# locuoco/coulomb_oscillators

Measured on AMD Instinct MI355X. Metric: particle-steps/sec (+ Gpair-interactions/sec), N=1048576 FMM-3D kd-tree p=6, 1 GPU(s), higher is better.
Workload: dtype f32; 1 GPU; FMM-3D kd-tree p=6, N=1048576 per GPU (one system of 1048576), leapfrog, Gaussian ball, tree rebuilt every 1 step(s); n_per_gpu=1048576, order=6, parallelism=single GPU, L=15, p2p_pairs=2017200, m2l_pairs=570291, build_mode=0, warm_builds=281, warm_misses=10, near_field=one-directional

## Files before the change

coulomb_oscillators_amd/csrc/k_farfield.hip:

```cpp
#include "nbco_internal.hpp"

namespace {

#include "fmm_ops.hpp"

constexpr int kBlock = 256;
constexpr int kTopNodes = 256;

__device__ inline float ld_agent(const float *p) { return __hip_atomic_load(p, __ATOMIC_RELAXED, __HIP_MEMORY_SCOPE_AGENT); }
__device__ inline int ld_agent(const int *p) { return __hip_atomic_load(p, __ATOMIC_RELAXED, __HIP_MEMORY_SCOPE_AGENT); }

template <int P, typename T>
__global__ __launch_bounds__(kBlock) void p2m_gen_kernel(const float4 *__restrict__ pos, const float *__restrict__ center,
                                                         const int *__restrict__ mult, const int *__restrict__ index, T *__restrict__ mpole,
                                                         int beg, int nleaf)
{
	constexpr int offM = P * (P + 1) * (P + 2) / 6;
	const int i = blockIdx.x * kBlock + threadIdx.x;
	if (i >= nleaf) return;
	const int leaf = beg + i, mlt = mult[leaf], ind = index[leaf];
	const T cx = (T)center[3 * leaf], cy = (T)center[3 * leaf + 1], cz = (T)center[3 * leaf + 2];
	T A[offM > 0 ? offM : 1];
#pragma unroll
	for (int k = 0; k < (offM > 0 ? offM : 1); ++k) A[k] = T(0);
// ... 32 lines not shown
	{
		float s = f0 * c0[a];
		s = s + f1 * c1[a];
		c[a] = s / ft;
	}
}
__device__ inline float4 node_csz(const float *__restrict__ lbound, const float *__restrict__ rbound, int i, float cx, float cy, float cz)
{
	const float dx = rbound[3 * i] - lbound[3 * i], dy = rbound[3 * i + 1] - lbound[3 * i + 1], dz = rbound[3 * i + 2] - lbound[3 * i + 2];
	const float sz = dx * dx + dy * dy + dz * dz;
	return make_float4(cx, cy, cz, sz);
}
#pragma clang fp contract(on)

__global__ __launch_bounds__(kBlock) void kd_centres_kernel(float *center, int *mult, int L, int lr, const float *__restrict__ lbound,
                                                            const float *__restrict__ rbound, float4 *__restrict__ csz, int leaves_too)
{
	__shared__ float Cl[kBlock][3];
	__shared__ int Nl[kBlock];
	const int t = threadIdx.x, b = blockIdx.x;
	const int nl = 1 << (L - lr);
	if (t < nl)
	{
		const int leaf = (1 << L) - 1 + b * nl + t;
		Cl[t][0] = center[3 * leaf]; Cl[t][1] = center[3 * leaf + 1]; Cl[t][2] = center[3 * leaf + 2];
		Nl[t] = mult[leaf];
		if (leaves_too) csz[leaf] = node_csz(lbound, rbound, leaf, Cl[t][0], Cl[t][1], Cl[t][2]);
	}
	__syncthreads();
	for (int l = L - 1; l >= lr; --l)
	{
		const int cnt = 1 << (l - lr);
		float c[3] = {0.f, 0.f, 0.f};
		int m0 = 0, m1 = 0;
		if (t < cnt)
		{
			m0 = Nl[2 * t]; m1 = Nl[2 * t + 1];
			centre_of(m0, m1, Cl[2 * t], Cl[2 * t + 1], c);
		}
		__syncthreads();
		if (t < cnt)
		{
			const int node = (1 << l) - 1 + b * cnt + t;
			Cl[t][0] = c[0]; Cl[t][1] = c[1]; Cl[t][2] = c[2];
			Nl[t] = m0 + m1;
			center[3 * node] = c[0]; center[3 * node + 1] = c[1]; center[3 * node + 2] = c[2];
			mult[node] = m0 + m1;
			csz[node] = node_csz(lbound, rbound, node, c[0], c[1], c[2]);
		}
		__syncthreads();
	}
}
__global__ __launch_bounds__(kBlock) void kd_centres_top_kernel(float *center, int *mult, int ltop, const float *__restrict__ lbound,
                                                                const float *__restrict__ rbound, float4 *__restrict__ csz)
{
	__shared__ float Cl[kBlock][3];
	__shared__ int Nl[kBlock];
	const int t = threadIdx.x;
	for (int l = ltop; l >= 0; --l)
	{
		const int cnt = 1 << l;
		float c[3] = {0.f, 0.f, 0.f};
		int mlt = 0;
		if (t < cnt)
		{
			if (l == ltop) parent_centre<false>(center, mult, (1 << l) - 1 + t, c, mlt);
			else
			{
				const int m0 = Nl[2 * t], m1 = Nl[2 * t + 1];
				centre_of(m0, m1, Cl[2 * t], Cl[2 * t + 1], c);
				mlt = m0 + m1;
			}
		}
		__syncthreads();
		if (t < cnt)
		{
			const int node = (1 << l) - 1 + t;
			Cl[t][0] = c[0]; Cl[t][1] = c[1]; Cl[t][2] = c[2];
			Nl[t] = mlt;
			center[3 * node] = c[0]; center[3 * node + 1] = c[1]; center[3 * node + 2] = c[2];
			mult[node] = mlt;
			csz[node] = node_csz(lbound, rbound, node, c[0], c[1], c[2]);
		}
		__syncthreads();
	}
}

template <int P, typename T>
__global__ __launch_bounds__(kTopNodes) void m2m_top_kernel(float *center, T *mpole, int *mult, int ltop, int lroot, int write_geom)
{
	constexpr int offM = P * (P + 1) * (P + 2) / 6, offS = offM > 0 ? offM : 1;
	extern __shared__ __attribute__((aligned(16))) unsigned char lds_raw[];
	const int width = 1 << (ltop - lroot);
	T *Ml = reinterpret_cast<T *>(lds_raw);
	float *Cl = reinterpret_cast<float *>(Ml + (size_t)width * offS);
	int *Nl = (int *)(Cl + (size_t)width * 3);
	const int t = threadIdx.x;
	for (int l = ltop; l >= lroot; --l)
	{
		const bool on = t < (1 << (l - lroot));
		const int k = (1 << l) - 1 + ((int)blockIdx.x << (l - lroot)) + t;
		T A[offS];
		float c[3] = {0.f, 0.f, 0.f};
		int mlt = 0;
		if (on)
		{
#pragma unroll
			for (int q = 0; q < offS; ++q) A[q] = T(0);
			if (l == ltop)
			{
				parent_centre<false>(center, mult, k, c, mlt);
				if (P >= 3)
					for (int ch = 0; ch < 2; ++ch)
					{
						const int child = 2 * k + 1 + ch;
						m2m_accum<P>(mpole + (size_t)child * offM, (T)c[0] - (T)center[3 * child], (T)c[1] - (T)center[3 * child + 1],
						             (T)c[2] - (T)center[3 * child + 2], A);
					}
			}
			else
			{
				const int s0 = 2 * t, s1 = 2 * t + 1;
				const int m0 = Nl[s0], m1 = Nl[s1];
				mlt = m0 + m1;
				centre_of(m0, m1, Cl + 3 * s0, Cl + 3 * s1, c);
				if (P >= 3)
					for (int ch = 0; ch < 2; ++ch)
					{
						const int sl = 2 * t + ch;
						m2m_accum<P>(Ml + (size_t)sl * offS, (T)c[0] - (T)Cl[3 * sl], (T)c[1] - (T)Cl[3 * sl + 1], (T)c[2] - (T)Cl[3 * sl + 2], A);
					}
			}
		}
		__syncthreads();
		if (on)
		{
			T *M = mpole + (size_t)k * offM;
			T *Ms = Ml + (size_t)t * offS;
			if (offM > 0) M[0] = (T)mlt;
			if (offM > 1) { M[1] = T(0); M[2] = T(0); M[3] = T(0); }
			m2m_store<P>(A, M);
			if (offM > 0) Ms[0] = (T)mlt;
			if (offM > 1) { Ms[1] = T(0); Ms[2] = T(0); Ms[3] = T(0); }
			m2m_store<P>(A, Ms);
			if (write_geom)
			{
				center[3 * k] = c[0]; center[3 * k + 1] = c[1]; center[3 * k + 2] = c[2];
				mult[k] = mlt;
			}
			Cl[3 * t] = c[0]; Cl[3 * t + 1] = c[1]; Cl[3 * t + 2] = c[2];
			Nl[t] = mlt;
		}
		__syncthreads();
	}
}

template <int P, typename T, bool AGENT>
__device__ inline void l2l_node(const float *center, T *local, int c)
{
	constexpr int offL = (P + 1) * (P + 1);
	const int p = (c - 1) >> 1;
	T Lp[offL], O[offL];
#pragma unroll
	for (int q = 0; q < offL; ++q) Lp[q] = local[(size_t)p * offL + q];
	l2l_body<P>(Lp, (T)center[3 * c] - (T)center[3 * p], (T)center[3 * c + 1] - (T)center[3 * p + 1], (T)center[3 * c + 2] - (T)center[3 * p + 2], O);
	T *Lc = local + (size_t)c * offL;
#pragma unroll
	for (int q = 1; q < offL; ++q) Lc[q] += O[q];
}

template <int P, typename T>
__global__ __launch_bounds__(kBlock) void l2l_gen_kernel(const float *__restrict__ center, T *local, int lchild, int first, int count)
{
	const int i = blockIdx.x * kBlock + threadIdx.x;
	if (i >= count) return;
	l2l_node<P, T, false>(center, local, (1 << lchild) - 1 + first + i);
}

template <int P, typename T>
__global__ __launch_bounds__(256) void l2l_sub_kernel(const float *__restrict__ center, T *local, int lroot, int L, int first)
{
	constexpr int offL = (P + 1) * (P + 1);
	extern __shared__ __attribute__((aligned(16))) unsigned char lds_raw[];
	T *lds = reinterpret_cast<T *>(lds_raw);
	const int t = threadIdx.x, r = first + blockIdx.x;
	for (int q = t; q < offL; q += blockDim.x) lds[q] = local[(size_t)((1 << lroot) - 1 + r) * offL + q];
	__syncthreads();
	for (int lc = lroot + 1; lc <= L; ++lc)
	{
		const bool on = t < (1 << (lc - lroot));
		const int c = (1 << lc) - 1 + (r << (lc - lroot)) + t, p = (c - 1) >> 1;
		T O[offL];
		if (on)
		{
			T Lp[offL];
			const T *src = lds + (size_t)(t >> 1) * offL;
#pragma unroll
			for (int q = 0; q < offL; ++q) Lp[q] = src[q];
			l2l_body<P>(Lp, (T)center[3 * c] - (T)center[3 * p], (T)center[3 * c + 1] - (T)center[3 * p + 1], (T)center[3 * c + 2] - (T)center[3 * p + 2], O);
			T *Lc = local + (size_t)c * offL;
#pragma unroll
			for (int q = 1; q < offL; ++q) { O[q] += Lc[q]; Lc[q] = O[q]; }
			O[0] = T(0);
		}
		if (lc == L) break;
		__syncthreads();
		if (on)
		{
			T *dst = lds + (size_t)t * offL;
#pragma unroll
			for (int q = 0; q < offL; ++q) dst[q] = O[q];
		}
		__syncthreads();
	}
}

template <int P, typename T>
__global__ __launch_bounds__(kBlock) void l2p_gen_kernel(const float4 *__restrict__ pos, const float *__restrict__ center,
                                                         const T *__restrict__ local, const float4 *__restrict__ near,
                                                         const int *__restrict__ chunk_off, const int *__restrict__ index, int mlt_max,
                                                         const int *__restrict__ unsort, int scatter, const float *__restrict__ param,
                                                         float *__restrict__ a_out, int have_near, long long n, int L, long long own0,
                                                         long long own_n, const int2 *__restrict__ sec_range, const float4 *__restrict__ react,
                                                         int react_cap, int react_stride)
{
	constexpr int offL = (P + 1) * (P + 1);
	const long long io = (long long)blockIdx.x * kBlock + threadIdx.x;
	if (io >= own_n) return;
	const long long i = own0 + io;
	const int lf = (int)(((1LL << L) * i) / n), leaf = (1 << L) - 1 + lf;
	const float4 p = pos[i];
	T Lp[offL];
#pragma unroll
	for (int q = 0; q < offL; ++q) Lp[q] = local[(size_t)leaf * offL + q];
	T fx, fy, fz;
	l2p_body<P>(Lp, (T)p.x - (T)center[3 * leaf], (T)p.y - (T)center[3 * leaf + 1], (T)p.z - (T)center[3 * leaf + 2], fx, fy, fz);
	if (have_near)
	{
		const int j = (int)(i - index[leaf]);
		float nx = 0.f, ny = 0.f, nz = 0.f;
		int ck0 = chunk_off[lf], ck1 = chunk_off[lf + 1];
		if (!NBCO_CHECKED_OK(ck0 >= 0 && ck0 <= ck1 && j >= 0 && j < mlt_max, NBCO_CHK_L2P)) ck1 = ck0;
#pragma unroll 8
		for (int ck = ck0; ck < ck1; ++ck)
		{
			const float4 nr = near[(size_t)ck * mlt_max + j];
			nx += nr.x; ny += nr.y; nz += nr.z;
		}
		if (sec_range)
		{
			int2 sr = sec_range[lf];
			if (!NBCO_CHECKED_OK(sr.x >= 0 && sr.x <= sr.y, NBCO_CHK_L2P)) sr.y = sr.x;
			if (sr.y > react_cap) sr.y = max(sr.x, react_cap);
#pragma unroll 8
			for (int e = sr.x; e < sr.y; ++e)
			{
				const float4 rr = react[(size_t)e * react_stride + j];
				nx += rr.x; ny += rr.y; nz += rr.z;
			}
		}
		fx += (T)nx; fy += (T)ny; fz += (T)nz;
	}
	const T scale = param ? (T)param[0] : T(1);
	const long long o = scatter ? (long long)unsort[io] : io;
	a_out[3 * o] = (float)(fx * scale); a_out[3 * o + 1] = (float)(fy * scale); a_out[3 * o + 2] = (float)(fz * scale);
}

#include "farfield_wide.hpp"

static int grid_for(long long n) { return (int)((n + kBlock - 1) / kBlock); }

template <int P, typename T>
static int run_upward_gen(nbco_ctx *c, const float4 *pos, float *center, T *mpole, int *mult, const int *index, int L, int write_geom)
{
	const int nleaf = 1 << L, beg = nleaf - 1;
	hipLaunchKernelGGL((p2m_gen_kernel<P, T>), dim3(grid_for(nleaf)), dim3(kBlock), 0, c->stream, pos, (const float *)center, (const int *)mult, index,
	                   mpole, beg, nleaf);
	constexpr int offM = P * (P + 1) * (P + 2) / 6, offS = offM > 0 ? offM : 1;
	int depth = 8;
	while (depth > 0 && (size_t)(1 << depth) * (offS * sizeof(T) + 16) > 60 * 1024) --depth;
	for (int l = L - 1; l >= 0;)
	{
		const int lroot = std::max(l - depth, 0), width = 1 << (l - lroot);
		hipLaunchKernelGGL((m2m_top_kernel<P, T>), dim3(1 << lroot), dim3(std::max(64, width)), (size_t)width * (offS * sizeof(T) + 16), c->stream, center, mpole,
		                   mult, l, lroot, write_geom);
		l = lroot - 1;
	}
	NBCO_HIP(hipGetLastError());
	return NBCO_OK;
}

template <int P, typename T>
static int run_m2m_top_gen(nbco_ctx *c, float *center, T *mpole, int *mult, int ltop, int write_geom)
{
	constexpr int offM = P * (P + 1) * (P + 2) / 6, offS = offM > 0 ? offM : 1;
	if ((1 << ltop) > kTopNodes || (size_t)(1 << ltop) * (offS * sizeof(T) + 16) > 60 * 1024)
		return c->fail(NBCO_ERR_UNSUPPORTED, "launch_m2m_top_gen: too many top levels");
	hipLaunchKernelGGL((m2m_top_kernel<P, T>), dim3(1), dim3(kTopNodes), (size_t)(1 << ltop) * (offS * sizeof(T) + 16), c->stream, center, mpole, mult, ltop, 0,
	                   write_geom);
	NBCO_HIP(hipGetLastError());
	return NBCO_OK;
}

template <int P, typename T>
static int run_downward_gen(nbco_ctx *c, const float *center, T *local, int L, int dom_d, int dom_g)
{
	constexpr int offL = (P + 1) * (P + 1);
	int top = kTopNodes;
	while (top > 4 && (size_t)top * offL * sizeof(T) > 60 * 1024) top >>= 1;
	int ltop = 1;
	while (ltop + 1 <= L && (1 << (ltop + 1)) <= top) ++ltop;
	{
	}
	constexpr int offD = P * (P + 1) * (P + 2) / 6;
	const int threads = 64 * ((std::max(offD, offL) + 63) / 64);
	const int wtop = ltop >= 2 ? std::max(ltop, L - 7) : 1;
	int lroot = L;
	if (ltop >= 2)
	{
		lroot = wtop;
		while (lroot < L && (size_t)(1 << (L - lroot - 1)) * offL * sizeof(T) > 60 * 1024) ++lroot;
		if (lroot < dom_d) lroot = L;
	}
	for (int lc = 2; lc <= lroot; ++lc)
	{
		const int first = lc >= dom_d ? dom_g << (lc - dom_d) : 0, count = lc >= dom_d ? 1 << (lc - dom_d) : 1 << lc;
		if (lc <= wtop) hipLaunchKernelGGL((l2l_wide_kernel<P, T>), dim3(count), dim3(threads), 0, c->stream, center, local, lc, first);
		else hipLaunchKernelGGL((l2l_gen_kernel<P, T>), dim3(grid_for(count)), dim3(kBlock), 0, c->stream, center, local, lc, first, count);
	}
	if (lroot < L)
	{
		const int first = dom_g << (lroot - dom_d), count = 1 << (lroot - dom_d);
		hipLaunchKernelGGL((l2l_sub_kernel<P, T>), dim3(count), dim3(std::max(64, 1 << (L - lroot))), (size_t)(1 << (L - lroot - 1)) * offL * sizeof(T),
		                   c->stream, center, local, lroot, L, first);
	}
	NBCO_HIP(hipGetLastError());
	return NBCO_OK;
}

template <int P, typename T>
static void launch_m2m_wide(nbco_ctx *c, float *center, T *mpole, int *mult, int l, int height, int write_geom)
{
	if (height <= 4) hipLaunchKernelGGL((m2m_wide_kernel<P, T, false>), dim3(1 << l), dim3(kWide), 0, c->stream, center, mpole, mult, l, write_geom);
	else hipLaunchKernelGGL((m2m_wide_kernel<P, T, true>), dim3(1 << l), dim3(kWide), 0, c->stream, center, mpole, mult, l, write_geom);
}
template <int P, typename T>
static int run_upward(nbco_ctx *c, const float4 *pos, float *center, T *mpole, int *mult, const int *index, int L, int write_geom)
{
	if constexpr (use_wide<P, T>())
	{
		const int nleaf = 1 << L;
		hipLaunchKernelGGL((p2m_wide_kernel<P, T>), dim3(nleaf), dim3(kWide), 0, c->stream, pos, (const float *)center, (const int *)mult, index, mpole,
		                   nleaf - 1);
		for (int l = L - 1; l >= 0; --l) launch_m2m_wide<P, T>(c, center, mpole, mult, l, L - l, write_geom);
		NBCO_HIP(hipGetLastError());
		return NBCO_OK;
	}
	else return run_upward_gen<P, T>(c, pos, center, mpole, mult, index, L, write_geom);
}
template <int P, typename T>
static int run_m2m_top(nbco_ctx *c, float *center, T *mpole, int *mult, int ltop, int L, int write_geom)
{
	if constexpr (use_wide<P, T>())
	{
		for (int l = ltop; l >= 0; --l) launch_m2m_wide<P, T>(c, center, mpole, mult, l, L - l, write_geom);
		NBCO_HIP(hipGetLastError());
		return NBCO_OK;
	}
	else return run_m2m_top_gen<P, T>(c, center, mpole, mult, ltop, write_geom);
}
template <int P, typename T>
static int run_downward(nbco_ctx *c, const float *center, T *local, int L, int dom_d, int dom_g)
{
	if constexpr (use_wide<P, T>())
	{
		for (int lc = 2; lc <= L; ++lc)
		{
			const int first = lc >= dom_d ? dom_g << (lc - dom_d) : 0, count = lc >= dom_d ? 1 << (lc - dom_d) : 1 << lc;
			hipLaunchKernelGGL((l2l_wide_kernel<P, T>), dim3(count), dim3(kWide), 0, c->stream, center, local, lc, first);
		}
		NBCO_HIP(hipGetLastError());
		return NBCO_OK;
	}
	else return run_downward_gen<P, T>(c, center, local, L, dom_d, dom_g);
}

template <int P, typename T>
static int run_l2p(nbco_ctx *c, const float4 *pos, const float *center, const T *local, const float4 *near, const int *chunk_off,
                   const int *index, int mlt_max, const int *unsort, int scatter, const float *param, float *a, int have_near, long long n, int L,
                   long long own0, long long own_n, const int2 *sec_range, const float4 *react, long long react_cap, int react_stride)
{
	hipLaunchKernelGGL((l2p_gen_kernel<P, T>), dim3(grid_for(own_n)), dim3(kBlock), 0, c->stream, pos, center, local, near, chunk_off, index, mlt_max,
	                   unsort, scatter, param, a, have_near, n, L, own0, own_n, sec_range, react, (int)std::min<long long>(react_cap, 0x7fffffff), react_stride);
	NBCO_HIP(hipGetLastError());
	return NBCO_OK;
}

}

#define NBCO_DISPATCH_P(P, CALL)                                                       \
	switch (P)                                                                         \
	{                                                                                  \
	case 1: return CALL(1); case 2: return CALL(2); case 3: return CALL(3); case 4: return CALL(4); \
	case 5: return CALL(5); case 6: return CALL(6); case 7: return CALL(7); case 8: return CALL(8); \
	case 9: return CALL(9); case 10: return CALL(10);                                                \
	default: return c->fail(NBCO_ERR_UNSUPPORTED, "generated far-field operators exist for orders 1..10"); \
	}

int launch_kd_centres(nbco_ctx *c, float *center, int *mult, int L, const float *lbound, const float *rbound, float4 *csz)
{
	if (L == 0)
	{
		hipLaunchKernelGGL(kd_centres_kernel, dim3(1), dim3(kBlock), 0, c->stream, center, mult, 0, 0, lbound, rbound, csz, 1);
		NBCO_HIP(hipGetLastError());
		return NBCO_OK;
	}
	int bottom = L;
	for (; bottom > 16; bottom -= 8)
		hipLaunchKernelGGL(kd_centres_kernel, dim3(1 << (bottom - 8)), dim3(kBlock), 0, c->stream, center, mult, bottom, bottom - 8, lbound, rbound, csz,
		                   bottom == L ? 1 : 0);
	const int lr = bottom > 8 ? bottom - 8 : 0;
	hipLaunchKernelGGL(kd_centres_kernel, dim3(1 << lr), dim3(kBlock), 0, c->stream, center, mult, bottom, lr, lbound, rbound, csz, bottom == L ? 1 : 0);
	if (lr > 0) hipLaunchKernelGGL(kd_centres_top_kernel, dim3(1), dim3(kBlock), 0, c->stream, center, mult, lr - 1, lbound, rbound, csz);
	NBCO_HIP(hipGetLastError());
	return NBCO_OK;
}

int launch_upward_gen(nbco_ctx *c, int P, const float4 *pos, float *center, void *mpole, int *mult, const int *index, int L, int write_geom, int f64)
{
	if (f64)
	{
#define CALL(PP) run_upward<PP, double>(c, pos, center, (double *)mpole, mult, index, L, write_geom)
		NBCO_DISPATCH_P(P, CALL)
#undef CALL
	}
#define CALL(PP) run_upward<PP, float>(c, pos, center, (float *)mpole, mult, index, L, write_geom)
	NBCO_DISPATCH_P(P, CALL)
#undef CALL
}

int launch_kd_centres_top(nbco_ctx *c, float *center, int *mult, int ltop, const float *lbound, const float *rbound, float4 *csz)
{
	if ((1 << ltop) > kBlock) return c->fail(NBCO_ERR_UNSUPPORTED, "launch_kd_centres_top: too many top levels");
	hipLaunchKernelGGL(kd_centres_top_kernel, dim3(1), dim3(kBlock), 0, c->stream, center, mult, ltop, lbound, rbound, csz);
	NBCO_HIP(hipGetLastError());
	return NBCO_OK;
}

int launch_m2m_top_gen(nbco_ctx *c, int P, float *center, void *mpole, int *mult, int ltop, int L, int write_geom, int f64)
{
	if (f64)
	{
#define CALL(PP) run_m2m_top<PP, double>(c, center, (double *)mpole, mult, ltop, L, write_geom)
		NBCO_DISPATCH_P(P, CALL)
#undef CALL
	}
#define CALL(PP) run_m2m_top<PP, float>(c, center, (float *)mpole, mult, ltop, L, write_geom)
	NBCO_DISPATCH_P(P, CALL)
#undef CALL
}

int launch_downward_gen(nbco_ctx *c, int P, const float *center, void *local, int L, int dom_d, int dom_g, int f64)
{
	if (f64)
	{
#define CALL(PP) run_downward<PP, double>(c, center, (double *)local, L, dom_d, dom_g)
		NBCO_DISPATCH_P(P, CALL)
#undef CALL
	}
#define CALL(PP) run_downward<PP, float>(c, center, (float *)local, L, dom_d, dom_g)
	NBCO_DISPATCH_P(P, CALL)
#undef CALL
}

int launch_l2p_gen(nbco_ctx *c, int P, const float4 *pos, const float *center, const void *local, const float4 *near, const int *chunk_off,
                   const int *index, int mlt_max, const int *unsort, int scatter, const float *param, float *a, int have_near, long long n, int L,
                   long long own0, long long own_n, const int2 *sec_range, const float4 *react, long long react_cap, int react_stride, int f64)
{
	if (f64)
	{
#define CALL(PP) run_l2p<PP, double>(c, pos, center, (const double *)local, near, chunk_off, index, mlt_max, unsort, scatter, param, a, have_near, n, L, own0, own_n, sec_range, react, react_cap, react_stride)
		NBCO_DISPATCH_P(P, CALL)
#undef CALL
	}
#define CALL(PP) run_l2p<PP, float>(c, pos, center, (const float *)local, near, chunk_off, index, mlt_max, unsort, scatter, param, a, have_near, n, L, own0, own_n, sec_range, react, react_cap, react_stride)
	NBCO_DISPATCH_P(P, CALL)
#undef CALL
}

NBCO_CHECKED_COLLECT(nbco_checked_collect_far)
```

coulomb_oscillators_amd/csrc/k_fmm_kd.hip:

```cpp
#include "nbco_internal.hpp"
#include "k_p2p.hpp"
#include "kd_common.hpp"
#include "host_util.hpp"
#include <chrono>
#include <cmath>
#include <algorithm>
#include <vector>

namespace {

using kdc::wave_scan_add;
using kdc::wave_min_u32;

constexpr int sym_off(int n) { return n * (n + 1) * (n + 2) / 6; }
constexpr int tl_off(int n) { return n * n; }

struct TreeView
{
	float *center, *lbound, *rbound;
	float4 *csz;
	float *mpole, *local;
	int *mult, *index, *splitdim;
	int L, ntot;
};

constexpr int kBlock = 256;

__host__ __device__ inline int kd_beg(int l) { return (1 << l) - 1; }
__host__ __device__ inline int kd_cnt(int l) { return 1 << l; }

struct Dom
{
	int d, g;
};
__host__ __device__ inline bool dom_touch(const Dom dm, int node)
{
#ifdef __HIP_DEVICE_COMPILE__
	const int l = 31 - __clz(node + 1);
#else
	int l = 0;
	while ((2 << l) <= node + 1) ++l;
#endif
	const int pos = node - ((1 << l) - 1);
	return l >= dm.d ? (pos >> (l - dm.d)) == dm.g : (dm.g >> (dm.d - l)) == pos;
}

#include "kd_build_kernels.hpp"
#include "kd_traverse_kernels.hpp"
#include "kd_list_kernels.hpp"

static int kd_levels(long long n, int p, float dens_inhom, int tree_L)
{
	int L;
	if (tree_L == 0)
	{
		float s = (float)(p * p);
		L = (int)std::round(std::log2(dens_inhom * (float)n / s));
	}
	else L = tree_L;
	L = std::max(2, std::min(30, L));
	while ((1LL << L) > n) --L;
	return L;
}

static TreeView view_of(const KdTreeDev &k)
{
	TreeView t;
	t.center = k.center; t.lbound = k.lbound; t.rbound = k.rbound; t.csz = k.csz; t.mpole = k.mpole; t.local = k.local;
	t.mult = k.mult; t.index = k.index; t.splitdim = k.splitdim; t.L = k.L; t.ntot = k.ntot;
	return t;
}

struct PackCounts
{
	__host__ __device__ uint64_t operator()(unsigned cnt) const { return (uint64_t)cnt | ((uint64_t)((cnt + kP2PChunk - 1) / kP2PChunk) << 32); }
};
struct SplitRef
{
	int *s, *o;
	__host__ __device__ SplitRef &operator=(uint64_t v) { *s = (int)(uint32_t)v; *o = (int)(v >> 32); return *this; }
};
struct SplitIter
{
	using iterator_category = std::random_access_iterator_tag;
	using value_type = uint64_t;
	using difference_type = std::ptrdiff_t;
	using pointer = uint64_t *;
	using reference = SplitRef;
	int *s, *o;
	__host__ __device__ SplitRef operator*() const { return SplitRef{s, o}; }
	__host__ __device__ SplitRef operator[](difference_type i) const { return SplitRef{s + i, o + i}; }
	__host__ __device__ SplitIter operator+(difference_type i) const { return SplitIter{s + i, o + i}; }
	__host__ __device__ SplitIter operator-(difference_type i) const { return SplitIter{s - i, o - i}; }
	__host__ __device__ SplitIter &operator+=(difference_type i) { s += i; o += i; return *this; }
	__host__ __device__ SplitIter &operator++() { ++s; ++o; return *this; }
	__host__ __device__ difference_type operator-(const SplitIter &b) const { return s - b.s; }
};
static int build_directed_list(nbco_ctx *c, const int2 *pairs, const int2 *ranks, const int *pref_dev, long long capR, long long npairs_hint, int sub,
                               int self0, int nself, int ntargets, int shift, unsigned *cnt, int *start, uint64_t *keys_tmp, uint64_t *keys_out,
                               DevBuf &scan_tmp, const int *leaf_index = nullptr, const int *leaf_mult = nullptr, int2 *desc = nullptr,
                               int *chunk_off = nullptr, int4 *chunks = nullptr, const MutualLists *mutual = nullptr)
{
	hipStream_t st = c->stream;
	if (desc)
	{
		NBCO_TRY(exclusive_scan(c, scan_tmp, rocprim::make_transform_iterator((const unsigned *)cnt, PackCounts{}), SplitIter{start, chunk_off}, (uint64_t)0,
		                        (size_t)(ntargets + 1)));
	}
	else
		NBCO_TRY(exclusive_scan(c, scan_tmp, (int *)cnt, start, 0, (size_t)(ntargets + 1)));
	hipLaunchKernelGGL(list_fill_kernel, dim3(grid1d(npairs_hint + nself)), dim3(kBlock), 0, st, pairs, ranks, pref_dev, capR, sub, self0, nself, shift,
	                   (const int *)start, keys_tmp, (const int *)chunk_off, ntargets, leaf_index, leaf_mult,
	                   (desc && !mutual) ? chunks : (int4 *)nullptr, mutual ? 1 : 0);
	if (desc)
	{
		MutualLists mu;
		if (mutual) { mu = *mutual; mu.chunk = chunks; mu.chunk_off = chunk_off; mu.self0 = self0; mu.nself = nself; }
		const bool long_kernel = shift >= 11 && shift <= 16 && c->hint_np2p > 0 && 2 * c->hint_np2p > 48LL * (nself > 0 ? nself : ntargets);
		const int long_from = long_kernel ? 512 : 0;
		c->info.long_lists = long_kernel ? 1 : 0;
		hipLaunchKernelGGL(list_segsort_kernel<true>, dim3((ntargets + kBlock / 64 - 1) / (kBlock / 64)), dim3(kBlock), 0, st, (const int *)start, ntargets,
		                   keys_tmp, keys_out, shift, leaf_index, leaf_mult, desc, mu, long_from);
		if (long_kernel)
			hipLaunchKernelGGL(list_longsort_kernel, dim3(256), dim3(kLongBlock), 0, st, (const int *)start,
			                   ntargets, (const uint64_t *)keys_tmp, keys_out, shift, leaf_index, leaf_mult, desc, mu, long_from);
	}
	else
		hipLaunchKernelGGL(list_segsort_kernel<false>, dim3((ntargets + kBlock / 64 - 1) / (kBlock / 64)), dim3(kBlock), 0, st, (const int *)start,
		                   ntargets, keys_tmp, keys_out, shift, (const int *)nullptr, (const int *)nullptr, (int2 *)nullptr, MutualLists{}, 0);
	NBCO_HIP(hipGetLastError());
	return NBCO_OK;
}

static int kd_carve(nbco_ctx *c, DevBuf &buf, KdTreeDev &k, int ntot, int offM, int offL)
{
	const size_t rb = c->o.far_fp64 ? 8 : 4;
	k.real_bytes = (int)rb;
	size_t bytes = (size_t)ntot * (3 * 3 * sizeof(float) + sizeof(float4) + (size_t)(offM + offL) * rb + 3 * sizeof(int)) + 256 + 64;
	NBCO_TRY(c->reserve(buf, bytes));
	char *q = (char *)buf.ptr;
	k.csz = (float4 *)q; q += sizeof(float4) * (size_t)ntot;
	k.center = (float *)q; q += 12 * (size_t)ntot;
	k.lbound = (float *)q; q += 12 * (size_t)ntot;
	k.rbound = (float *)q; q += 12 * (size_t)ntot;
	q = (char *)(((uintptr_t)q + 15) & ~(uintptr_t)15);
	k.mpole = (float *)q; q += rb * (size_t)ntot * offM;
	q = (char *)(((uintptr_t)q + 15) & ~(uintptr_t)15);
	k.local = (float *)q; q += rb * (size_t)ntot * offL;
	q = (char *)(((uintptr_t)q + 15) & ~(uintptr_t)15);
	k.mult = (int *)q; q += 4 * (size_t)ntot;
	k.index = (int *)q; q += 4 * (size_t)ntot;
	k.splitdim = (int *)q;
	return NBCO_OK;
}

static int kd_build_top(nbco_ctx *c, const TreeView &tv, float4 *&pos, float4 *&pos_alt, int *&unsort, int *&unsort_alt, long long n, int l0,
                        bool use_select, bool select_ready = false, bool warm = false, const KdRoot &root = KdRoot{})
{
	hipStream_t st = c->stream;
	if (use_select && l0 > 0 && !select_ready) NBCO_TRY(kd_select_begin(c, l0));
	for (int l = 0; l < l0; ++l)
	{
		if (use_select)
			NBCO_TRY(kd_select_level(c, l, n, pos, unsort, pos_alt, unsort_alt, tv.lbound, tv.rbound, tv.splitdim, tv.index,
			                         c->counters.as<int>() + 110, warm, root));
		else
		{
			if (l > 0) hipLaunchKernelGGL(kd_box_kernel, dim3(grid1d(kd_cnt(l))), dim3(kBlock), 0, st, tv, pos, n, l);
			hipLaunchKernelGGL(kd_keys_kernel, dim3(grid1d(n)), dim3(kBlock), 0, st, pos, tv.splitdim + kd_beg(l), n, l,
			                   c->keys.as<uint64_t>(), c->idx.as<uint32_t>());
			NBCO_TRY(sort_pairs(c, c->sort_tmp, c->keys.as<uint64_t>(), c->keys_alt.as<uint64_t>(), c->idx.as<uint32_t>(), c->idx_alt.as<uint32_t>(), n, 0u,
			                    (unsigned)(32 + l)));
			hipLaunchKernelGGL(kd_permute_kernel, dim3(grid1d(n)), dim3(kBlock), 0, st, pos, unsort, c->idx_alt.as<uint32_t>(), pos_alt, unsort_alt, n);
		}
		std::swap(pos, pos_alt);
		std::swap(unsort, unsort_alt);
	}
	if (l0 > 0 && !use_select) hipLaunchKernelGGL(kd_box_kernel, dim3(grid1d(kd_cnt(l0))), dim3(kBlock), 0, st, tv, pos, n, l0);
	NBCO_HIP(hipGetLastError());
	return NBCO_OK;
}

static int kd_reserve_particles(nbco_ctx *c, long long n)
{
	NBCO_TRY(c->reserve(c->pos4, sizeof(float4) * (size_t)n));
	NBCO_TRY(c->reserve(c->pos4_alt, sizeof(float4) * (size_t)n));
	NBCO_TRY(c->reserve(c->unsort, sizeof(int) * (size_t)n));
	NBCO_TRY(c->reserve(c->unsort_alt, sizeof(int) * (size_t)n));
	NBCO_TRY(c->reserve(c->keys, sizeof(uint64_t) * (size_t)n));
	NBCO_TRY(c->reserve(c->keys_alt, sizeof(uint64_t) * (size_t)n));
	NBCO_TRY(c->reserve(c->idx, sizeof(uint32_t) * (size_t)n));
	NBCO_TRY(c->reserve(c->idx_alt, sizeof(uint32_t) * (size_t)n));
	NBCO_TRY(c->reserve(c->counters, sizeof(int) * 128));
	return NBCO_OK;
}

static int kd_top_levels(long long n, int L)
{
	int l0 = 0;
	while (l0 < L && (n + (1LL << l0) - 1) / (1LL << l0) > kSubS) ++l0;
	return l0;
}

static int kd_build(nbco_ctx *c, const float *p, long long n, int L, const KdRoot &root, bool &rebuild, KdStepLink *link)
{
	const int P = c->o.fmm_order;
	const int ntot = (1 << (L + 1)) - 1, nleaf = 1 << L;
	const int mlt_max = (int)((n - 1) / nleaf + 1);
	hipStream_t st = c->stream;
	NBCO_TRY(c->join_aux());
	KdTreeDev &k = c->kd;
	const int old_real = k.real_bytes;
	NBCO_TRY(kd_carve(c, c->treebuf, k, ntot, sym_off(P), tl_off(P + 1)));
	const bool topo_change = k.L != L || k.ntot != ntot || k.order != P || k.n != n || k.real_bytes != old_real;
	if (topo_change) c->tree_valid = false;
	k.L = L; k.ntot = ntot; k.order = P; k.mlt_max = mlt_max; k.n = n;
	NBCO_TRY(kd_reserve_particles(c, n));
	rebuild = c->o.unsort || !c->tree_valid || (c->eval_counter % c->o.tree_steps) == 0;
	TreeView tv = view_of(c->kd);
	float4 *pos = c->pos4.as<float4>(), *pos_alt = c->pos4_alt.as<float4>();
	int *unsort = c->unsort.as<int>(), *unsort_alt = c->unsort_alt.as<int>();
	PhaseScope ph(c, NBCO_PH_BUILD);
	const int prep_done = link ? link->prep_done : 0;
	if (rebuild)
	{
		const int l0 = kd_top_levels(n, L);
		const bool use_select = !c->force_sort_build;
		long long words_a = 0, words_b = 0;
		if (use_select && l0 > 0) NBCO_TRY(kd_select_begin(c, l0, false, &words_a, &words_b));
		if (!c->prep_state.ptr)
		{
			NBCO_TRY(c->reserve(c->prep_state, 64));
			const unsigned arm[8] = {0xFFFFFFFFu, 0xFFFFFFFFu, 0xFFFFFFFFu, 0u, 0u, 0u, 0u, 0u};
			NBCO_HIP(hipMemcpyAsync(c->prep_state.ptr, arm, sizeof arm, hipMemcpyHostToDevice, st));
			NBCO_HIP(hipStreamSynchronize(st));
		}
		if (c->perm_primed_n != n)
		{
			hipLaunchKernelGGL(iota_kernel, dim3(grid1d(n)), dim3(kBlock), 0, st, unsort_alt, n);
			hipLaunchKernelGGL(iota_kernel, dim3(grid1d(n)), dim3(kBlock), 0, st, unsort, n);
			c->perm_primed_n = n;
		}
		if (prep_done != 1)
			hipLaunchKernelGGL(kd_prep_kernel, dim3(kPrepGrid), dim3(kPrepBlock), 0, st, p, n, pos, unsort, c->sel_hist.as<uint32_t>(), words_a,
			                   c->sel_nodes.as<uint32_t>(), words_b, c->counters.as<int>() + 110, c->prep_state.as<unsigned>(), tv, root.root6);
		bool warm = use_select && l0 > 0 && c->sel_warm_enabled && c->tree_valid && !c->sel_three_pass;
		if (warm && c->sel_warm_cooldown > 0) { --c->sel_warm_cooldown; warm = false; }
		c->sel_warm_used = warm;
		if (warm) ++c->sel_warm_builds;
		NBCO_TRY(kd_build_top(c, tv, pos, pos_alt, unsort, unsort_alt, n, l0, use_select, true, warm, root));
		int launches = 1;
#ifdef NBCO_SUBTREE_PROF
		if (std::getenv("NBCO_SUBTREE_TWICE")) launches = 2;
#endif
		for (int i = 0; i < launches; ++i)
			hipLaunchKernelGGL(kd_subtree_kernel, dim3(kd_cnt(l0)), dim3(kSubT), 0, st, tv, (const float4 *)pos, (const int *)unsort, pos_alt, unsort_alt, n, l0,
			                   use_select ? 1 : 0, c->sel_three_pass ? 0 : 1, c->counters.as<int>() + 110, root.top_sd, root.top_root1);
		std::swap(pos, pos_alt);
		std::swap(unsort, unsort_alt);
		NBCO_HIP(hipGetLastError());
		if (pos != c->pos4.as<float4>()) { std::swap(c->pos4, c->pos4_alt); std::swap(c->unsort, c->unsort_alt); }
	}
	else
	{
		c->sel_warm_used = false;
		if (prep_done == 0)
		{
			NBCO_TRY(launch_pack4(c, pos, p, n));
			NBCO_HIP(hipMemsetAsync(c->counters.as<int>() + 110, 0, sizeof(int), st));
		}
		hipLaunchKernelGGL(kd_leaf_kernel, dim3(grid1d(nleaf)), dim3(kBlock), 0, st, tv, pos, n);
	}
	if (link) link->prep_done = 0;
	NBCO_TRY(launch_kd_centres(c, tv.center, tv.mult, L, tv.lbound, tv.rbound, tv.csz));
	NBCO_HIP(hipGetLastError());
	return NBCO_OK;
}

static int kd_upward(nbco_ctx *c)
{
	const KdTreeDev &k = c->kd;
	NBCO_TRY(c->fork_aux());
	StreamScope on_aux(c, c->aux);
	PhaseScope ph(c, NBCO_PH_P2M_M2M);
	NBCO_TRY(launch_upward_gen(c, k.order, c->pos4.as<float4>(), k.center, k.mpole, k.mult, k.index, k.L, 0, k.real_bytes == 8));
	NBCO_HIP(hipGetLastError());
	return NBCO_OK;
}

struct LetHave { const unsigned char *node, *leaf; };
constexpr int kLetWord = 16;
__global__ __launch_bounds__(kBlock) void let_guard_kernel(const uint64_t *__restrict__ keys, const int *__restrict__ total, int shift,
                                                           const unsigned char *__restrict__ have, int *__restrict__ host_word)
{
	const uint64_t mask = (1ull << shift) - 1;
	const int n = *total;
	int missing = 0;
	for (int i = blockIdx.x * kBlock + threadIdx.x; i < n; i += gridDim.x * kBlock)
	{
		const int id = (int)(keys[i] & mask);
		if (!have[id]) missing = id + 1;
	}
	if (missing) { *host_word = missing; __threadfence_system(); }
}
static int launch_let_guard(nbco_ctx *c, const uint64_t *keys, const int *total, int shift, const unsigned char *have, int word, long long hint)
{
	hipLaunchKernelGGL(let_guard_kernel, dim3(grid1d(hint, 2048)), dim3(kBlock), 0, c->stream, keys, total, shift, have,
	                   c->h_flags + kLetWord + 2 * (int)(c->dist.let_epoch & 1) + word);
	NBCO_HIP(hipGetLastError());
	return NBCO_OK;
}

struct KdCounts
{
	long long np2p = 0, nm2l = 0;
	int sel_overflow = 0, react_overflow = 0;
};

static int kd_list_room(nbco_ctx *c, int ntot, long long &capR, long long &cap)
{
	capR = 2 * (((long long)c->o.list_factor * c->list_growth * ntot + 4096 + kTravK - 1) / kTravK);
	cap = capR * kTravK;
	NBCO_TRY(c->reserve(c->frontier_a, sizeof(int2) * (size_t)cap));
	NBCO_TRY(c->reserve(c->frontier_b, sizeof(int2) * (size_t)cap));
	NBCO_TRY(c->reserve(c->p2p_list, sizeof(int2) * 2 * (size_t)cap));
	NBCO_TRY(c->reserve(c->m2l_list, sizeof(int2) * 2 * (size_t)cap));
	NBCO_TRY(c->reserve(c->counters, sizeof(int) * 128));
	c->list_cap = cap;
	return NBCO_OK;
}

static int kd_traverse(nbco_ctx *c, const TreeView &tv, long long n, const Dom dm)
{
	const int L = tv.L, ntot = tv.ntot, nleaf = 1 << L;
	const int self0 = dm.g << (L - dm.d), nself = 1 << (L - dm.d);
	hipStream_t st = c->stream;
	long long capR, cap;
	NBCO_TRY(kd_list_room(c, ntot, capR, cap));
	PhaseScope ph(c, NBCO_PH_TRAVERSE);
	AdmTab tab;
	for (int l = 0; l < 32; ++l)
	{
		long long lo = l <= L ? (n >> l) : 0;
		long long hi = l <= L ? ((n + (1LL << l) - 1) >> l) : 0;
		tab.lo[l] = (int)lo;
		const float e = 1.f / (float)(3 * c->o.fmm_order + 6);
		tab.Mlo[l] = lo > 0 ? std::pow((float)lo / (float)n, e) : 0.f;
		tab.Mhi[l] = hi > 0 ? std::pow((float)hi / (float)n, e) : 0.f;
	}
	int *ctr = c->counters.as<int>();
	int2 *fa = c->frontier_a.as<int2>(), *fb = c->frontier_b.as<int2>();
	const size_t np_ = (size_t)nleaf + 2, nm_ = (size_t)ntot + 2;
	NBCO_TRY(c->reserve(c->list_cnt, sizeof(unsigned) * 2 * (np_ + nm_)));
	unsigned *cnt_p2p = c->list_cnt.as<unsigned>(), *cnt_m2l = cnt_p2p + 2 * np_;
	NBCO_TRY(c->reserve(c->trav_ctr, sizeof(int) * 1024));
	static_assert(kTcInts <= 1024, "traversal counter block");
	int *tctr = c->trav_ctr.as<int>();
	NBCO_TRY(c->flags_begin());
	hipLaunchKernelGGL(traverse_init_kernel, dim3(grid1d((long long)(2 * (np_ + nm_)) / 8 + 1, 256)), dim3(kBlock), 0, st, fa, ctr, 104, tctr,
	                   c->list_cnt.as<unsigned>(), (long long)(2 * (np_ + nm_)), (long long)self0, (long long)(c->o.coll ? nself : 0));
	const int iters = L + NBCO_TRAV_EXTRA;
	for (int it = 0; it < iters; ++it)
	{
		hipLaunchKernelGGL(traverse_kernel, dim3(1024), dim3(kBlock), 0, st, tv, tab, (const int2 *)fa, fb, c->p2p_list.as<int2>(),
		                   c->m2l_list.as<int2>(), c->p2p_list.as<int2>() + cap, c->m2l_list.as<int2>() + cap, ctr, tctr, it, capR,
		                   c->o.tree_radius, c->o.m2l_first, cnt_p2p, cnt_m2l, dm);
		std::swap(fa, fb);
	}
	hipLaunchKernelGGL(traverse_finish_kernel, dim3(1), dim3(1024), 0, st, ctr, tctr, capR, c->list_cnt.as<unsigned>(), (long long)(2 * (np_ + nm_)),
	                   cnt_p2p + self0, c->o.coll ? nself : 0, c->h_flags, iters, ++c->flags_seq);
	NBCO_HIP(hipGetLastError());
	NBCO_HIP(hipEventRecord(c->ev_flags, st));
	return NBCO_OK;
}

static int kd_no_pre_far() { return NBCO_OK; }

template <class PreFar>
static int kd_fields(nbco_ctx *c, const TreeView &tv, const float4 *pos, long long n, int mlt_max, const Dom dm, long long own0, long long own_n,
                     const int *unsort, float *a, const float *param, KdCounts &out, PreFar pre_far, const LetHave *let = nullptr)
{
	const int P = c->o.fmm_order;
	const int L = tv.L, ntot = tv.ntot, nleaf = 1 << L, beg = kd_beg(L);
	const int offL = tl_off(P + 1);
	out = KdCounts{};
	const int self0 = dm.g << (L - dm.d), nself = 1 << (L - dm.d);
	long long capR, cap;
	NBCO_TRY(kd_list_room(c, ntot, capR, cap));
	const int *p2p_pref = c->trav_ctr.as<int>() + kTcP2PPref, *m2l_pref = c->trav_ctr.as<int>() + kTcM2LPref;
	const int shift = L + 1;
	const long long dp2p_cap = c->o.coll ? 2 * cap + nself : 0, dm2l_cap = 2 * cap;
	const long long np2p_hint = c->hint_np2p > 0 ? std::min(cap, c->hint_np2p + c->hint_np2p / 4 + 1024) : cap;
	const long long nm2l_hint = c->hint_nm2l > 0 ? std::min(cap, c->hint_nm2l + c->hint_nm2l / 4 + 1024) : cap;
	const long long dp2p_hint = 2 * np2p_hint + nself;
	const long long max_chunks = c->o.coll ? dp2p_cap / kP2PChunk + nself : 0, chunks_hint = dp2p_hint / kP2PChunk + nself;
	const int mutual_th = (c->o.coll && c->o.p2p_mutual) ? p2p_mutual_halves(mlt_max) : 0;
	const bool mutual = mutual_th > 0;
	c->info.p2p_halves = mutual_th;
	long long react_cap = 0;
	if (mutual)
	{
		if (c->hint_np2p <= 0)
		{
			NBCO_TRY(c->wait_flags());
			c->hint_np2p = c->h_flags[0];
			c->hint_nm2l = c->h_flags[1];
		}
		const long long pairs_room = std::min(cap, c->hint_np2p + c->hint_np2p / 4 + 1024);
		react_cap = 2 * pairs_room + nself;
		NBCO_TRY(c->reserve(c->p2p_react, sizeof(float4) * 32 * (size_t)mutual_th * (size_t)react_cap));
	}
	float4 *near = nullptr;
	auto enqueue_p2p = [&]() -> int {
		NBCO_TRY(c->reserve(c->part, sizeof(float4) * (size_t)max_chunks * (size_t)mlt_max));
		near = c->part.as<float4>();
		PhaseScope ph(c, NBCO_PH_P2P);
		const int4 *pc = c->p2p_chunks.as<int4>();
		const int *pt = c->p2p_chunk_off.as<int>() + nleaf;
		const int2 *pd = c->p2p_desc.as<int2>();
		if (mutual)
		{
			launch_p2p_mutual(c, mutual_th, pos, c->p2p_desc.as<int4>(), pc, pt, chunks_hint, mlt_max, near, c->p2p_react.as<float4>(), react_cap, n);
		}
		else if (mlt_max <= 8) launch_p2p<8>(c, pos, pd, pc, pt, chunks_hint, mlt_max, mlt_max, near, n);
		else if (mlt_max <= 16) launch_p2p<16>(c, pos, pd, pc, pt, chunks_hint, mlt_max, mlt_max, near, n);
		else if (mlt_max <= 32) launch_p2p<32>(c, pos, pd, pc, pt, chunks_hint, mlt_max, mlt_max, near, n);
		else launch_p2p<64>(c, pos, pd, pc, pt, chunks_hint, mlt_max, mlt_max, near, n);
		NBCO_HIP(hipGetLastError());
		static const char *dump_path = std::getenv("NBCO_P2P_DUMP");
		if (dump_path && !mutual) NBCO_TRY(p2p_dump(c, dump_path, pos, pd, pc, pt, c->p2p_start.as<int>() + nleaf, mlt_max, near, n));
		return NBCO_OK;
	};
	{
		NBCO_TRY(c->reserve(c->p2p_keys, sizeof(uint64_t) * (size_t)(dp2p_cap + 1)));
		NBCO_TRY(c->reserve(c->p2p_keys_alt, sizeof(uint64_t) * (size_t)(dp2p_cap + 1)));
		NBCO_TRY(c->reserve(c->m2l_keys, sizeof(uint64_t) * (size_t)(dm2l_cap + 1)));
		NBCO_TRY(c->reserve(c->m2l_keys_alt, sizeof(uint64_t) * (size_t)(dm2l_cap + 1)));
		NBCO_TRY(c->reserve(c->p2p_start, sizeof(int) * (size_t)(nleaf + 2)));
		NBCO_TRY(c->reserve(c->m2l_start, sizeof(int) * (size_t)(ntot + 2)));
		NBCO_TRY(c->fork_mark());
		if (c->o.coll)
		{
			PhaseScope ph(c, NBCO_PH_LISTS);
			unsigned *cp = c->list_cnt.as<unsigned>();
			NBCO_TRY(c->reserve(c->p2p_desc, (mutual ? sizeof(int4) : sizeof(int2)) * (size_t)(dp2p_cap + 1)));
			MutualLists mu;
			if (mutual)
			{
				NBCO_TRY(c->reserve(c->p2p_sec, sizeof(int2) * (size_t)(nleaf + 2)));
				mu.desc4 = c->p2p_desc.as<int4>();
				mu.sec_range = c->p2p_sec.as<int2>();
			}
			NBCO_TRY(c->reserve(c->p2p_chunk_off, sizeof(int) * (size_t)(nleaf + 2)));
			NBCO_TRY(c->reserve(c->p2p_chunks, sizeof(int4) * (size_t)max_chunks));
			NBCO_TRY(build_directed_list(c, c->p2p_list.as<int2>(), c->p2p_list.as<int2>() + cap, p2p_pref, capR, np2p_hint, beg, self0, nself, nleaf, shift, cp,
			                             c->p2p_start.as<int>(), c->p2p_keys.as<uint64_t>(), c->p2p_keys_alt.as<uint64_t>(), c->sort_tmp,
			                             tv.index + beg, tv.mult + beg, c->p2p_desc.as<int2>(), c->p2p_chunk_off.as<int>(), c->p2p_chunks.as<int4>(),
			                             mutual ? &mu : nullptr));
			if (mutual) launch_p2p_link(c, c->p2p_desc.as<int4>(), c->p2p_keys_alt.as<uint64_t>(), c->p2p_start.as<int>(), c->p2p_start.as<int>() + nleaf, shift, dp2p_hint);
			if (let) NBCO_TRY(launch_let_guard(c, c->p2p_keys_alt.as<uint64_t>(), c->p2p_start.as<int>() + nleaf, shift, let->leaf, 1, dp2p_hint));
			c->pc_mult = tv.mult + beg; c->pc_shift = shift; c->pc_total = c->p2p_start.as<int>() + nleaf;
		}
		if (c->o.coll) NBCO_TRY(enqueue_p2p());
		const int f64 = c->o.far_fp64 ? 1 : 0;
		NBCO_HIP(hipMemsetAsync(tv.local, 0, (f64 ? sizeof(double) : sizeof(float)) * (size_t)ntot * offL, c->aux));
		NBCO_TRY(c->fork_wait());
		{
			StreamScope on_aux(c, c->aux);
			NBCO_TRY(pre_far());
			unsigned *cm = c->list_cnt.as<unsigned>() + 2 * ((size_t)nleaf + 2);
			NBCO_TRY(build_directed_list(c, c->m2l_list.as<int2>(), c->m2l_list.as<int2>() + cap, m2l_pref, capR, nm2l_hint, 0, 0, 0, ntot, shift, cm,
			                             c->m2l_start.as<int>(), c->m2l_keys.as<uint64_t>(), c->m2l_keys_alt.as<uint64_t>(), c->scan_tmp_aux));
			if (let) NBCO_TRY(launch_let_guard(c, c->m2l_keys_alt.as<uint64_t>(), c->m2l_start.as<int>() + ntot, shift, let->node, 0, 2 * nm2l_hint));
			{
				PhaseScope ph(c, NBCO_PH_M2L);
				if (f64) NBCO_TRY(launch_m2l_lanes_f64(c, P, tv.csz, (const double *)tv.mpole, (double *)tv.local, c->m2l_keys_alt.as<uint64_t>(), c->m2l_start.as<int>(), shift, ntot));
				else NBCO_TRY(launch_m2l_lanes(c, P, tv.csz, tv.mpole, tv.local, c->m2l_keys_alt.as<uint64_t>(), c->m2l_start.as<int>(), shift, ntot));
			}
			{
				PhaseScope ph(c, NBCO_PH_L2L);
				NBCO_TRY(launch_downward_gen(c, P, tv.center, tv.local, L, dm.d, dm.g, f64));
			}
		}
		NBCO_HIP(hipGetLastError());
	}
	NBCO_TRY(c->join_aux());
	{
		PhaseScope ph(c, NBCO_PH_L2P);
		NBCO_TRY(launch_l2p_gen(c, P, pos, tv.center, tv.local, near, c->p2p_chunk_off.as<int>(), tv.index, mlt_max, unsort, c->o.unsort ? 1 : 0,
		                        param, a, c->o.coll ? 1 : 0, n, L, own0, own_n, mutual ? c->p2p_sec.as<int2>() : nullptr,
		                        mutual ? c->p2p_react.as<float4>() : nullptr, react_cap, 32 * mutual_th, c->o.far_fp64 ? 1 : 0));
	}
	{
		const auto t0 = std::chrono::steady_clock::now();
		NBCO_TRY(c->wait_flags());
		c->host_wait_s += std::chrono::duration<double>(std::chrono::steady_clock::now() - t0).count();
	}
	const int *h = c->h_flags;
	if (h[3] != 0)
	{
		out.sel_overflow = 1;
		return NBCO_OK;
	}
	if (h[2] == 2) return c->fail(NBCO_ERR_HIP, "internal error: the dual tree traversal did not finish in its launches");
	if (h[2] != 0) return c->fail(NBCO_ERR_CAPACITY, "dual tree traversal exceeded the list capacity (raise opts.list_factor or set opts.list_grow)");
	out.np2p = h[0]; out.nm2l = h[1];
	c->hint_np2p = h[0]; c->hint_nm2l = h[1];
	{
		nbco_ctx::LastEval &le = c->last_eval;
		le.valid = true;
		le.center = tv.center; le.csz = tv.csz; le.mpole = tv.mpole; le.mult = tv.mult; le.index = tv.index;
		le.L = L; le.ntot = ntot; le.order = P; le.shift = shift; le.real_bytes = c->o.far_fp64 ? 8 : 4;
		le.pos = pos; le.n = n; le.own0 = own0; le.own_n = own_n;
		le.have_p2p = c->o.coll != 0;
	}
	if (mutual && 2LL * h[0] + nself > react_cap) out.react_overflow = 1;
	return NBCO_OK;
}

static int kd_finish_order(nbco_ctx *c, float *p, long long n, KdStepLink *link)
{
	PhaseScope ph(c, NBCO_PH_FINISH);
	hipStream_t st = c->stream;
	NBCO_TRY(c->reserve(c->tmp3, sizeof(float) * 3 * (size_t)n));
	const int *order_in = nullptr;
	int *order_out = nullptr;
	if (c->o.track_order)
	{
		NBCO_TRY(c->reserve(c->order, sizeof(int) * (size_t)n));
		NBCO_TRY(c->reserve(c->order_alt, sizeof(int) * (size_t)n));
		if (c->order_n == n) order_in = c->order.as<int>();
		order_out = c->order_alt.as<int>();
	}
	else c->order_n = -1;
	hipLaunchKernelGGL(reorder_state_kernel, dim3(grid1d(n)), dim3(kBlock), 0, st, (const float4 *)c->pos4.as<float4>(), (const int *)c->unsort.as<int>(),
	                   (const float *)(p + 3 * n), p, c->tmp3.as<float>(), n, order_in, order_out);
	if (order_out) { std::swap(c->order, c->order_alt); c->order_n = n; }
	if (link && link->defer_v_copy) link->v_now = c->tmp3.as<float>();
	else NBCO_HIP(hipMemcpyAsync(p + 3 * n, c->tmp3.ptr, sizeof(float) * 3 * (size_t)n, hipMemcpyDeviceToDevice, st));
	NBCO_HIP(hipGetLastError());
	return NBCO_OK;
}

#include "kd_energy_kernels.hpp"
}

int kd_energy_fmm(nbco_ctx *c, long long n_own, double *half_phi_sum)
{
	const nbco_ctx::LastEval &le = c->last_eval;
	if (!le.valid || !c->tree_valid) return c->fail(NBCO_ERR_ARG, "nbco_energy_fmm: no kd-tree evaluation to take the lists from");
	if (le.own_n != n_own) return c->fail(NBCO_ERR_ARG, "nbco_energy_fmm: particle count differs from the last evaluation's");
	const int grid = (int)((le.own_n + kBlock - 1) / kBlock);
	NBCO_TRY(c->reserve(c->part, sizeof(double) * (size_t)grid));
	double *part = c->part.as<double>();
	switch (le.order)
	{
	case 1: launch_potential<1>(c, grid, part); break;
	case 2: launch_potential<2>(c, grid, part); break;
	case 3: launch_potential<3>(c, grid, part); break;
	case 4: launch_potential<4>(c, grid, part); break;
	case 5: launch_potential<5>(c, grid, part); break;
	case 6: launch_potential<6>(c, grid, part); break;
	case 7: launch_potential<7>(c, grid, part); break;
	case 8: launch_potential<8>(c, grid, part); break;
	case 9: launch_potential<9>(c, grid, part); break;
	case 10: launch_potential<10>(c, grid, part); break;
	default: return c->fail(NBCO_ERR_UNSUPPORTED, "nbco_energy_fmm: order");
	}
	NBCO_HIP(hipGetLastError());
	std::vector<double> h((size_t)grid);
	NBCO_HIP(hipMemcpyAsync(h.data(), part, sizeof(double) * (size_t)grid, hipMemcpyDeviceToHost, c->stream));
	NBCO_HIP(hipStreamSynchronize(c->stream));
	double s = 0.0;
	for (double v : h) s += v;
	*half_phi_sum = 0.5 * s;
	return NBCO_OK;
}

static bool kd_wants_room(nbco_ctx *c, int rc, const KdCounts &cnt, int ntot)
{
	if (rc == NBCO_ERR_CAPACITY) return c->grow_lists(ntot);
	return rc == NBCO_OK && cnt.react_overflow && !cnt.sel_overflow;
}

static int kd_retry(nbco_ctx *c, int rc, const KdCounts &cnt, bool rebuild, int ntot, bool &again)
{
	again = true;
	if (kd_wants_room(c, rc, cnt, ntot)) return NBCO_OK;
	if (rc != NBCO_OK) return rc;
	if (cnt.sel_overflow)
		return c->demote_build() ? NBCO_OK : c->fail(NBCO_ERR_UNSUPPORTED, "kd-tree build: tie flag raised by the sorting build");
	if (rebuild && c->sel_warm_used) c->note_warm_ok();
	again = false;
	return NBCO_OK;
}

static void kd_commit(nbco_ctx *c, const KdTreeDev &k, long long n, const KdCounts &cnt, bool rebuilt)
{
	c->tree_valid = true;
	c->tree_n = n;
	c->tree_order = k.order;
	c->eval_counter += 1;
	nbco_kd_info &info = c->info;
	info.L = k.L; info.ntot = k.ntot; info.order = k.order; info.mlt_max = k.mlt_max; info.n = k.n;
	info.p2p_pairs = cnt.np2p; info.m2l_pairs = cnt.nm2l; info.rebuilt = rebuilt ? 1 : 0;
	info.directed_p2p = -1;
}

int kd_finish_pending_order(nbco_ctx *c, float *p, long long n, KdStepLink *link)
{
	if (!link->order_pending) return NBCO_OK;
	link->order_pending = false;
	return kd_finish_order(c, p, n, link);
}

int kd_turnaround(nbco_ctx *c, float *p, const float *param, float ks, float ds, bool elastic, long long n, KdStepLink *link, const float *root6)
{
	const bool gather = link->order_pending;
	link->order_pending = false;
	float *x = p, *v = p + 3 * n, *a = p + 6 * n;
	const float *v_in = link->v_now ? link->v_now : v;
	const int L = c->kd.L;
	const bool next_rebuild = (c->eval_counter % c->o.tree_steps) == 0;
	long long words_a = 0, words_b = 0;
	if (next_rebuild)
	{
		const int l0 = kd_top_levels(n, L);
		if (!c->force_sort_build && l0 > 0) NBCO_TRY(kd_select_begin(c, l0, false, &words_a, &words_b));
	}
	float *v_out = v;
	if (gather)
	{
		NBCO_TRY(c->reserve(c->tmp3, sizeof(float) * 3 * (size_t)n));
		NBCO_TRY(c->reserve(c->tmp3b, sizeof(float) * 3 * (size_t)n));
		v_out = v_in == c->tmp3.as<float>() ? c->tmp3b.as<float>() : c->tmp3.as<float>();
	}
	else if (v_in != v) v_out = const_cast<float *>(v_in);
	PhaseScope ph(c, NBCO_PH_AXPY);
	TreeView tv = view_of(c->kd);
	hipStream_t st = c->stream;
#define NBCO_TURN_ARGS c->pos4.as<float4>(), c->unsort.as<int>(), x, v_in, v_out, (const float *)a, param, ks, ds, elastic ? 1 : 0, n, next_rebuild ? 1 : 0, \
	c->sel_hist.as<uint32_t>(), words_a, c->sel_nodes.as<uint32_t>(), words_b, c->counters.as<int>() + 110, c->prep_state.as<unsigned>(), tv, root6
	if (gather) hipLaunchKernelGGL(kd_turnaround_kernel<true>, dim3(kPrepGrid), dim3(kPrepBlock), 0, st, NBCO_TURN_ARGS);
	else hipLaunchKernelGGL(kd_turnaround_kernel<false>, dim3(kPrepGrid), dim3(kPrepBlock), 0, st, NBCO_TURN_ARGS);
#undef NBCO_TURN_ARGS
	NBCO_HIP(hipGetLastError());
	link->prep_done = next_rebuild ? 1 : 2;
	c->order_n = -1;
	c->last_eval.valid = false;
	link->v_now = v_out == v ? nullptr : v_out;
	return NBCO_OK;
}

int fmm_kdtree_eval(nbco_ctx *c, float *p, float *a, long long n, const float *param, KdStepLink *link)
{
	if (n <= 0) return c->fail(NBCO_ERR_ARG, "nbco_fmm_kdtree: n must be positive");
	if (n > 0x7fffffffLL / 4) return c->fail(NBCO_ERR_UNSUPPORTED, "nbco_fmm_kdtree: n too large for 32-bit tree indices");
	const int L = kd_levels(n, c->o.fmm_order, c->o.dens_inhom, c->o.tree_L);
	const Dom whole{0, 0};
	bool rebuild = false;
	KdCounts cnt;
	for (bool again = true; again;)
	{
		NBCO_TRY(kd_build(c, p, n, L, KdRoot{}, rebuild, link));
		NBCO_TRY(kd_upward(c));
		const TreeView tv = view_of(c->kd);
		int rc = kd_traverse(c, tv, n, whole);
		if (rc == NBCO_OK) rc = kd_fields(c, tv, c->pos4.as<float4>(), n, c->kd.mlt_max, whole, 0, n, c->unsort.as<int>(), a, param, cnt, kd_no_pre_far);
		NBCO_TRY(kd_retry(c, rc, cnt, rebuild, c->kd.ntot, again));
	}
	if (!c->o.unsort && rebuild)
	{
		if (link && link->defer_order) link->order_pending = true;
		else NBCO_TRY(kd_finish_order(c, p, n, link));
	}
	kd_commit(c, c->kd, n, cnt, rebuild);
	return NBCO_OK;
}

#include "kd_dist.hpp"
#include "kd_let.hpp"
int kd_count_pairs(nbco_ctx *c, long long *out)
{
	if (!c->pc_mult || !c->p2p_keys_alt.ptr) { *out = 0; return NBCO_OK; }
	unsigned long long *ctr = (unsigned long long *)(c->counters.as<int>() + 100);
	NBCO_HIP(hipMemsetAsync(ctr, 0, sizeof(unsigned long long), c->stream));
	hipLaunchKernelGGL(pair_count_kernel, dim3(1024), dim3(kBlock), 0, c->stream, c->pc_mult, (const uint64_t *)c->p2p_keys_alt.as<uint64_t>(), c->pc_total,
	                   c->pc_shift, ctr);
	NBCO_HIP(hipGetLastError());
	unsigned long long v = 0;
	NBCO_HIP(hipMemcpyAsync(&v, ctr, sizeof v, hipMemcpyDeviceToHost, c->stream));
	NBCO_HIP(hipStreamSynchronize(c->stream));
	*out = (long long)v;
	return NBCO_OK;
}

int kd_copy_out(nbco_ctx *c, int which, void *dst, long long bytes)
{
	const KdTreeDev &k = c->kd;
	if (!c->tree_valid) return c->fail(NBCO_ERR_ARG, "nbco_kd_copy: no kd-tree evaluation has run");
	const void *src = nullptr;
	size_t need = 0;
	const int offM = sym_off(k.order), offL = tl_off(k.order + 1);
	switch (which)
	{
	case NBCO_KD_MULT: src = k.mult; need = 4 * (size_t)k.ntot; break;
	case NBCO_KD_INDEX: src = k.index; need = 4 * (size_t)k.ntot; break;
	case NBCO_KD_SPLITDIM: src = k.splitdim; need = 4 * (size_t)k.ntot; break;
	case NBCO_KD_CENTER: src = k.center; need = 12 * (size_t)k.ntot; break;
	case NBCO_KD_LBOUND: src = k.lbound; need = 12 * (size_t)k.ntot; break;
	case NBCO_KD_RBOUND: src = k.rbound; need = 12 * (size_t)k.ntot; break;
	case NBCO_KD_MPOLE: src = k.mpole; need = (size_t)k.real_bytes * (size_t)k.ntot * offM; break;
	case NBCO_KD_LOCAL: src = k.local; need = (size_t)k.real_bytes * (size_t)k.ntot * offL; break;
	case NBCO_KD_P2P_LIST:
	case NBCO_KD_M2L_LIST:
	{
		const bool p2p = which == NBCO_KD_P2P_LIST;
		need = 8 * (size_t)(p2p ? c->info.p2p_pairs : c->info.m2l_pairs);
		const long long capR = c->list_cap / kTravK;
		hipLaunchKernelGGL(list_compact_kernel, dim3(1024), dim3(kBlock), 0, c->stream, (const int2 *)(p2p ? c->p2p_list.ptr : c->m2l_list.ptr),
		                   (const int *)(c->trav_ctr.as<int>() + (p2p ? kTcP2PPref : kTcM2LPref)), capR, c->frontier_a.as<int2>());
		NBCO_HIP(hipGetLastError());
		src = c->frontier_a.ptr;
		break;
	}
	case NBCO_KD_UNSORT: src = c->unsort.ptr; need = 4 * (size_t)k.n; break;
	case NBCO_KD_ORDER:
		if (!c->o.track_order || c->order_n != k.n) return c->fail(NBCO_ERR_ARG, "nbco_kd_copy: NBCO_KD_ORDER needs opts.track_order and unsort = 0 evaluations");
		src = c->order.ptr; need = 4 * (size_t)k.n; break;
	default: return c->fail(NBCO_ERR_ARG, "nbco_kd_copy: unknown array");
	}
	if ((long long)need > bytes) return c->fail(NBCO_ERR_ARG, "nbco_kd_copy: destination too small");
	NBCO_HIP(hipStreamSynchronize(c->stream));
	if (need) NBCO_HIP(hipMemcpy(dst, src, need, hipMemcpyDeviceToHost));
	return NBCO_OK;
}

NBCO_CHECKED_COLLECT(nbco_checked_collect_kd)
```

coulomb_oscillators_amd/csrc/k_m2l.hip:

```cpp
#include "nbco_internal.hpp"

namespace {

__device__ __forceinline__ float nb_fma(float a, float b, float c) { return __builtin_fmaf(a, b, c); }
__device__ __forceinline__ double nb_fma(double a, double b, double c) { return __builtin_fma(a, b, c); }
__device__ __forceinline__ float nb_sqrt(float x) { return sqrtf(x); }
__device__ __forceinline__ double nb_sqrt(double x) { return sqrt(x); }

template <int P, typename T> struct M2LBody;

#include "m2l_gen.inc"

constexpr int kTargets = 6;

template <int P, typename T>
__global__ __launch_bounds__(64) void m2l_lane_kernel(const float4 *__restrict__ csz, const T *__restrict__ mpole,
                                                      T *__restrict__ local, const uint64_t *__restrict__ keys,
                                                      const int *__restrict__ start, int shift, int ntot, float eps2, int mstride)
{
	constexpr int offM = P * (P + 1) * (P + 2) / 6, offL = (P + 1) * (P + 1), NOUT = offL - 1;
	constexpr int CPL = (NOUT + 63) / 64;
	__shared__ T buf[64][NOUT + 1 + (NOUT % 2)];
	__shared__ int tg[64];
	const int lane = threadIdx.x;
	const int t0 = blockIdx.x * kTargets, t1 = min(t0 + kTargets, ntot);
	const int i0 = start[t0], i1 = start[t1];
	const uint64_t mask = (1ull << shift) - 1;
	T acc[CPL];
#pragma unroll
	for (int q = 0; q < CPL; ++q) acc[q] = T(0);
	int cur = -1;
	for (int base = i0; base < i1; base += 64)
	{
		const int i = base + lane;
		int tgt = -1;
		T L[NOUT];
		if (i < i1)
		{
			const uint64_t key = keys[i];
			tgt = (int)(key >> shift);
			const int src = (int)(key & mask);
			const float4 ct = csz[tgt], cs = csz[src];
			const T dx = (T)ct.x - (T)cs.x, dy = (T)ct.y - (T)cs.y, dz = (T)ct.z - (T)cs.z;
			const T r = nb_sqrt(dx * dx + dy * dy + dz * dz + (T)eps2);
			const T rinv = T(1) / r;
			M2LBody<P, T>::run(mpole + (size_t)src * mstride, dx * rinv, dy * rinv, dz * rinv, rinv, L);
		}
		else
		{
#pragma unroll
			for (int c = 0; c < NOUT; ++c) L[c] = T(0);
		}
#pragma unroll
		for (int c = 0; c < NOUT; ++c) buf[lane][c] = L[c];
		tg[lane] = tgt;
		__syncthreads();
		const int rows = min(64, i1 - base);
		constexpr int RB = 8;
		for (int r0 = 0; r0 < rows; r0 += RB)
		{
			T v[RB][CPL];
			int tt[RB];
#pragma unroll
			for (int k = 0; k < RB; ++k)
			{
				const int r = min(r0 + k, 63);
				tt[k] = tg[r];
#pragma unroll
				for (int q = 0; q < CPL; ++q)
				{
					const int c = lane + 64 * q;
					v[k][q] = c < NOUT ? buf[r][c] : T(0);
				}
			}
#pragma unroll
			for (int k = 0; k < RB; ++k)
			{
				if (r0 + k >= rows) break;
				const int t = tt[k];
				if (t != cur)
				{
					if (cur >= 0)
					{
#pragma unroll
						for (int q = 0; q < CPL; ++q)
						{
							const int c = lane + 64 * q;
							if (c < NOUT) local[(size_t)cur * offL + 1 + c] = acc[q];
						}
					}
#pragma unroll
					for (int q = 0; q < CPL; ++q) acc[q] = T(0);
					cur = t;
				}
#pragma unroll
				for (int q = 0; q < CPL; ++q) acc[q] += v[k][q];
			}
		}
		__syncthreads();
	}
	if (cur >= 0)
	{
#pragma unroll
		for (int q = 0; q < CPL; ++q)
		{
			const int c = lane + 64 * q;
			if (c < NOUT) local[(size_t)cur * offL + 1 + c] = acc[q];
		}
	}
}

template <int P, typename T>
static void launch(nbco_ctx *c, const float4 *csz, const T *mpole, T *local, const uint64_t *keys, const int *start, int shift, int ntot, int mstride)
{
	const int grid = (ntot + kTargets - 1) / kTargets;
	hipLaunchKernelGGL((m2l_lane_kernel<P, T>), dim3(grid), dim3(64), 0, c->stream, csz, mpole, local, keys, start, shift, ntot, c->o.eps2,
	                   mstride > 0 ? mstride : P * (P + 1) * (P + 2) / 6);
}

template <typename T>
static int dispatch(nbco_ctx *c, int P, const float4 *csz, const T *mpole, T *local, const uint64_t *keys, const int *start, int shift, int ntot, int mstride)
{
	switch (P)
	{
	case 1: launch<1, T>(c, csz, mpole, local, keys, start, shift, ntot, mstride); break;
	case 2: launch<2, T>(c, csz, mpole, local, keys, start, shift, ntot, mstride); break;
	case 3: launch<3, T>(c, csz, mpole, local, keys, start, shift, ntot, mstride); break;
	case 4: launch<4, T>(c, csz, mpole, local, keys, start, shift, ntot, mstride); break;
	case 5: launch<5, T>(c, csz, mpole, local, keys, start, shift, ntot, mstride); break;
	case 6: launch<6, T>(c, csz, mpole, local, keys, start, shift, ntot, mstride); break;
	case 7: launch<7, T>(c, csz, mpole, local, keys, start, shift, ntot, mstride); break;
	case 8: launch<8, T>(c, csz, mpole, local, keys, start, shift, ntot, mstride); break;
	case 9: launch<9, T>(c, csz, mpole, local, keys, start, shift, ntot, mstride); break;
	case 10: launch<10, T>(c, csz, mpole, local, keys, start, shift, ntot, mstride); break;
	default: return c->fail(NBCO_ERR_UNSUPPORTED, "launch_m2l_lanes: order not generated");
	}
	NBCO_HIP(hipGetLastError());
	return NBCO_OK;
}

}

int launch_m2l_lanes(nbco_ctx *c, int P, const float4 *csz, const float *mpole, float *local, const uint64_t *keys, const int *start,
                     int shift, int ntot, int mstride)
{
	return dispatch<float>(c, P, csz, mpole, local, keys, start, shift, ntot, mstride);
}
int launch_m2l_lanes_f64(nbco_ctx *c, int P, const float4 *csz, const double *mpole, double *local, const uint64_t *keys, const int *start,
                         int shift, int ntot, int mstride)
{
	return dispatch<double>(c, P, csz, mpole, local, keys, start, shift, ntot, mstride);
}
```

coulomb_oscillators_amd/csrc/kd_traverse_kernels.hpp:

```cpp

__device__ inline uint64_t block_exclusive_scan3(uint64_t v, uint64_t *sh_wave, uint64_t &total)
{
	const int lane = threadIdx.x & 63, w = threadIdx.x >> 6;
	const uint64_t incl = (uint64_t)wave_scan_add((uint32_t)(v & 0xFFFFFu)) | ((uint64_t)wave_scan_add((uint32_t)((v >> 20) & 0xFFFFFu)) << 20) |
	                      ((uint64_t)wave_scan_add((uint32_t)(v >> 40)) << 40);
	if (lane == 63) sh_wave[w] = incl;
	__syncthreads();
	uint64_t base = 0, tot = 0;
	for (int k = 0; k < 4; ++k)
	{
		uint64_t s = sh_wave[k];
		if (k < w) base += s;
		tot += s;
	}
	total = tot;
	return base + incl - v;
}

__device__ inline int classify_pair(const TreeView &t, const AdmTab *tab, int2 np, float par, int m2l_first, const Dom dm)
{
	const int ntot = t.ntot;
	if (dm.d > 0 && !dom_touch(dm, np.x) && !dom_touch(dm, np.y)) return 0;
	const bool leaf1 = 2 * np.x + 1 >= ntot, leaf2 = 2 * np.y + 1 >= ntot;
	if (!m2l_first && leaf1 && leaf2) return (np.x != np.y) ? 1 : 0;
	if (np.x == np.y) return leaf1 ? 0 : 3;
	const float4 c1 = t.csz[np.x], c2 = t.csz[np.y];
	if (kd_admissible(c1, c2, np.x, np.y, t.mult, tab, par)) return 2;
	if (leaf1 && leaf2) return 1;
	return (leaf1 || (!leaf2 && c1.w <= c2.w)) ? 4 : 5;
}

struct NodeRec { float4 c; int m; };
#pragma clang fp contract(off)
__device__ inline bool kd_admissible_rec(const NodeRec a, const NodeRec b, int n1, int n2, const AdmTab *tabp, float par)
{
	float dx = b.c.x - a.c.x, dy = b.c.y - a.c.y, dz = b.c.z - a.c.z;
	float dist2 = dx * dx + dy * dy + dz * dz;
	int nb = a.m >= b.m ? n1 : n2, mb = a.m >= b.m ? a.m : b.m;
	int lev = 31 - __clz(nb + 1);
	float M = (mb == tabp->lo[lev]) ? tabp->Mlo[lev] : tabp->Mhi[lev];
	float parM = par * M;
	float sz = fmaxf(a.c.w, b.c.w);
	return parM * parM * sz < dist2;
}
#pragma clang fp contract(fast)
__device__ inline int classify_rec(int ntot, const AdmTab *tab, int2 np, const NodeRec a, const NodeRec b, float par, int m2l_first, const Dom dm)
{
	if (dm.d > 0 && !dom_touch(dm, np.x) && !dom_touch(dm, np.y)) return 0;
	const bool leaf1 = 2 * np.x + 1 >= ntot, leaf2 = 2 * np.y + 1 >= ntot;
	if (!m2l_first && leaf1 && leaf2) return (np.x != np.y) ? 1 : 0;
	if (np.x == np.y) return leaf1 ? 0 : 3;
	if (kd_admissible_rec(a, b, np.x, np.y, tab, par)) return 2;
	if (leaf1 && leaf2) return 1;
	return (leaf1 || (!leaf2 && a.c.w <= b.c.w)) ? 4 : 5;
}

struct PairKids
{
	int2 a, b, c;
	int n;
};
__device__ inline PairKids pair_children(int kd, int2 np)
{
	const int x1 = 2 * np.x + 1, x2 = 2 * np.x + 2, y1 = 2 * np.y + 1, y2 = 2 * np.y + 2;
	PairKids k;
	k.a.x = kd == 4 ? np.x : x1;
	k.a.y = kd == 5 ? np.y : (kd == 4 ? y1 : x1);
	k.b.x = kd == 4 ? np.x : (kd == 5 ? x2 : x1);
	k.b.y = kd == 5 ? np.y : (kd == 4 ? y2 : x2);
	k.c.x = x2;
	k.c.y = x2;
	k.n = kd == 3 ? 3 : (kd >= 4 ? 2 : 0);
	return k;
}

constexpr int kTravK = 16;
constexpr int kTcFrontier = 0;
constexpr int kTcP2P = 36 * kTravK;
constexpr int kTcM2L = kTcP2P + kTravK;
constexpr int kTcP2PPref = kTcM2L + kTravK;
constexpr int kTcM2LPref = kTcP2PPref + kTravK + 1;
constexpr int kTcInts = kTcM2LPref + kTravK + 1;
#ifndef NBCO_TRAV_EXTRA
#define NBCO_TRAV_EXTRA 1
#endif

__device__ inline long long region_slot(const int *__restrict__ pref, long long capR, long long i)
{
	int r = 0;
#pragma unroll
	for (int q = 1; q < kTravK; ++q) r += (i >= pref[q]) ? 1 : 0;
	return (long long)r * capR + (i - pref[r]);
}

__global__ __launch_bounds__(kBlock) void traverse_kernel(TreeView t, AdmTab tab_arg, const int2 *__restrict__ fin, int2 *__restrict__ fout,
                                                          int2 *__restrict__ p2p, int2 *__restrict__ m2l, int2 *__restrict__ p2p_rank,
                                                          int2 *__restrict__ m2l_rank, int *__restrict__ counters,
                                                          int *__restrict__ tctr, int it, long long capR, float par, int m2l_first,
                                                          unsigned *__restrict__ cnt_p2p, unsigned *__restrict__ cnt_m2l, const Dom dm)
{
	__shared__ uint64_t sh_wave[4];
	__shared__ int sh_base[3];
	__shared__ int in_pref[kTravK + 1];
	__shared__ AdmTab tab;
#ifdef NBCO_SUBTREE_PROF
	bool first_pass;
#endif
	TRAV_FIRST_PASS(true);
	TRAV_MARK(0);
	for (int q = threadIdx.x; q < (int)(sizeof(AdmTab) / sizeof(int)); q += kBlock) reinterpret_cast<int *>(&tab)[q] = reinterpret_cast<const int *>(&tab_arg)[q];
	if (threadIdx.x < 64)
	{
		const int lane = threadIdx.x;
		const int v = lane < kTravK ? (int)min((long long)tctr[kTcFrontier + it * kTravK + lane], capR) : 0, incl = (int)wave_scan_add((uint32_t)v);
		if (lane < kTravK) in_pref[lane] = incl - v;
		if (lane == kTravK - 1) in_pref[kTravK] = incl;
	}
	__syncthreads();
	TRAV_MARK(1);
	const int nin = in_pref[kTravK];
	const int lbeg = kd_beg(t.L);
	const int rout = (blockIdx.x + 5 * it) & (kTravK - 1);
	const long long obase = (long long)rout * capR;
	for (long long base = (long long)blockIdx.x * kBlock; base < nin; base += (long long)gridDim.x * kBlock)
	{
		const long long i = base + threadIdx.x;
		int2 p0 = make_int2(0, 0);
		int k0 = 0, k1 = 0, k2 = 0, k3 = 0;
		PairKids ch;
		ch.a = ch.b = ch.c = make_int2(0, 0);
		ch.n = 0;
		if (i < nin)
		{
			p0 = fin[region_slot(in_pref, capR, i)];
			if (!NBCO_CHECKED_OK((unsigned)p0.x < (unsigned)t.ntot && (unsigned)p0.y < (unsigned)t.ntot, NBCO_CHK_FRONTIER)) p0 = make_int2(0, 0);
			TRAV_DEP(p0.x);
			TRAV_MARK(2);
			const int last = t.ntot - 1;
			const int ix1 = min(2 * p0.x + 1, last), ix2 = min(2 * p0.x + 2, last), iy1 = min(2 * p0.y + 1, last), iy2 = min(2 * p0.y + 2, last);
			const NodeRec X{t.csz[p0.x], t.mult[p0.x]}, Y{t.csz[p0.y], t.mult[p0.y]};
			const NodeRec X1{t.csz[ix1], t.mult[ix1]}, X2{t.csz[ix2], t.mult[ix2]}, Y1{t.csz[iy1], t.mult[iy1]}, Y2{t.csz[iy2], t.mult[iy2]};
			TRAV_DEP(Y2.m); TRAV_DEP(X.c.x); TRAV_DEP(Y.c.x); TRAV_DEP(X1.c.x); TRAV_DEP(X2.c.x); TRAV_DEP(Y1.c.x); TRAV_DEP(Y2.c.x);
			TRAV_MARK(3);
			k0 = classify_rec(t.ntot, &tab, p0, X, Y, par, m2l_first, dm);
			ch = pair_children(k0, p0);
			const NodeRec A1 = k0 == 4 ? X : X1, A2 = k0 == 5 ? Y : (k0 == 4 ? Y1 : X1);
			const NodeRec B1 = k0 == 4 ? X : (k0 == 5 ? X2 : X1), B2 = k0 == 5 ? Y : (k0 == 4 ? Y2 : X2);
			if (ch.n > 0) k1 = classify_rec(t.ntot, &tab, ch.a, A1, A2, par, m2l_first, dm);
			if (ch.n > 1) k2 = classify_rec(t.ntot, &tab, ch.b, B1, B2, par, m2l_first, dm);
			if (ch.n > 2) k3 = classify_rec(t.ntot, &tab, ch.c, X2, X2, par, m2l_first, dm);
		}
		const int nch = ch.n;
		TRAV_DEP(k0 + k1 + k2 + k3);
		TRAV_MARK(4);
		auto weight = [](int q) { return (uint64_t)(q == 3 ? 3 : (q >= 4 ? 2 : 0)) | ((uint64_t)(q == 1) << 20) | ((uint64_t)(q == 2) << 40); };
		const uint64_t cnt = nch > 0 ? weight(k1) + weight(k2) + weight(k3) : weight(k0);
		uint64_t tot;
		const uint64_t off = block_exclusive_scan3(cnt, sh_wave, tot);
		const int tf = (int)(tot & 0xFFFFF), tp = (int)((tot >> 20) & 0xFFFFF), tm = (int)(tot >> 40);
		TRAV_MARK(5);
		if (threadIdx.x == 0) sh_base[0] = tf ? atomicAdd(&tctr[kTcFrontier + (it + 1) * kTravK + rout], tf) : 0;
		if (threadIdx.x == 64) sh_base[1] = tp ? atomicAdd(&tctr[kTcP2P + rout], tp) : 0;
		if (threadIdx.x == 128) sh_base[2] = tm ? atomicAdd(&tctr[kTcM2L + rout], tm) : 0;
		const int lane = threadIdx.x & 63;
		const int m2l_at = (int)(cnt_m2l - cnt_p2p);
		struct Req { int from, place; unsigned pend; };
		auto request = [&](int key, bool on) {
			Req r{lane, 0, 0u};
			const uint64_t todo = __ballot(on);
			int size = 1;
			if (todo)
			{
				const int first = __builtin_amdgcn_readfirstlane(__ffsll((unsigned long long)todo) - 1);
				const int v = __builtin_amdgcn_readlane(key, first);
				const uint64_t same = __ballot(on && key == v);
				if (on && key == v) { r.from = first; r.place = __popcll(same & ((1ull << lane) - 1ull)); size = __popcll(same); }
			}
			if (on && r.from == lane) r.pend = atomicAdd(&cnt_p2p[key], (unsigned)size);
			return r;
		};
		auto slots = [&](int q, int2 np, bool ok, Req &rx, Req &ry) {
			const bool lst = ok && (q == 1 || q == 2);
			const int kx = q == 1 ? np.x - lbeg : m2l_at + np.x, ky = q == 1 ? np.y - lbeg : m2l_at + np.y;
			rx = request(kx, lst && (dm.d == 0 || dom_touch(dm, np.x)));
			ry = request(ky, lst && (dm.d == 0 || dom_touch(dm, np.y)));
			return make_int2(lst && (dm.d == 0 || dom_touch(dm, np.x)) ? 0 : -1, lst && (dm.d == 0 || dom_touch(dm, np.y)) ? 0 : -1);
		};
		Req q0x, q0y, q1x, q1y, q2x, q2y, q3x, q3y;
		int2 r0 = slots(k0, p0, nch == 0 && i < nin, q0x, q0y), r1 = slots(k1, ch.a, nch > 0, q1x, q1y), r2 = slots(k2, ch.b, nch > 1, q2x, q2y),
		     r3 = slots(k3, ch.c, nch > 2, q3x, q3y);
		asm volatile("s_waitcnt lgkmcnt(0)\n\ts_barrier" ::: "memory");
		TRAV_MARK(7);
		long long bf = sh_base[0], bp = sh_base[1], bm = sh_base[2];
		const bool okf = bf + tf <= capR, okp = bp + tp <= capR, okm = bm + tm <= capR;
		if (threadIdx.x == 0 && !(okf && okp && okm)) counters[2] = 1;
		if (!okf && bf < capR)
			for (long long k = bf + threadIdx.x; k < capR; k += kBlock) fout[obase + k] = make_int2(0, 0);
		bf += (long long)(off & 0xFFFFF); bp += (long long)((off >> 20) & 0xFFFFF); bm += (long long)(off >> 40);
		auto emit = [&](int q, int2 np) {
			long long at = -1;
			if (q == 1 && okp) { p2p[obase + bp] = np; at = obase + bp; }
			if (q == 2 && okm) { m2l[obase + bm] = np; at = obase + bm; }
			const PairKids g = pair_children(q, np);
			if (q >= 3 && okf)
			{
				fout[obase + bf] = g.a;
				fout[obase + bf + 1] = g.b;
				if (g.n > 2) fout[obase + bf + 2] = g.c;
			}
			bp += q == 1 ? 1 : 0;
			bm += q == 2 ? 1 : 0;
			bf += g.n;
			return at;
		};
		long long at0 = -1, at1 = -1, at2 = -1, at3 = -1;
		if (nch == 0) at0 = emit(k0, p0);
		else
		{
			at1 = emit(k1, ch.a);
			at2 = emit(k2, ch.b);
			if (nch > 2) at3 = emit(k3, ch.c);
		}
		auto settle = [&](const Req &rq, int &slot) {
			const int base = __shfl((int)rq.pend, rq.from);
			if (slot >= 0) slot = base + rq.place;
		};
		settle(q0x, r0.x); settle(q0y, r0.y); settle(q1x, r1.x); settle(q1y, r1.y);
		settle(q2x, r2.x); settle(q2y, r2.y); settle(q3x, r3.x); settle(q3y, r3.y);
		TRAV_DEP(r0.x + r1.x + r2.x + r3.x + r0.y + r1.y + r2.y + r3.y);
		TRAV_MARK(6);
		auto put_slots = [&](int q, long long at, int2 r) {
			if (at < 0) return;
			if (q == 1) p2p_rank[at] = r; else m2l_rank[at] = r;
		};
		put_slots(k0, at0, r0); put_slots(k1, at1, r1); put_slots(k2, at2, r2); put_slots(k3, at3, r3);
		TRAV_MARK(8);
		TRAV_DRAIN();
		TRAV_MARK(9);
		__syncthreads();
		TRAV_MARK(10);
		TRAV_FIRST_PASS(false);
	}
	TRAV_MARK(11);
}

__global__ __launch_bounds__(kBlock) void traverse_init_kernel(int2 *frontier, int *counters, int nctr, int *tctr, unsigned *__restrict__ list_cnt,
                                                               long long words, long long self0, long long nself)
{
	for (long long i = (long long)blockIdx.x * kBlock + threadIdx.x; i < words; i += (long long)gridDim.x * kBlock)
		list_cnt[i] = (i >= self0 && i < self0 + nself) ? 1u : 0u;
	if (blockIdx.x != 0) return;
	for (int i = threadIdx.x; i < nctr; i += kBlock) counters[i] = 0;
	for (int i = threadIdx.x; i < kTcInts; i += kBlock) tctr[i] = 0;
	__syncthreads();
	if (threadIdx.x == 0) { frontier[0] = make_int2(0, 0); tctr[kTcFrontier] = 1; }
}

__global__ __launch_bounds__(1024) void traverse_finish_kernel(int *counters, int *tctr, long long capR, unsigned *cnt_all, long long ncnt,
                                                               unsigned *cnt_self, int nself, int *__restrict__ host_flags, int iters, int seq)
{
	const int lane = threadIdx.x;
	const bool overflow = counters[2] != 0;
	if (overflow)
	{
		for (long long i = threadIdx.x; i < ncnt; i += blockDim.x) cnt_all[i] = 0u;
		__syncthreads();
		for (int i = threadIdx.x; i < nself; i += blockDim.x) cnt_self[i] = 1u;
	}
	if (lane >= 64) return;
	for (int which = 0; which < 2; ++which)
	{
		const int src = which ? kTcM2L : kTcP2P, dst = which ? kTcM2LPref : kTcP2PPref;
		int v = (lane < kTravK && !overflow) ? tctr[src + lane] : 0, incl = v;
		for (int o = 1; o < kTravK; o <<= 1) { const int y = __shfl_up(incl, o); if (lane >= o) incl += y; }
		if (lane < kTravK) tctr[dst + lane] = incl - v;
		if (lane == kTravK - 1) { tctr[dst + kTravK] = incl; counters[which] = incl; host_flags[which] = incl; }
	}
	int left = lane < kTravK ? tctr[kTcFrontier + iters * kTravK + lane] : 0;
	for (int o = 32; o > 0; o >>= 1) left += __shfl_xor(left, o);
	if (lane == 0) { host_flags[2] = overflow ? 1 : (left != 0 ? 2 : 0); host_flags[3] = counters[110]; }
	__threadfence_system();
	if (lane == 0) __hip_atomic_store(&host_flags[4], seq, __ATOMIC_RELEASE, __HIP_MEMORY_SCOPE_SYSTEM);
}

__global__ __launch_bounds__(kBlock) void list_compact_kernel(const int2 *__restrict__ src, const int *__restrict__ pref, long long capR,
                                                              int2 *__restrict__ dst)
{
	const long long n = pref[kTravK];
	for (long long i = (long long)blockIdx.x * kBlock + threadIdx.x; i < n; i += (long long)gridDim.x * kBlock) dst[i] = src[region_slot(pref, capR, i)];
}
```

coulomb_oscillators_amd/csrc/nbco_api.hip:

```cpp
#include "nbco_internal.hpp"
#include <chrono>
#include <cstdio>
#include <cmath>
#include <new>
#include <random>

int nbco_ctx::reserve(DevBuf &b, size_t bytes)
{
	nbco_ctx *c = this;
	if (bytes <= b.bytes) return NBCO_OK;
	if (b.ptr)
	{
		NBCO_HIP(hipStreamSynchronize(stream));
		NBCO_HIP(hipFree(b.ptr));
		b.ptr = nullptr;
		b.bytes = 0;
	}
	size_t want = bytes + bytes / 8 + 256;
	NBCO_HIP(hipMalloc(&b.ptr, want));
	b.bytes = want;
	if (poison) NBCO_HIP(hipMemsetAsync(b.ptr, 0x7f, want, stream));
	return NBCO_OK;
}

void nbco_ctx::phase_begin(int ph)
{
	if (!(profiling & (1u << ph))) return;
	hipEvent_t a, b;
	if (hipEventCreate(&a) != hipSuccess || hipEventCreate(&b) != hipSuccess) return;
	hipEventRecord(a, stream);
	timers[ph].pending.push_back({a, b});
}

void nbco_ctx::phase_end(int ph)
{
	if (!(profiling & (1u << ph)) || timers[ph].pending.empty()) return;
	hipEventRecord(timers[ph].pending.back().second, stream);
}

int nbco_ctx::fork_mark()
{
	if (!aux && !aux_is_main)
	{
		int prio_lo = 0, prio_hi = 0;
		NBCO_HIP_M(this, hipDeviceGetStreamPriorityRange(&prio_lo, &prio_hi));
		if (getenv("NBCO_AUX_PRIO") && atoi(getenv("NBCO_AUX_PRIO")) == 0) prio_hi = prio_lo;
		if (getenv("NBCO_AUX_SERIAL") && atoi(getenv("NBCO_AUX_SERIAL")) != 0) { aux = stream; aux_is_main = true; }
		else NBCO_HIP_M(this, hipStreamCreateWithPriority(&aux, hipStreamNonBlocking, prio_hi));
		NBCO_HIP_M(this, hipEventCreateWithFlags(&ev_fork, hipEventDisableTiming));
		NBCO_HIP_M(this, hipEventCreateWithFlags(&ev_join, hipEventDisableTiming));
	}
	NBCO_HIP_M(this, hipEventRecord(ev_fork, stream));
	return NBCO_OK;
}

int nbco_ctx::fork_wait()
{
	NBCO_HIP_M(this, hipStreamWaitEvent(aux, ev_fork, 0));
	aux_pending = true;
	return NBCO_OK;
}

int nbco_ctx::fork_aux()
{
	NBCO_TRY(fork_mark());
	return fork_wait();
}

int nbco_ctx::flags_begin()
{
	if (!h_flags)
	{
		NBCO_HIP_M(this, hipHostMalloc((void **)&h_flags, 64 * sizeof(int), hipHostMallocDefault));
		memset(h_flags, 0, 64 * sizeof(int));
		NBCO_HIP_M(this, hipEventCreateWithFlags(&ev_flags, hipEventDisableTiming));
	}
	return NBCO_OK;
}

int nbco_ctx::wait_flags()
{
	nbco_ctx *c = this;
	volatile int *seq = h_flags + 4;
	for (unsigned spin = 1;; ++spin)
	{
		if (__atomic_load_n(seq, __ATOMIC_ACQUIRE) == flags_seq) return NBCO_OK;
		if ((spin & 0x3FFu) == 0)
		{
			const hipError_t e = hipEventQuery(ev_flags);
			if (e == hipSuccess) { if (__atomic_load_n(seq, __ATOMIC_ACQUIRE) == flags_seq) return NBCO_OK; NBCO_HIP(hipEventSynchronize(ev_flags)); return NBCO_OK; }
			if (e != hipErrorNotReady) return fail_hip(e, "hipEventQuery(ev_flags)", __FILE__, __LINE__);
		}
#if defined(__x86_64__)
		__builtin_ia32_pause();
#endif
	}
}

int nbco_ctx::join_aux()
{
	if (!aux_pending) return NBCO_OK;
	NBCO_HIP_M(this, hipEventRecord(ev_join, aux));
	NBCO_HIP_M(this, hipStreamWaitEvent(stream, ev_join, 0));
	aux_pending = false;
	return NBCO_OK;
}

static int check_opts(nbco_ctx *c, const nbco_opts *o)
{
	if (o->fmm_order < 1 || o->fmm_order > kMaxOrder) return c->fail(NBCO_ERR_ARG, "fmm_order must be in 1..10");
	if (!(o->tree_radius > 0)) return c->fail(NBCO_ERR_ARG, "tree_radius must be positive");
	if (!(o->eps2 > 0)) return c->fail(NBCO_ERR_ARG, "eps2 must be positive");
	if (!(o->dens_inhom > 0)) return c->fail(NBCO_ERR_ARG, "dens_inhom must be positive");
	if (o->tree_L < 0 || o->tree_L > 30) return c->fail(NBCO_ERR_ARG, "tree_L must be in 0..30");
	if (o->tree_steps < 1) return c->fail(NBCO_ERR_ARG, "tree_steps must be >= 1");
	if (o->list_factor < 1) return c->fail(NBCO_ERR_ARG, "list_factor must be >= 1");
	return NBCO_OK;
}

template <class Run>
static int closing_kick(nbco_ctx *c, KdStepLink &link, Run run, float *buf, long long n, const float *param, float ds, bool elastic)
{
	float *x = buf, *v = buf + 3 * n, *a = buf + 6 * n;
	link.defer_v_copy = true;
	link.v_now = nullptr;
	const int rc = run();
	const float *v_in = link.v_now ? link.v_now : v;
	if (rc != NBCO_OK)
	{
		if (v_in != v) hipMemcpyAsync(v, v_in, sizeof(float) * 3 * (size_t)n, hipMemcpyDeviceToDevice, c->stream);
		return rc;
	}
	PhaseScope ph(c, NBCO_PH_AXPY);
	return launch_finish_kick(c, x, v_in, v, a, param, ds, n, elastic);
}

extern "C" {

int nbco_opts_default(nbco_opts *o)
{
	if (!o) return NBCO_ERR_ARG;
	o->fmm_order = 3;
	o->tree_radius = 1.f;
	o->eps2 = 1.e-18f;
	o->coll = 1;
	o->unsort = 1;
	o->dens_inhom = 1.f;
	o->tree_L = 0;
	o->tree_steps = 1;
	o->m2l_first = 0;
	o->sync = 1;
	o->list_factor = 48;
	o->list_grow = 1;
	o->far_fp64 = 0;
	o->p2p_mutual = 0;
	o->track_order = 0;
	o->stream = nullptr;
	return NBCO_OK;
}

int nbco_create(nbco_ctx **out, const nbco_opts *o)
{
	if (!out) return NBCO_ERR_ARG;
	*out = nullptr;
	nbco_ctx *c = new (std::nothrow) nbco_ctx();
	if (!c) return NBCO_ERR_HIP;
	nbco_opts def;
	nbco_opts_default(&def);
	c->o = o ? *o : def;
	int rc = check_opts(c, &c->o);
	if (rc != NBCO_OK) { delete c; return rc; }
	int ndev = 0;
	hipError_t e = hipGetDeviceCount(&ndev);
	if (e != hipSuccess || ndev <= 0)
	{
		fprintf(stderr, "nbco_create: no usable HIP device (%s)\n", e != hipSuccess ? hipGetErrorString(e) : "device count is 0");
		delete c;
		return NBCO_ERR_HIP;
	}
	if (hipGetDevice(&c->device) != hipSuccess) { delete c; return NBCO_ERR_HIP; }
	hipDeviceProp_t prop;
	if (hipGetDeviceProperties(&prop, c->device) == hipSuccess) c->num_cu = prop.multiProcessorCount;
	c->stream = (hipStream_t)c->o.stream;
	c->poison = getenv("NBCO_POISON") && atoi(getenv("NBCO_POISON")) != 0;
	if (getenv("NBCO_SEL_WARM")) c->sel_warm_enabled = atoi(getenv("NBCO_SEL_WARM")) != 0;
	if (hipMalloc(&c->small.ptr, 4096) != hipSuccess) { delete c; return NBCO_ERR_HIP; }
	c->small.bytes = 4096;
	*out = c;
	return NBCO_OK;
}

int nbco_destroy(nbco_ctx *c)
{
	if (c && getenv("NBCO_HOST_TIMING") && c->host_calls)
		fprintf(stderr, "[nbco] nbco_integrate: %lld calls, %.1f us host time per call, of which %.1f us waiting for the traversal flags\n", c->host_calls,
		        1e6 * c->host_call_s / c->host_calls, 1e6 * c->host_wait_s / c->host_calls);
	if (!c) return NBCO_OK;
	hipStreamSynchronize(c->stream);
	if (c->aux && !c->aux_is_main) { hipStreamSynchronize(c->aux); hipStreamDestroy(c->aux); }
	if (c->ev_fork) hipEventDestroy(c->ev_fork);
	if (c->ev_join) hipEventDestroy(c->ev_join);
	if (c->ev_flags) hipEventDestroy(c->ev_flags);
	if (c->h_flags) hipHostFree(c->h_flags);
	for (auto &t : c->timers)
		for (auto &ev : t.pending) { hipEventDestroy(ev.first); hipEventDestroy(ev.second); }
	delete c;
	return NBCO_OK;
}

int nbco_set_opts(nbco_ctx *c, const nbco_opts *o)
{
	if (!c || !o) return NBCO_ERR_ARG;
	NBCO_TRY(check_opts(c, o));
	if ((hipStream_t)o->stream != c->stream) NBCO_HIP(hipStreamSynchronize(c->stream));
	if (o->list_factor != c->o.list_factor) c->list_growth = 1;
	bool topo = o->fmm_order != c->o.fmm_order || o->dens_inhom != c->o.dens_inhom || o->tree_L != c->o.tree_L
	            || o->unsort != c->o.unsort || o->p2p_mutual != c->o.p2p_mutual || o->track_order != c->o.track_order
	            || o->tree_steps != c->o.tree_steps;
	c->o = *o;
	c->stream = (hipStream_t)o->stream;
	if (topo) { c->tree_valid = false; c->eval_counter = 0; }
	if (!o->track_order) c->order_n = -1;
	return NBCO_OK;
}

int nbco_get_opts(const nbco_ctx *c, nbco_opts *o)
{
	if (!c || !o) return NBCO_ERR_ARG;
	*o = c->o;
	return NBCO_OK;
}

const char *nbco_last_error(const nbco_ctx *c) { return c ? c->err.c_str() : "null context"; }

int nbco_sync(nbco_ctx *c)
{
	if (!c) return NBCO_ERR_ARG;
	NBCO_HIP(hipStreamSynchronize(c->stream));
	return NBCO_OK;
}

static int maybe_sync(nbco_ctx *c)
{
	if (c->o.sync) NBCO_HIP(hipStreamSynchronize(c->stream));
	return NBCO_OK;
}

int nbco_step(nbco_ctx *c, float *b, const float *a, float ds, long long n)
{
	if (!c || !b || !a || n < 0) return c ? c->fail(NBCO_ERR_ARG, "nbco_step: bad arguments") : NBCO_ERR_ARG;
	PhaseScope ph(c, NBCO_PH_AXPY);
	return launch_step(c, b, a, ds, 3 * n);
}
int nbco_add_elastic(nbco_ctx *c, const float *p, float *a, long long n, const float *k)
{
	if (!c || !p || !a || n < 0) return c ? c->fail(NBCO_ERR_ARG, "nbco_add_elastic: bad arguments") : NBCO_ERR_ARG;
	PhaseScope ph(c, NBCO_PH_AXPY);
	return launch_add_elastic(c, p, a, n, k, false);
}
int nbco_elastic(nbco_ctx *c, const float *p, float *a, long long n, const float *k)
{
	if (!c || !p || !a || n < 0) return c ? c->fail(NBCO_ERR_ARG, "nbco_elastic: bad arguments") : NBCO_ERR_ARG;
	PhaseScope ph(c, NBCO_PH_AXPY);
	return launch_add_elastic(c, p, a, n, k, true);
}
int nbco_rescale(nbco_ctx *c, float *a, long long n, const float *param)
{
	if (!c || !a || !param || n < 0) return c ? c->fail(NBCO_ERR_ARG, "nbco_rescale: bad arguments") : NBCO_ERR_ARG;
	PhaseScope ph(c, NBCO_PH_AXPY);
	return launch_rescale(c, a, 3 * n, param);
}
int nbco_gather(nbco_ctx *c, float *dst, const float *src, const int *map, long long n)
{
	if (!c || !dst || !src || !map || n < 0) return c ? c->fail(NBCO_ERR_ARG, "nbco_gather: bad arguments") : NBCO_ERR_ARG;
	return launch_gather3(c, dst, src, map, n, false);
}
int nbco_gather_inverse(nbco_ctx *c, float *dst, const float *src, const int *map, long long n)
{
	if (!c || !dst || !src || !map || n < 0) return c ? c->fail(NBCO_ERR_ARG, "nbco_gather_inverse: bad arguments") : NBCO_ERR_ARG;
	return launch_gather3(c, dst, src, map, n, true);
}
int nbco_copy(nbco_ctx *c, float *dst, const float *src, long long n)
{
	if (!c || !dst || !src || n < 0) return c ? c->fail(NBCO_ERR_ARG, "nbco_copy: bad arguments") : NBCO_ERR_ARG;
	return launch_copy(c, dst, src, 3 * n);
}

int nbco_direct(nbco_ctx *c, const float *p, float *a, long long n, const float *param)
{
	if (!c || !p || !a) return c ? c->fail(NBCO_ERR_ARG, "nbco_direct: null pointer") : NBCO_ERR_ARG;
	NBCO_TRY(launch_direct(c, p, a, n, param, false));
	return maybe_sync(c);
}
int nbco_direct3(nbco_ctx *c, const float *p, float *a, long long n, const float *param)
{
	if (!c || !p || !a) return c ? c->fail(NBCO_ERR_ARG, "nbco_direct3: null pointer") : NBCO_ERR_ARG;
	NBCO_TRY(launch_direct(c, p, a, n, param, true));
	return maybe_sync(c);
}
int nbco_fmm_kdtree(nbco_ctx *c, float *p, float *a, long long n, const float *param)
{
	if (!c || !p || !a) return c ? c->fail(NBCO_ERR_ARG, "nbco_fmm_kdtree: null pointer") : NBCO_ERR_ARG;
	NBCO_TRY(fmm_kdtree_eval(c, p, a, n, param));
	return maybe_sync(c);
}
int nbco_fmm_traceless(nbco_ctx *c, float *p, float *a, long long n, const float *param)
{
	if (!c || !p || !a) return c ? c->fail(NBCO_ERR_ARG, "nbco_fmm_traceless: null pointer") : NBCO_ERR_ARG;
	NBCO_TRY(fmm_oct_traceless_eval(c, p, a, n, param));
	return maybe_sync(c);
}
int nbco_fmm_symmetric(nbco_ctx *c, float *p, float *a, long long n, const float *param)
{
	if (!c || !p || !a) return c ? c->fail(NBCO_ERR_ARG, "nbco_fmm_symmetric: null pointer") : NBCO_ERR_ARG;
	NBCO_TRY(fmm_oct_traceless_eval(c, p, a, n, param, true));
	return maybe_sync(c);
}
int nbco_oct_get_info(nbco_ctx *c, nbco_oct_info *out)
{
	if (!c || !out) return c ? c->fail(NBCO_ERR_ARG, "nbco_oct_get_info: null pointer") : NBCO_ERR_ARG;
	if (!c->oct.valid) return c->fail(NBCO_ERR_ARG, "nbco_oct_get_info: no octree evaluation has run");
	const OctTreeDev &o = c->oct;
	out->L = o.L; out->ntot = o.ntot; out->order = o.order; out->tpl = o.tpl; out->n = o.n;
	out->m2l_entries = o.m2l_entries; out->p2p_groups = o.p2p_groups; out->p2p_desc = o.p2p_desc; out->p2p_chunks = o.p2p_chunks;
	out->real_bytes = o.real_bytes;
	out->mpole_reals = o.mpole_reals;
	return NBCO_OK;
}
int nbco_oct_copy(nbco_ctx *c, int which, void *host_dst, long long host_bytes)
{
	if (!c || !host_dst) return c ? c->fail(NBCO_ERR_ARG, "nbco_oct_copy: null pointer") : NBCO_ERR_ARG;
	return oct_copy_out(c, which, host_dst, host_bytes);
}

int nbco_dist_layout_query(nbco_ctx *c, long long n_global, int world, int rank, nbco_dist_layout *out)
{
	if (!c || !out) return c ? c->fail(NBCO_ERR_ARG, "nbco_dist_layout_query: null pointer") : NBCO_ERR_ARG;
	return kd_dist_layout(c, n_global, world, rank, out);
}
int nbco_dist_partition(nbco_ctx *c, const float *state_all, long long n_global, int world, int rank, float *state_local)
{
	if (!c || !state_all || !state_local) return c ? c->fail(NBCO_ERR_ARG, "nbco_dist_partition: null pointer") : NBCO_ERR_ARG;
	NBCO_TRY(kd_dist_partition(c, state_all, n_global, world, rank, state_local));
	return maybe_sync(c);
}
int nbco_dist_local(nbco_ctx *c, float *buf_local, long long n_local, void *nodes_send, void *pos_send)
{
	if (!c || !buf_local || !nodes_send || !pos_send) return c ? c->fail(NBCO_ERR_ARG, "nbco_dist_local: null pointer") : NBCO_ERR_ARG;
	NBCO_TRY(kd_dist_local_build(c, buf_local, n_local, pos_send, nullptr, false));
	NBCO_TRY(kd_dist_local_upward(c, n_local, nodes_send, nullptr, false));
	return maybe_sync(c);
}
int nbco_dist_local_build(nbco_ctx *c, float *buf_local, long long n_local, void *pos_send)
{
	if (!c || !buf_local || !pos_send) return c ? c->fail(NBCO_ERR_ARG, "nbco_dist_local_build: null pointer") : NBCO_ERR_ARG;
	NBCO_TRY(kd_dist_local_build(c, buf_local, n_local, pos_send, nullptr, false));
	return maybe_sync(c);
}
int nbco_dist_local_upward(nbco_ctx *c, float *buf_local, long long n_local, void *nodes_send)
{
	if (!c || !buf_local || !nodes_send) return c ? c->fail(NBCO_ERR_ARG, "nbco_dist_local_upward: null pointer") : NBCO_ERR_ARG;
	NBCO_TRY(kd_dist_local_upward(c, n_local, nodes_send, nullptr, false));
	return maybe_sync(c);
}
int nbco_dist_local_geom(nbco_ctx *c, float *buf_local, long long n_local, void *pos_send, void *csz_send)
{
	if (!c || !buf_local || !pos_send || !csz_send) return c ? c->fail(NBCO_ERR_ARG, "nbco_dist_local_geom: null pointer") : NBCO_ERR_ARG;
	NBCO_TRY(kd_dist_local_build(c, buf_local, n_local, pos_send, csz_send, false));
	return maybe_sync(c);
}
int nbco_dist_local_mpole(nbco_ctx *c, float *buf_local, long long n_local, void *mpole_send)
{
	if (!c || !buf_local || !mpole_send) return c ? c->fail(NBCO_ERR_ARG, "nbco_dist_local_mpole: null pointer") : NBCO_ERR_ARG;
	NBCO_TRY(kd_dist_local_upward(c, n_local, nullptr, mpole_send, false));
	return maybe_sync(c);
}
int nbco_dist_let_local_geom(nbco_ctx *c, float *buf_local, long long n_local, void *csz_send)
{
	if (!c || !buf_local || !csz_send) return c ? c->fail(NBCO_ERR_ARG, "nbco_dist_let_local_geom: null pointer") : NBCO_ERR_ARG;
	NBCO_TRY(kd_dist_local_build(c, buf_local, n_local, nullptr, csz_send, true));
	return maybe_sync(c);
}
int nbco_dist_let_local_mpole(nbco_ctx *c, float *buf_local, long long n_local)
{
	if (!c || !buf_local) return c ? c->fail(NBCO_ERR_ARG, "nbco_dist_let_local_mpole: null pointer") : NBCO_ERR_ARG;
	return kd_dist_local_upward(c, n_local, nullptr, nullptr, true);
}
int nbco_dist_let_select(nbco_ctx *c, const void *csz_all, long long *counts_send)
{
	if (!c || !csz_all || !counts_send) return c ? c->fail(NBCO_ERR_ARG, "nbco_dist_let_select: null pointer") : NBCO_ERR_ARG;
	return kd_dist_let_select(c, csz_all, counts_send);
}
int nbco_dist_let_pack(nbco_ctx *c, const long long *counts_all, void *pos_send, void *mpole_send)
{
	if (!c || !counts_all) return c ? c->fail(NBCO_ERR_ARG, "nbco_dist_let_pack: null pointer") : NBCO_ERR_ARG;
	return kd_dist_let_pack(c, counts_all, pos_send, mpole_send);
}
int nbco_dist_let_finish(nbco_ctx *c, const long long *counts_all, const void *pos_recv, const void *mpole_recv, float *buf_local, float *a_local,
                         const float *param)
{
	if (!c || !counts_all || !buf_local || !a_local) return c ? c->fail(NBCO_ERR_ARG, "nbco_dist_let_finish: null pointer") : NBCO_ERR_ARG;
	NBCO_TRY(kd_dist_let_finish(c, counts_all, pos_recv, mpole_recv, buf_local, a_local, param));
	return maybe_sync(c);
}
int nbco_dist_turnaround(nbco_ctx *c, float *buf_local, long long n_local, const float *param, double dt_, double scale_, int elastic)
{
	if (!c || !buf_local || !param) return c ? c->fail(NBCO_ERR_ARG, "nbco_dist_turnaround: null pointer") : NBCO_ERR_ARG;
	const long double dt = dt_, scale = scale_;
	return kd_dist_turnaround(c, buf_local, n_local, param, (float)(dt * scale * 0.5L), (float)dt, elastic != 0);
}
int nbco_dist_let_check(nbco_ctx *c)
{
	if (!c) return NBCO_ERR_ARG;
	return kd_dist_let_check(c);
}
int nbco_dist_let_pack_capped(nbco_ctx *c, const long long *caps_out, void *pos_send, void *mpole_send)
{
	if (!c || !caps_out) return c ? c->fail(NBCO_ERR_ARG, "nbco_dist_let_pack_capped: null pointer") : NBCO_ERR_ARG;
	return kd_dist_let_pack_capped(c, caps_out, pos_send, mpole_send);
}
int nbco_dist_let_finish_capped(nbco_ctx *c, const long long *caps_in, const void *pos_recv, const void *mpole_recv, float *buf_local, float *a_local,
                                const float *param)
{
	if (!c || !caps_in || !buf_local || !a_local) return c ? c->fail(NBCO_ERR_ARG, "nbco_dist_let_finish_capped: null pointer") : NBCO_ERR_ARG;
	NBCO_TRY(kd_dist_let_finish_capped(c, caps_in, pos_recv, mpole_recv, buf_local, a_local, param));
	return maybe_sync(c);
}
int nbco_dist_let_settle(nbco_ctx *c, int ok)
{
	if (!c) return NBCO_ERR_ARG;
	return kd_dist_let_settle(c, ok);
}
int nbco_dist_repartition_workspace(nbco_ctx *c, long long n_global, int world, long long *bytes)
{
	if (!c || !bytes) return c ? c->fail(NBCO_ERR_ARG, "nbco_dist_repartition_workspace: null pointer") : NBCO_ERR_ARG;
	return dpart_workspace(c, n_global, world, bytes);
}
int nbco_dist_repartition_begin(nbco_ctx *c, float *state_local, long long n_global, int world, int rank, void *work, long long work_bytes, nbco_dist_step *next)
{
	if (!c || !state_local || !work || !next) return c ? c->fail(NBCO_ERR_ARG, "nbco_dist_repartition_begin: null pointer") : NBCO_ERR_ARG;
	return dpart_begin(c, state_local, n_global, world, rank, work, work_bytes, next);
}
int nbco_dist_repartition_next(nbco_ctx *c, nbco_dist_step *next)
{
	if (!c || !next) return c ? c->fail(NBCO_ERR_ARG, "nbco_dist_repartition_next: null pointer") : NBCO_ERR_ARG;
	return dpart_next(c, next);
}
int nbco_dist_finish_traverse(nbco_ctx *c, const void *csz_all, const void *pos_all)
{
	if (!c || !csz_all || !pos_all) return c ? c->fail(NBCO_ERR_ARG, "nbco_dist_finish_traverse: null pointer") : NBCO_ERR_ARG;
	return kd_dist_finish_traverse(c, csz_all, pos_all);
}
int nbco_dist_finish_rest(nbco_ctx *c, const void *mpole_all, float *buf_local, float *a_local, const float *param)
{
	if (!c || !mpole_all || !buf_local || !a_local) return c ? c->fail(NBCO_ERR_ARG, "nbco_dist_finish_rest: null pointer") : NBCO_ERR_ARG;
	NBCO_TRY(kd_dist_finish_rest(c, mpole_all, buf_local, a_local, param));
	return maybe_sync(c);
}
int nbco_aux_stream(nbco_ctx *c, void **stream_out)
{
	if (!c || !stream_out) return c ? c->fail(NBCO_ERR_ARG, "nbco_aux_stream: null pointer") : NBCO_ERR_ARG;
	NBCO_TRY(c->fork_mark());
	*stream_out = (void *)c->aux;
	return NBCO_OK;
}
int nbco_dist_finish(nbco_ctx *c, const void *nodes_all, const void *pos_all, float *buf_local, float *a_local, const float *param)
{
	if (!c || !nodes_all || !pos_all || !buf_local || !a_local) return c ? c->fail(NBCO_ERR_ARG, "nbco_dist_finish: null pointer") : NBCO_ERR_ARG;
	NBCO_TRY(kd_dist_finish(c, nodes_all, pos_all, buf_local, a_local, param));
	return maybe_sync(c);
}

static int eval_kind(nbco_ctx *c, int kind, float *p, float *a, long long n, const float *param, KdStepLink *link = nullptr)
{
	switch (kind)
	{
	case NBCO_EVAL_DIRECT: return launch_direct(c, p, a, n, param, false);
	case NBCO_EVAL_DIRECT_KAHAN: return launch_direct(c, p, a, n, param, true);
	case NBCO_EVAL_FMM_KDTREE: return fmm_kdtree_eval(c, p, a, n, param, link);
	case NBCO_EVAL_FMM_TRACELESS: return fmm_oct_traceless_eval(c, p, a, n, param, false);
	case NBCO_EVAL_FMM_SYMMETRIC: return fmm_oct_traceless_eval(c, p, a, n, param, true);
	default: return c->fail(NBCO_ERR_ARG, "unknown evaluator kind");
	}
}

int nbco_fmm_oct_shard(nbco_ctx *c, float *p, float *a, long long n, const float *param, int symmetric, int world, int rank, long long *bounds_host)
{
	if (!c || !p || !a || !bounds_host) return c ? c->fail(NBCO_ERR_ARG, "nbco_fmm_oct_shard: null pointer") : NBCO_ERR_ARG;
	NBCO_TRY(fmm_oct_traceless_eval(c, p, a, n, param, symmetric != 0, world, rank, bounds_host));
	return maybe_sync(c);
}

int nbco_force(nbco_ctx *c, int kind, float *buf, long long n, const float *param, int elastic)
{
	if (!c || !buf || !param || n <= 0) return c ? c->fail(NBCO_ERR_ARG, "nbco_force: bad arguments") : NBCO_ERR_ARG;
	float *x = buf, *a = buf + 6 * n;
	NBCO_TRY(eval_kind(c, kind, x, a, n, param));
	if (elastic)
	{
		PhaseScope ph(c, NBCO_PH_AXPY);
		NBCO_TRY(launch_add_elastic(c, x, a, n, param + 3, false));
	}
// ... 343 lines not shown
```

coulomb_oscillators_amd/csrc/nbco_internal.hpp:

```cpp
#pragma once
#include <hip/hip_runtime.h>
#include <cstdint>
#include <cstdio>
#include <cstring>
#include <string>
#include <utility>
#include <vector>
#include "../../include/nbco.h"

#define NBCO_HIP(call)                                                                           \
	do {                                                                                         \
		hipError_t e_ = (call);                                                                  \
		if (e_ != hipSuccess) return c->fail_hip(e_, #call, __FILE__, __LINE__);                 \
	} while (0)

#define NBCO_HIP_M(ctx_, call)                                                                   \
	do {                                                                                         \
		hipError_t e_ = (call);                                                                  \
		if (e_ != hipSuccess) return (ctx_)->fail_hip(e_, #call, __FILE__, __LINE__);            \
	} while (0)

#define NBCO_TRY(call)                   \
	do {                                 \
		int rc_ = (call);                \
		if (rc_ != NBCO_OK) return rc_;  \
	} while (0)

enum
{
	NBCO_CHK_FRONTIER = 0,
	NBCO_CHK_FILL = 1,
	NBCO_CHK_SORT = 2,
	NBCO_CHK_CHUNK = 3,
	NBCO_CHK_DESC = 4,
	NBCO_CHK_L2P = 5,
	NBCO_CHK_SITES = 8
};
#ifdef NBCO_CHECKED
namespace { __device__ unsigned nbco_violation_count[NBCO_CHK_SITES]; }
#define NBCO_CHECKED_OK(cond, site) ((cond) ? true : (atomicAdd(&nbco_violation_count[site], 1u), false))
#define NBCO_CHECKED_COLLECT(fn)                                                                                      \
	int fn(unsigned *out)                                                                                             \
	{                                                                                                                 \
		unsigned v[NBCO_CHK_SITES];                                                                                   \
		if (hipMemcpyFromSymbol(v, HIP_SYMBOL(nbco_violation_count), sizeof v) != hipSuccess) return NBCO_ERR_HIP;    \
		for (int i = 0; i < NBCO_CHK_SITES; ++i) out[i] += v[i];                                                      \
		return NBCO_OK;                                                                                               \
	}
#else
#define NBCO_CHECKED_OK(cond, site) (true)
#define NBCO_CHECKED_COLLECT(fn) int fn(unsigned *) { return NBCO_OK; }
#endif
int nbco_checked_collect_kd(unsigned *out);
int nbco_checked_collect_oct(unsigned *out);
int nbco_checked_collect_far(unsigned *out);

struct DevBuf
{
	void *ptr = nullptr;
	size_t bytes = 0;
	DevBuf() = default;
	DevBuf(DevBuf &&o) noexcept : ptr(o.ptr), bytes(o.bytes) { o.ptr = nullptr; o.bytes = 0; }
	DevBuf &operator=(DevBuf &&o) noexcept { std::swap(ptr, o.ptr); std::swap(bytes, o.bytes); return *this; }
	~DevBuf() { if (ptr) hipFree(ptr); }
	template <class T> T *as() const { return (T *)ptr; }
};

struct PhaseTimer
{
	std::vector<std::pair<hipEvent_t, hipEvent_t>> pending;
	double total_ms = 0;
	long long launches = 0;
};

constexpr int kMaxOrder = 10;

struct KdTreeDev
{
	int L = 0, ntot = 0, order = 0, mlt_max = 0;
	long long n = 0;
	float *center = nullptr, *lbound = nullptr, *rbound = nullptr;
	float4 *csz = nullptr;
	float *mpole = nullptr, *local = nullptr;
	int *mult = nullptr, *index = nullptr, *splitdim = nullptr;
	int real_bytes = 4;
};

struct OctTreeDev
{
	bool valid = false;
	int L = 0, ntot = 0, order = 0, tpl = 0;
	long long n = 0, m2l_entries = 0, p2p_groups = 0, p2p_desc = 0, p2p_chunks = 0;
	float4 *csz = nullptr;
	void *mpole = nullptr, *local = nullptr;
	int real_bytes = 4;
	int mpole_reals = 0;
	int *mult = nullptr, *index = nullptr;
	uint32_t *keys = nullptr, *perm = nullptr;
};

struct KdStepLink
{
	bool defer_order = false, defer_v_copy = false;
	int prep_done = 0;
	bool order_pending = false;
	const float *v_now = nullptr;
};

struct KdRoot { const float *root6 = nullptr; const int *top_sd = nullptr; int top_root1 = 1; };

struct nbco_ctx
{
	nbco_opts o;
	hipStream_t stream = nullptr;
	hipStream_t aux = nullptr;
	hipEvent_t ev_fork = nullptr, ev_join = nullptr;
	bool aux_pending = false;
	int list_growth = 1;
	bool grow_lists(int ntot)
	{
		if (!o.list_grow || list_growth >= 64) return false;
		if (8LL * list_growth * o.list_factor * (long long)ntot + 16384 + ntot >= (1LL << 31)) return false;
		list_growth *= 2;
		return true;
	}
	long long perm_primed_n = -1;
	double host_wait_s = 0, host_call_s = 0;
	long long host_calls = 0;
	bool aux_is_main = false;
	bool poison = false;
	int *h_flags = nullptr;
	hipEvent_t ev_flags = nullptr;
	long long hint_np2p = 0, hint_nm2l = 0;
	int flags_begin();
	int flags_seq = 0;
	int wait_flags();
	DevBuf scan_tmp_aux;
	int fork_aux();
	int fork_mark();
	int fork_wait();
	int join_aux();
	std::string err;
	int device = 0;
	int num_cu = 256;

	DevBuf pos4;
	DevBuf pos4_alt;
	DevBuf part;
	DevBuf small;
	DevBuf tmp3, tmp3b;
	DevBuf keys, keys_alt, idx, idx_alt, unsort, unsort_alt, sort_tmp;
	DevBuf treebuf;
	KdTreeDev kd;
	DevBuf frontier_a, frontier_b, p2p_list, m2l_list, counters;
	DevBuf p2p_keys, p2p_keys_alt, m2l_keys, m2l_keys_alt, p2p_start, m2l_start;
	DevBuf p2p_chunk_off, p2p_chunks, p2p_desc;
	DevBuf order, order_alt;
	long long order_n = -1;
	DevBuf p2p_sec, p2p_react;
	const int *pc_mult = nullptr, *pc_total = nullptr;
	int pc_shift = 0;
	DevBuf list_cnt, trav_ctr;
	DevBuf prep_state;
	DevBuf sel_hist, sel_nodes, sel_ties;
	DevBuf dist_top, dist_tree;
	DevBuf let_sel, let_have, dist_pos;
	DevBuf oct_tree, oct_groups;
	DevBuf f2d_tree, f2d_keys, f2d_tmp, f2d_part;
	OctTreeDev oct;
	struct DistState
	{
		int world = 0, rank = 0, d = 0, L = 0;
		long long n_global = 0, n_local = 0;
		bool partitioned = false, build_done = false, local_done = false, rebuilt = false, traversed = false, let_selected = false, let_packed = false;
		const void *pos_all = nullptr;
		bool let_capped = false, let_flagged = false;
		long long let_epoch = 0;
		bool let_ignore[2] = {false, false};
		int prep_done = 0;
	} dist;
	bool sel_warm_enabled = true, sel_warm_used = false;
	int sel_warm_coarsen = 0, sel_warm_good = 0, sel_warm_recent = 0, sel_warm_recent_miss = 0, sel_warm_cooldown = 0, sel_warm_cool_len = 128;
	long long sel_warm_builds = 0, sel_warm_misses = 0;
	void note_warm_miss()
	{
		++sel_warm_misses;
		sel_warm_good = 0;
		if (sel_warm_coarsen < 3) ++sel_warm_coarsen;
		if (++sel_warm_recent_miss >= 2)
		{
			sel_warm_cooldown = sel_warm_cool_len;
			sel_warm_cool_len = sel_warm_cool_len < 2048 ? 2 * sel_warm_cool_len : 4096;
			sel_warm_recent = sel_warm_recent_miss = 0;
		}
	}
	void note_warm_ok()
	{
		if (++sel_warm_recent >= 32) sel_warm_recent = sel_warm_recent_miss = 0;
		if (++sel_warm_good >= 64)
		{
			if (sel_warm_coarsen > 0) --sel_warm_coarsen;
			sel_warm_cool_len = sel_warm_cool_len > 256 ? sel_warm_cool_len / 2 : 128;
			sel_warm_good = 0;
		}
	}
	bool sel_three_pass = false;
	bool force_sort_build = false;
	bool escalate_build()
	{
		if (!sel_three_pass) { sel_three_pass = true; return true; }
		if (!force_sort_build) { force_sort_build = true; return true; }
		return false;
	}
	bool demote_build()
	{
		tree_valid = false;
		if (sel_warm_used) note_warm_miss();
		return sel_warm_used || escalate_build();
	}
	long long list_cap = 0;
	struct DPart
	{
		int stage = 0, level = 0, pass = 0, world = 0, rank = 0, d = 0;
		long long n_global = 0, n_local = 0;
		float *state = nullptr;
		void *work = nullptr;
		size_t tie_bytes = 0;
		bool seg_flip = false, pos_flip = false;
		long long rows_send[64] = {}, rows_recv[64] = {};
	} dpart;
	DevBuf dpart_buf;
	struct LastEval
	{
		bool valid = false, have_p2p = false;
		const float *center = nullptr, *mpole = nullptr;
		const float4 *csz = nullptr, *pos = nullptr;
		const int *mult = nullptr, *index = nullptr;
		int L = 0, ntot = 0, order = 0, shift = 0, real_bytes = 4;
		long long n = 0, own0 = 0, own_n = 0;
	} last_eval;
	nbco_kd_info info{};
	long long eval_counter = 0;
	bool tree_valid = false;
	long long tree_n = 0;
	int tree_order = 0;
	unsigned profiling = 0;
	PhaseTimer timers[NBCO_PH_COUNT];

	int fail(int code, const std::string &msg) { err = msg; return code; }
	int fail_hip(hipError_t e, const char *what, const char *file, int line)
	{
		char buf[512];
		snprintf(buf, sizeof buf, "HIP error: %s (%s) at %s:%d", hipGetErrorString(e), what, file, line);
		err = buf;
		return NBCO_ERR_HIP;
	}
	int reserve(DevBuf &b, size_t bytes);
	void phase_begin(int ph);
	void phase_end(int ph);
};

struct StreamScope
{
	nbco_ctx *c;
	hipStream_t saved;
	StreamScope(nbco_ctx *c_, hipStream_t s) : c(c_), saved(c_->stream) { c->stream = s; }
	~StreamScope() { c->stream = saved; }
};

struct PhaseScope
{
	nbco_ctx *c;
	int ph;
	PhaseScope(nbco_ctx *c_, int ph_) : c(c_), ph(ph_) { c->phase_begin(ph); }
	~PhaseScope() { c->phase_end(ph); }
};

static inline int ceil_div(long long a, long long b) { return (int)((a + b - 1) / b); }

int launch_step(nbco_ctx *c, float *b, const float *a, float ds, long long n3);
int launch_add_elastic(nbco_ctx *c, const float *p, float *a, long long n, const float *k, bool assign);
int launch_rescale(nbco_ctx *c, float *a, long long n3, const float *param);
int launch_gather3(nbco_ctx *c, float *dst, const float *src, const int *map, long long n, bool inverse);
int launch_copy(nbco_ctx *c, float *dst, const float *src, long long n3);
int launch_pack4(nbco_ctx *c, float4 *dst, const float *src3, long long n);
int launch_kick_drift(nbco_ctx *c, float *x, float *v, const float *a, float ks, float ds, long long n3);
int launch_finish_kick(nbco_ctx *c, const float *x, const float *v_in, float *v, float *a, const float *param, float ks, long long n, bool elastic);
int launch_direct(nbco_ctx *c, const float *p, float *a, long long n, const float *param, bool kahan);
int launch_minmax(nbco_ctx *c, const float *p3, long long n, float *out6_dev);
int launch_minmax4(nbco_ctx *c, const float4 *p4, long long n, float *out6_dev);
int launch_mean_relerr(nbco_ctx *c, const float *x, const float *ref, long long n, float *out_host);
int launch_pow_sum(nbco_ctx *c, const float *x, int expo, long long n, double *out3_host);
int launch_energy(nbco_ctx *c, const float *buf, long long n, const float *param, double *out3_host);
int fmm_kdtree_eval(nbco_ctx *c, float *p, float *a, long long n, const float *param, KdStepLink *link = nullptr);
int kd_copy_out(nbco_ctx *c, int which, void *host_dst, long long host_bytes);
int kd_count_pairs(nbco_ctx *c, long long *out);
int kd_energy_fmm(nbco_ctx *c, long long n_own, double *half_phi_sum);
int launch_energy_kin_ela(nbco_ctx *c, const float *buf, long long n, const float *param, double *out2_host);
int fmm_oct_traceless_eval(nbco_ctx *c, float *p, float *a, long long n, const float *param, bool symmetric = false, int world = 1, int rank = 0,
                           long long *pbounds_host = nullptr);
int oct_copy_out(nbco_ctx *c, int which, void *host_dst, long long host_bytes);
int kd_dist_layout(nbco_ctx *c, long long n_global, int world, int rank, nbco_dist_layout *out);
int kd_dist_partition(nbco_ctx *c, const float *state_all, long long n_global, int world, int rank, float *state_local);
int dpart_workspace(nbco_ctx *c, long long n_global, int world, long long *bytes);
int dpart_begin(nbco_ctx *c, float *state_local, long long n_global, int world, int rank, void *work, long long work_bytes, nbco_dist_step *out);
int dpart_next(nbco_ctx *c, nbco_dist_step *out);
int kd_finish_pending_order(nbco_ctx *c, float *p, long long n, KdStepLink *link);
int kd_turnaround(nbco_ctx *c, float *p, const float *param, float ks, float ds, bool elastic, long long n, KdStepLink *link, const float *root6 = nullptr);
int kd_dist_turnaround(nbco_ctx *c, float *buf_local, long long n_local, const float *param, float ks, float ds, bool elastic);
int kd_dist_let_select(nbco_ctx *c, const void *csz_all, long long *counts);
int kd_dist_let_pack(nbco_ctx *c, const long long *counts_all, void *pos_send, void *mpole_send);
int kd_dist_let_finish(nbco_ctx *c, const long long *counts_all, const void *pos_recv, const void *mpole_recv, float *buf_local, float *a_local, const float *param);
int kd_dist_let_check(nbco_ctx *c);
int kd_dist_let_pack_capped(nbco_ctx *c, const long long *caps_out, void *pos_send, void *mpole_send);
int kd_dist_let_finish_capped(nbco_ctx *c, const long long *caps_in, const void *pos_recv, const void *mpole_recv, float *buf_local, float *a_local, const float *param);
int kd_dist_let_settle(nbco_ctx *c, int ok);
int kd_dist_local_build(nbco_ctx *c, float *buf_local, long long n_local, void *pos_send, void *csz_send, bool let);
int kd_dist_local_upward(nbco_ctx *c, long long n_local, void *nodes_send, void *mpole_send, bool let);
int kd_dist_finish(nbco_ctx *c, const void *nodes_all, const void *pos_all, float *buf_local, float *a_local, const float *param);
int kd_dist_finish_traverse(nbco_ctx *c, const void *csz_all, const void *pos_all);
int kd_dist_finish_rest(nbco_ctx *c, const void *mpole_all, float *buf_local, float *a_local, const float *param);
int kd_select_begin(nbco_ctx *c, int l0, bool zero = true, long long *words_a = nullptr, long long *words_b = nullptr);
int kd_select_level(nbco_ctx *c, int l, long long n, const float4 *pos_in, const int *unsort_in, float4 *pos_out, int *unsort_out,
                    float *lbound, float *rbound, int *splitdim, int *index, int *flag, bool warm = false, const KdRoot &root = KdRoot{});
int launch_upward_gen(nbco_ctx *c, int P, const float4 *pos, float *center, void *mpole, int *mult, const int *index, int L, int write_geom, int f64 = 0);
int launch_kd_centres(nbco_ctx *c, float *center, int *mult, int L, const float *lbound, const float *rbound, float4 *csz);
int launch_downward_gen(nbco_ctx *c, int P, const float *center, void *local, int L, int dom_d, int dom_g, int f64 = 0);
int launch_m2m_top_gen(nbco_ctx *c, int P, float *center, void *mpole, int *mult, int ltop, int L, int write_geom, int f64 = 0);
int launch_kd_centres_top(nbco_ctx *c, float *center, int *mult, int ltop, const float *lbound, const float *rbound, float4 *csz);
int launch_l2p_gen(nbco_ctx *c, int P, const float4 *pos, const float *center, const void *local, const float4 *near, const int *chunk_off,
                   const int *index, int mlt_max, const int *unsort, int scatter, const float *param, float *a, int have_near, long long n, int L,
                   long long own0, long long own_n, const int2 *sec_range = nullptr, const float4 *react = nullptr, long long react_cap = 0,
                   int react_stride = 32, int f64 = 0);
int launch_m2l_lanes(nbco_ctx *c, int P, const float4 *csz, const float *mpole, float *local, const uint64_t *keys, const int *start,
                     int shift, int ntot, int mstride = 0);
int launch_m2l_lanes_f64(nbco_ctx *c, int P, const float4 *csz, const double *mpole, double *local, const uint64_t *keys, const int *start,
                         int shift, int ntot, int mstride = 0);
```

coulomb_oscillators_amd/engine.py:

```python
import ctypes as C
import os
import subprocess

_HERE = os.path.dirname(os.path.abspath(__file__))
_LIB = os.environ.get("NBCO_LIB") or os.path.join(_HERE, "libnbco_hip.so")

EVAL_DIRECT, EVAL_DIRECT_KAHAN, EVAL_FMM_KDTREE, EVAL_FMM_TRACELESS, EVAL_FMM_SYMMETRIC = 0, 1, 2, 3, 4
INTEG_EULER, INTEG_PRE_EULER, INTEG_LEAPFROG, INTEG_FORESTRUTH, INTEG_PEFRL = 0, 1, 2, 3, 4
EVAL2D_DIRECT, EVAL2D_DIRECT_KAHAN, EVAL2D_FMM = 0, 1, 2
REF_SEED, REF_DISCARD = 5351550349027530206, 1248
PHASES = ["build", "p2m_m2m", "traverse", "lists", "p2p", "m2l", "l2l", "l2p", "finish", "direct", "axpy"]

KD_FIELDS = {"mult": 0, "index": 1, "splitdim": 2, "center": 3, "lbound": 4, "rbound": 5,
             "mpole": 6, "local": 7, "p2p": 8, "m2l": 9, "unsort": 10, "order": 11}


class EngineError(RuntimeError):

    def __init__(self, msg, status=None):
        super().__init__(msg)
        self.status = status


ERR_UNSUPPORTED = 4


class Opts(C.Structure):
    _fields_ = [("fmm_order", C.c_int), ("tree_radius", C.c_float), ("eps2", C.c_float), ("coll", C.c_int),
                ("unsort", C.c_int), ("dens_inhom", C.c_float), ("tree_L", C.c_int), ("tree_steps", C.c_int),
                ("m2l_first", C.c_int), ("sync", C.c_int), ("list_factor", C.c_int), ("list_grow", C.c_int), ("far_fp64", C.c_int),
                ("p2p_mutual", C.c_int), ("track_order", C.c_int), ("stream", C.c_void_p)]


class KdInfo(C.Structure):
    _fields_ = [("L", C.c_int), ("ntot", C.c_int), ("order", C.c_int), ("mlt_max", C.c_int), ("n", C.c_longlong),
                ("p2p_pairs", C.c_longlong), ("m2l_pairs", C.c_longlong), ("directed_p2p", C.c_longlong),
                ("rebuilt", C.c_int), ("build_mode", C.c_int), ("p2p_halves", C.c_int), ("warm_builds", C.c_longlong), ("warm_misses", C.c_longlong),
                ("real_bytes", C.c_int), ("long_lists", C.c_int)]


class OctInfo(C.Structure):
    _fields_ = [("L", C.c_int), ("ntot", C.c_int), ("order", C.c_int), ("tpl", C.c_int), ("n", C.c_longlong),
                ("m2l_entries", C.c_longlong), ("p2p_groups", C.c_longlong), ("p2p_desc", C.c_longlong),
                ("p2p_chunks", C.c_longlong), ("real_bytes", C.c_int), ("mpole_reals", C.c_int)]


OCT_FIELDS = {"mult": 0, "index": 1, "center4": 2, "mpole": 3, "local": 4, "keys": 5, "perm": 6}


class DistLayout(C.Structure):
    _fields_ = [("world", C.c_int), ("rank", C.c_int), ("d", C.c_int), ("L", C.c_int), ("L_local", C.c_int),
                ("ntot_local", C.c_int), ("order", C.c_int), ("n_global", C.c_longlong), ("n_local", C.c_longlong),
                ("nodes_bytes", C.c_longlong), ("pos_bytes", C.c_longlong), ("csz_bytes", C.c_longlong),
                ("mpole_bytes", C.c_longlong), ("let_node_bytes", C.c_longlong), ("let_counts", C.c_int)]


class DistStep(C.Structure):
    _fields_ = [("op", C.c_int), ("row_bytes", C.c_int), ("send_off", C.c_longlong), ("recv_off", C.c_longlong), ("count", C.c_longlong),
                ("rows_send", C.c_longlong * 64), ("rows_recv", C.c_longlong * 64)]


COLL_DONE, COLL_ALLREDUCE_MIN_I32, COLL_ALLREDUCE_SUM_I32, COLL_ALLGATHER, COLL_ALLTOALL = range(5)


def lib_path():
    return _LIB


def build_library(force=False):
    csrc = os.path.join(_HERE, "csrc")
    cmd = ["make", "-C", csrc, "-s", "-j8"]
    if force:
        cmd.append("-B")
    subprocess.check_call(cmd)
    return _LIB


_lib = None


def _load():
    global _lib
    if _lib is not None:
        return _lib
    if not os.path.exists(_LIB):
        raise EngineError("libnbco_hip.so is not built (run `python -c 'import __graft_entry__ as g; g.build()'`); "
                          "there is no CPU fallback")
    L = C.CDLL(_LIB)
    P, LL, I, F, D = C.c_void_p, C.c_longlong, C.c_int, C.c_float, C.c_double
    sig = {
        "nbco_opts_default": [C.POINTER(Opts)],
        "nbco_create": [C.POINTER(P), C.POINTER(Opts)],
        "nbco_destroy": [P],
        "nbco_set_opts": [P, C.POINTER(Opts)],
        "nbco_get_opts": [P, C.POINTER(Opts)],
        "nbco_sync": [P],
        "nbco_step": [P, P, P, F, LL],
        "nbco_add_elastic": [P, P, P, LL, P],
        "nbco_elastic": [P, P, P, LL, P],
        "nbco_rescale": [P, P, LL, P],
        "nbco_gather": [P, P, P, P, LL],
        "nbco_gather_inverse": [P, P, P, P, LL],
        "nbco_copy": [P, P, P, LL],
        "nbco_direct": [P, P, P, LL, P],
        "nbco_direct3": [P, P, P, LL, P],
        "nbco_fmm_kdtree": [P, P, P, LL, P],
        "nbco_fmm_traceless": [P, P, P, LL, P],
        "nbco_fmm_symmetric": [P, P, P, LL, P],
        "nbco_fmm_oct_shard": [P, P, P, LL, P, I, I, I, C.POINTER(LL)],
        "nbco_force": [P, I, P, LL, P, I],
        "nbco_integrate": [P, I, I, P, LL, P, D, D, I],
        "nbco_integrate_steps": [P, I, I, P, LL, P, D, D, I, I],
        "nbco_minmax": [P, P, LL, P],
        "nbco_mean_relerr": [P, P, P, LL, C.POINTER(F)],
        "nbco_pow_sum": [P, P, I, LL, C.POINTER(D)],
        "nbco_energy": [P, P, LL, P, C.POINTER(D)],
        "nbco_energy_fmm": [P, P, LL, P, C.POINTER(D)],
        "nbco_kd_get_info": [P, C.POINTER(KdInfo)],
        "nbco_kd_copy": [P, I, P, LL],
        "nbco_oct_get_info": [P, C.POINTER(OctInfo)],
        "nbco_oct_copy": [P, I, P, LL],
        "nbco_dist_layout_query": [P, LL, I, I, C.POINTER(DistLayout)],
        "nbco_dist_partition": [P, P, LL, I, I, P],
        "nbco_dist_local": [P, P, LL, P, P],
        "nbco_dist_local_build": [P, P, LL, P],
        "nbco_dist_local_upward": [P, P, LL, P],
        "nbco_dist_finish": [P, P, P, P, P, P],
        "nbco_dist_local_geom": [P, P, LL, P, P],
        "nbco_dist_local_mpole": [P, P, LL, P],
        "nbco_dist_finish_traverse": [P, P, P],
        "nbco_dist_finish_rest": [P, P, P, P, P],
        "nbco_dist_repartition_workspace": [P, LL, I, C.POINTER(LL)],
        "nbco_dist_repartition_begin": [P, P, LL, I, I, P, LL, C.POINTER(DistStep)],
        "nbco_dist_repartition_next": [P, C.POINTER(DistStep)],
        "nbco_dist_let_local_geom": [P, P, LL, P],
        "nbco_dist_let_local_mpole": [P, P, LL],
        "nbco_dist_let_select": [P, P, P],
        "nbco_dist_let_pack": [P, P, P, P],
        "nbco_dist_let_finish": [P, P, P, P, P, P, P],
        "nbco_dist_let_check": [P],
        "nbco_dist_let_pack_capped": [P, P, P, P],
        "nbco_dist_let_finish_capped": [P, P, P, P, P, P, P],
        "nbco_dist_let_settle": [P, I],
        "nbco_dist_turnaround": [P, P, LL, P, D, D, I],
        "nbco_aux_stream": [P, C.POINTER(C.c_void_p)],
        "nbco_debug_violations": [P, C.POINTER(LL)],
        "nbco_profile_enable": [P, I],
        "nbco_profile_reset": [P],
        "nbco_profile_get": [P, I, C.POINTER(D), C.POINTER(LL)],
        "nbco_2d_direct": [P, P, P, LL, P],
        "nbco_2d_direct3": [P, P, P, LL, P],
        "nbco_2d_fmm": [P, P, P, LL, P],
        "nbco_2d_force": [P, I, P, LL, P, I],
        "nbco_2d_integrate": [P, I, I, P, LL, P, D, D, I],
        "nbco_2d_integrate_steps": [P, I, I, P, LL, P, D, D, I, I],
        "nbco_2d_mean_relerr": [P, P, P, LL, C.POINTER(D)],
        "nbco_2d_energy": [P, P, LL, P, C.POINTER(D), P],
        "nbco_2d_energy_fmm": [P, P, LL, P, C.POINTER(D), P],
        "nbco_2d_init_kv": [P, LL, P, P, C.c_ulonglong, C.c_ulonglong],
        "nbco_2d_init_gaussian": [P, LL, P, P, C.c_ulonglong, C.c_ulonglong],
    }
    for name, args in sig.items():
        fn = getattr(L, name)
        fn.argtypes = args
        fn.restype = I
    L.nbco_last_error.argtypes = [P]
    L.nbco_last_error.restype = C.c_char_p
    _lib = L
    return L


def init2d(n, kind="kv", a=None, b=None, seed=REF_SEED, discard=REF_DISCARD):
    import numpy as np
    out = np.zeros((2, n, 2), dtype=np.float64)
    a2 = (C.c_double * 2)(*a)
    b2 = (C.c_double * 2)(*b)
    fn = _load().nbco_2d_init_kv if kind == "kv" else _load().nbco_2d_init_gaussian
    rc = fn(out.ctypes.data_as(C.c_void_p), n, C.cast(a2, C.c_void_p), C.cast(b2, C.c_void_p), seed, discard)
    if rc != 0:
        raise EngineError("nbco_2d_init_%s failed with status %d" % (kind, rc), status=rc)
    return out


def default_opts(**kw):
    o = Opts()
    _load().nbco_opts_default(C.byref(o))
    for k, v in kw.items():
        setattr(o, k, v)
    return o


def _ptr(t):
    return C.c_void_p(t.data_ptr()) if t is not None else None


class Engine:

    def __init__(self, stream=None, **opts):
        import torch
        self.lib = _load()
        if not torch.cuda.is_available():
            raise EngineError("no HIP device visible to PyTorch; the engine has no CPU fallback")
        self.torch = torch
        if stream is None:
            stream = torch.cuda.current_stream().cuda_stream
        o = default_opts(**opts)
        o.stream = stream
        self.ctx = C.c_void_p()
        rc = self.lib.nbco_create(C.byref(self.ctx), C.byref(o))
        if rc != 0:
            raise EngineError("nbco_create failed with status %d" % rc)

    def close(self):
        if getattr(self, "ctx", None):
            self.lib.nbco_destroy(self.ctx)
            self.ctx = None

    def __del__(self):
        try:
            self.close()
        except Exception:
            pass

    def _chk(self, rc):
        if rc != 0:
            raise EngineError("nbco status %d: %s" % (rc, self.lib.nbco_last_error(self.ctx).decode()), status=rc)

    def opts(self):
        o = Opts()
        self._chk(self.lib.nbco_get_opts(self.ctx, C.byref(o)))
        return o

    def set(self, **kw):
        o = self.opts()
        for k, v in kw.items():
            setattr(o, k, v)
        self._chk(self.lib.nbco_set_opts(self.ctx, C.byref(o)))

    def sync(self):
        self._chk(self.lib.nbco_sync(self.ctx))

    def step(self, b, a, ds, n=None):
        n = b.numel() // 3 if n is None else n
        self._chk(self.lib.nbco_step(self.ctx, _ptr(b), _ptr(a), ds, n))

    def add_elastic(self, p, a, n, k=None):
        self._chk(self.lib.nbco_add_elastic(self.ctx, _ptr(p), _ptr(a), n, _ptr(k)))

    def elastic(self, p, a, n, k=None):
        self._chk(self.lib.nbco_elastic(self.ctx, _ptr(p), _ptr(a), n, _ptr(k)))

    def rescale(self, a, n, param):
        self._chk(self.lib.nbco_rescale(self.ctx, _ptr(a), n, _ptr(param)))

    def gather(self, dst, src, idx, n):
        self._chk(self.lib.nbco_gather(self.ctx, _ptr(dst), _ptr(src), _ptr(idx), n))

    def gather_inverse(self, dst, src, idx, n):
        self._chk(self.lib.nbco_gather_inverse(self.ctx, _ptr(dst), _ptr(src), _ptr(idx), n))

    def copy(self, dst, src, n):
        self._chk(self.lib.nbco_copy(self.ctx, _ptr(dst), _ptr(src), n))

    def direct(self, p, a, n, param=None):
        self._chk(self.lib.nbco_direct(self.ctx, _ptr(p), _ptr(a), n, _ptr(param)))

    def direct3(self, p, a, n, param=None):
        self._chk(self.lib.nbco_direct3(self.ctx, _ptr(p), _ptr(a), n, _ptr(param)))

    def fmm_cart3_kdtree(self, p, a, n, param=None):
        self._chk(self.lib.nbco_fmm_kdtree(self.ctx, _ptr(p), _ptr(a), n, _ptr(param)))

    def fmm_cart3_traceless(self, p, a, n, param=None):
        self._chk(self.lib.nbco_fmm_traceless(self.ctx, _ptr(p), _ptr(a), n, _ptr(param)))

    def fmm_cart3(self, p, a, n, param=None):
        self._chk(self.lib.nbco_fmm_symmetric(self.ctx, _ptr(p), _ptr(a), n, _ptr(param)))

    def fmm_oct_shard(self, p, a, n, param, world, rank, symmetric=False):
        b = (C.c_longlong * (world + 1))()
        self._chk(self.lib.nbco_fmm_oct_shard(self.ctx, _ptr(p), _ptr(a), n, _ptr(param), int(symmetric), world, rank, b))
        return list(b)

    def compute_force(self, kind, buf, n, param, elastic=True):
        self._chk(self.lib.nbco_force(self.ctx, kind, _ptr(buf), n, _ptr(param), int(elastic)))

    def integrate(self, scheme, kind, buf, n, param, dt, scale=1.0, elastic=True):
        self._chk(self.lib.nbco_integrate(self.ctx, scheme, kind, _ptr(buf), n, _ptr(param), dt, scale, int(elastic)))

    def integrate_steps(self, scheme, kind, buf, n, param, dt, steps, scale=1.0, elastic=True):
        self._chk(self.lib.nbco_integrate_steps(self.ctx, scheme, kind, _ptr(buf), n, _ptr(param), dt, scale, int(elastic), int(steps)))

    def direct_2d(self, p, a, n, param=None):
        self._chk(self.lib.nbco_2d_direct(self.ctx, _ptr(p), _ptr(a), n, _ptr(param)))

    def direct3_2d(self, p, a, n, param=None):
        self._chk(self.lib.nbco_2d_direct3(self.ctx, _ptr(p), _ptr(a), n, _ptr(param)))

    def fmm_2d(self, p, a, n, param):
        self._chk(self.lib.nbco_2d_fmm(self.ctx, _ptr(p), _ptr(a), n, _ptr(param)))

    def compute_force_2d(self, kind, buf, n, param, elastic=True):
        self._chk(self.lib.nbco_2d_force(self.ctx, kind, _ptr(buf), n, _ptr(param), int(elastic)))

    def integrate_2d(self, scheme, kind, buf, n, param, dt, scale=1.0, elastic=True):
        self._chk(self.lib.nbco_2d_integrate(self.ctx, scheme, kind, _ptr(buf), n, _ptr(param), dt, scale, int(elastic)))

    def integrate_steps_2d(self, scheme, kind, buf, n, param, dt, steps, scale=1.0, elastic=True):
        self._chk(self.lib.nbco_2d_integrate_steps(self.ctx, scheme, kind, _ptr(buf), n, _ptr(param), dt, scale, int(elastic), int(steps)))

    def mean_relerr_2d(self, x, ref, n):
        out = C.c_double()
        self._chk(self.lib.nbco_2d_mean_relerr(self.ctx, _ptr(x), _ptr(ref), n, C.byref(out)))
        return out.value

    def _energy_2d(self, fn, buf, n, param, phi):
        import numpy as np
        out = (C.c_double * 3)()
        self._chk(fn(self.ctx, _ptr(buf), n, _ptr(param), out, _ptr(phi)))
        return np.array(out[:], dtype=np.float64)

    def energy_2d(self, buf, n, param, phi=None):
        return self._energy_2d(self.lib.nbco_2d_energy, buf, n, param, phi)

    def energy_fmm_2d(self, buf, n, param, phi=None):
        return self._energy_2d(self.lib.nbco_2d_energy_fmm, buf, n, param, phi)

    def minmax(self, p, n):
        out = self.torch.empty(6, dtype=self.torch.float32, device=p.device)
        self._chk(self.lib.nbco_minmax(self.ctx, _ptr(p), n, _ptr(out)))
        return out.view(2, 3)

    def mean_relerr(self, x, ref, n):
        out = C.c_float()
        self._chk(self.lib.nbco_mean_relerr(self.ctx, _ptr(x), _ptr(ref), n, C.byref(out)))
        return out.value

    def pow_sum(self, x, expo, n):
        out = (C.c_double * 3)()
        self._chk(self.lib.nbco_pow_sum(self.ctx, _ptr(x), expo, n, out))
        return list(out)
# ... 163 lines not shown
```

include/nbco.h:

```cpp
#ifndef NBCO_H
#define NBCO_H

#ifdef __cplusplus
extern "C" {
#endif

typedef struct nbco_ctx nbco_ctx;

enum {
	NBCO_OK = 0,
	NBCO_ERR_HIP = 1,
	NBCO_ERR_ARG = 2,
	NBCO_ERR_CAPACITY = 3,
	NBCO_ERR_UNSUPPORTED = 4
};

enum {
	NBCO_EVAL_DIRECT = 0,
	NBCO_EVAL_DIRECT_KAHAN = 1,
	NBCO_EVAL_FMM_KDTREE = 2,
	NBCO_EVAL_FMM_TRACELESS = 3,
	NBCO_EVAL_FMM_SYMMETRIC = 4
};

enum {
	NBCO_INTEG_EULER = 0,
	NBCO_INTEG_PRE_EULER = 1,
	NBCO_INTEG_LEAPFROG = 2,
	NBCO_INTEG_FORESTRUTH = 3,
	NBCO_INTEG_PEFRL = 4
};

typedef struct nbco_opts {
	int   fmm_order;
	float tree_radius;
	float eps2;
	int   coll;
	int   unsort;
	float dens_inhom;
	int   tree_L;
	int   tree_steps;
	int   m2l_first;
	int   sync;
	int   list_factor;
	int   list_grow;
	int   far_fp64;
	int   p2p_mutual;
	int   track_order;
	void *stream;
} nbco_opts;

int nbco_opts_default(nbco_opts *o);

int nbco_create(nbco_ctx **out, const nbco_opts *o);
int nbco_destroy(nbco_ctx *c);
int nbco_set_opts(nbco_ctx *c, const nbco_opts *o);
int nbco_get_opts(const nbco_ctx *c, nbco_opts *o);
const char *nbco_last_error(const nbco_ctx *c);
int nbco_sync(nbco_ctx *c);

int nbco_step(nbco_ctx *c, float *b, const float *a, float ds, long long n);
int nbco_add_elastic(nbco_ctx *c, const float *p, float *a, long long n, const float *k);
int nbco_elastic(nbco_ctx *c, const float *p, float *a, long long n, const float *k);
int nbco_rescale(nbco_ctx *c, float *a, long long n, const float *param);
int nbco_gather(nbco_ctx *c, float *dst, const float *src, const int *map, long long n);
int nbco_gather_inverse(nbco_ctx *c, float *dst, const float *src, const int *map, long long n);
int nbco_copy(nbco_ctx *c, float *dst, const float *src, long long n);

int nbco_direct(nbco_ctx *c, const float *p, float *a, long long n, const float *param);
int nbco_direct3(nbco_ctx *c, const float *p, float *a, long long n, const float *param);
int nbco_fmm_kdtree(nbco_ctx *c, float *p, float *a, long long n, const float *param);
int nbco_fmm_traceless(nbco_ctx *c, float *p, float *a, long long n, const float *param);
int nbco_fmm_symmetric(nbco_ctx *c, float *p, float *a, long long n, const float *param);

int nbco_force(nbco_ctx *c, int kind, float *buf, long long n, const float *param, int elastic);

int nbco_integrate(nbco_ctx *c, int scheme, int kind, float *buf, long long n, const float *param,
                   double dt, double scale, int elastic);
int nbco_integrate_steps(nbco_ctx *c, int scheme, int kind, float *buf, long long n, const float *param,
                         double dt, double scale, int elastic, int steps);

int nbco_minmax(nbco_ctx *c, const float *p, long long n, float *minmax6_dev);
int nbco_mean_relerr(nbco_ctx *c, const float *x, const float *ref, long long n, float *out_host);
int nbco_pow_sum(nbco_ctx *c, const float *x, int expo, long long n, double *out3_host);
int nbco_energy(nbco_ctx *c, const float *buf, long long n, const float *param, double *out3_host);
int nbco_energy_fmm(nbco_ctx *c, const float *buf, long long n, const float *param, double *out3_host);

typedef struct nbco_kd_info {
	int L, ntot, order, mlt_max;
	long long n;
	long long p2p_pairs;
	long long m2l_pairs;
	long long directed_p2p;
	int rebuilt;
	int build_mode;
	int p2p_halves;
	long long warm_builds;
	long long warm_misses;
	int real_bytes;
	int long_lists;
} nbco_kd_info;
int nbco_kd_get_info(nbco_ctx *c, nbco_kd_info *info);

enum {
	NBCO_KD_MULT = 0, NBCO_KD_INDEX = 1, NBCO_KD_SPLITDIM = 2,
	NBCO_KD_CENTER = 3, NBCO_KD_LBOUND = 4, NBCO_KD_RBOUND = 5,
	NBCO_KD_MPOLE = 6,
	NBCO_KD_LOCAL = 7,
	NBCO_KD_P2P_LIST = 8, NBCO_KD_M2L_LIST = 9,
	NBCO_KD_UNSORT = 10,
	NBCO_KD_ORDER = 11
};
int nbco_kd_copy(nbco_ctx *c, int which, void *host_dst, long long host_bytes);

typedef struct nbco_oct_info {
	int L, ntot, order;
	int tpl;
	long long n;
	long long m2l_entries;
	long long p2p_groups, p2p_desc, p2p_chunks;
	int real_bytes;
	int mpole_reals;
} nbco_oct_info;
int nbco_oct_get_info(nbco_ctx *c, nbco_oct_info *out);
enum {
	NBCO_OCT_MULT = 0, NBCO_OCT_INDEX = 1,
	NBCO_OCT_CENTER4 = 2,
	NBCO_OCT_MPOLE = 3, NBCO_OCT_LOCAL = 4,
	NBCO_OCT_KEYS = 5,
	NBCO_OCT_PERM = 6
};
int nbco_oct_copy(nbco_ctx *c, int which, void *host_dst, long long host_bytes);

int nbco_fmm_oct_shard(nbco_ctx *c, float *p, float *a, long long n, const float *param, int symmetric, int world, int rank,
                       long long *bounds_host);

typedef struct nbco_dist_layout {
	int world, rank;
	int d;
	int L, L_local;
	int ntot_local;
	int order;
	long long n_global, n_local;
	long long nodes_bytes;
	long long pos_bytes;
	long long csz_bytes;
	long long mpole_bytes;
	long long let_node_bytes;
	int let_counts;
} nbco_dist_layout;
int nbco_dist_layout_query(nbco_ctx *c, long long n_global, int world, int rank, nbco_dist_layout *out);
int nbco_dist_partition(nbco_ctx *c, const float *state_all, long long n_global, int world, int rank, float *state_local);
int nbco_dist_local(nbco_ctx *c, float *buf_local, long long n_local, void *nodes_send, void *pos_send);
enum {
	NBCO_COLL_DONE = 0,
	NBCO_COLL_ALLREDUCE_MIN_I32 = 1,
	NBCO_COLL_ALLREDUCE_SUM_I32 = 2,
	NBCO_COLL_ALLGATHER = 3,
	NBCO_COLL_ALLTOALL = 4
};
typedef struct nbco_dist_step {
	int op, row_bytes;
	long long send_off, recv_off, count;
	long long rows_send[64], rows_recv[64];
} nbco_dist_step;
int nbco_dist_repartition_workspace(nbco_ctx *c, long long n_global, int world, long long *bytes);
int nbco_dist_repartition_begin(nbco_ctx *c, float *state_local, long long n_global, int world, int rank, void *work,
                                long long work_bytes, nbco_dist_step *next);
int nbco_dist_repartition_next(nbco_ctx *c, nbco_dist_step *next);
int nbco_dist_local_build(nbco_ctx *c, float *buf_local, long long n_local, void *pos_send);
int nbco_dist_local_upward(nbco_ctx *c, float *buf_local, long long n_local, void *nodes_send);
int nbco_dist_finish(nbco_ctx *c, const void *nodes_all, const void *pos_all, float *buf_local, float *a_local,
                     const float *param);
int nbco_dist_local_geom(nbco_ctx *c, float *buf_local, long long n_local, void *pos_send, void *csz_send);
int nbco_dist_local_mpole(nbco_ctx *c, float *buf_local, long long n_local, void *mpole_send);
int nbco_dist_finish_traverse(nbco_ctx *c, const void *csz_all, const void *pos_all);
int nbco_dist_finish_rest(nbco_ctx *c, const void *mpole_all, float *buf_local, float *a_local, const float *param);
int nbco_dist_let_local_geom(nbco_ctx *c, float *buf_local, long long n_local, void *csz_send);
int nbco_dist_let_local_mpole(nbco_ctx *c, float *buf_local, long long n_local);
int nbco_dist_let_select(nbco_ctx *c, const void *csz_all, long long *counts_send);
int nbco_dist_let_pack(nbco_ctx *c, const long long *counts_all, void *pos_send, void *mpole_send);
int nbco_dist_let_finish(nbco_ctx *c, const long long *counts_all, const void *pos_recv, const void *mpole_recv, float *buf_local,
                         float *a_local, const float *param);
int nbco_dist_let_check(nbco_ctx *c);
int nbco_dist_let_pack_capped(nbco_ctx *c, const long long *caps_out, void *pos_send, void *mpole_send);
int nbco_dist_let_finish_capped(nbco_ctx *c, const long long *caps_in, const void *pos_recv, const void *mpole_recv, float *buf_local,
                                float *a_local, const float *param);
int nbco_dist_let_settle(nbco_ctx *c, int ok);
int nbco_dist_turnaround(nbco_ctx *c, float *buf_local, long long n_local, const float *param, double dt, double scale, int elastic);
int nbco_aux_stream(nbco_ctx *c, void **stream_out);

enum {
	NBCO_PH_BUILD = 0, NBCO_PH_P2M_M2M = 1, NBCO_PH_TRAVERSE = 2, NBCO_PH_LISTS = 3, NBCO_PH_P2P = 4,
	NBCO_PH_M2L = 5, NBCO_PH_L2L = 6, NBCO_PH_L2P = 7, NBCO_PH_FINISH = 8, NBCO_PH_DIRECT = 9,
	NBCO_PH_AXPY = 10, NBCO_PH_COUNT = 11
};
int nbco_profile_enable(nbco_ctx *c, int mask);
int nbco_profile_reset(nbco_ctx *c);
int nbco_profile_get(nbco_ctx *c, int phase, double *total_ms, long long *launches);

int nbco_debug_violations(nbco_ctx *c, long long *out8);

#define NBCO_REF_SEED 5351550349027530206ULL
#define NBCO_REF_DISCARD 1248ULL
int nbco_init_gaussian(float *host_state, long long n, const float *sigma_x3, const float *sigma_u3,
                       unsigned long long seed, unsigned long long discard, int uniform_positions);
int nbco_init_gaussian_slice(float *host_slice, long long n, long long first, long long count, const float *sigma_x3,
                             const float *sigma_u3, unsigned long long seed, unsigned long long discard, int uniform_positions);

enum { NBCO_2D_EVAL_DIRECT = 0, NBCO_2D_EVAL_DIRECT_KAHAN = 1, NBCO_2D_EVAL_FMM = 2 };
int nbco_2d_direct(nbco_ctx *c, const double *p, double *a, long long n, const double *param);
int nbco_2d_direct3(nbco_ctx *c, const double *p, double *a, long long n, const double *param);
int nbco_2d_fmm(nbco_ctx *c, double *p, double *a, long long n, const double *param);
int nbco_2d_force(nbco_ctx *c, int kind, double *buf, long long n, const double *param, int elastic);
int nbco_2d_integrate(nbco_ctx *c, int scheme, int kind, double *buf, long long n, const double *param, double dt, double scale,
                      int elastic);
int nbco_2d_integrate_steps(nbco_ctx *c, int scheme, int kind, double *buf, long long n, const double *param, double dt,
                            double scale, int elastic, int steps);
int nbco_2d_mean_relerr(nbco_ctx *c, const double *x, const double *ref, long long n, double *out_host);
int nbco_2d_energy(nbco_ctx *c, const double *buf, long long n, const double *param, double *out3_host, double *phi_dev);
int nbco_2d_energy_fmm(nbco_ctx *c, const double *buf, long long n, const double *param, double *out3_host, double *phi_dev);
int nbco_2d_init_kv(double *host_state, long long n, const double *A2, const double *omega2, unsigned long long seed,
                    unsigned long long discard);
int nbco_2d_init_gaussian(double *host_state, long long n, const double *x2, const double *u2, unsigned long long seed,
                          unsigned long long discard);

#ifdef __cplusplus
}
#endif
#endif
```

Measured before the change: 682.3 million particle-steps/s.

## Fuse top traversal levels into one block kernel and overlap top far-field on second stream

Adds a single-block traverse_head_kernel that walks the first several dual-tree levels in shared memory and replaces that many per-level traverse launches, with a cooldown fallback when its frontier overflows. Separately, it splits M2L by target range so the top-level M2L and L2L run on a new high-priority stream while the remaining M2L runs on the aux stream, then joins before the lower L2L levels. Both aim to cut launch overhead and serialization on small top-of-tree work. The cost is extra streams and events, a head-kernel fallback path, and more complex ordering between the streams.

```diff
diff --git a/coulomb_oscillators_amd/csrc/k_farfield.hip b/coulomb_oscillators_amd/csrc/k_farfield.hip
--- a/coulomb_oscillators_amd/csrc/k_farfield.hip
+++ b/coulomb_oscillators_amd/csrc/k_farfield.hip
@@ -358,18 +358,15 @@
 	return NBCO_OK;
 }
 
-template <int P, typename T>
-static int run_downward_gen(nbco_ctx *c, const float *center, T *local, int L, int dom_d, int dom_g)
+struct DownShape { int ltop, wtop, lroot; };
+template <int P, typename T>
+static DownShape down_shape(int L, int dom_d)
 {
 	constexpr int offL = (P + 1) * (P + 1);
 	int top = kTopNodes;
 	while (top > 4 && (size_t)top * offL * sizeof(T) > 60 * 1024) top >>= 1;
 	int ltop = 1;
 	while (ltop + 1 <= L && (1 << (ltop + 1)) <= top) ++ltop;
-	{
-	}
-	constexpr int offD = P * (P + 1) * (P + 2) / 6;
-	const int threads = 64 * ((std::max(offD, offL) + 63) / 64);
 	const int wtop = ltop >= 2 ? std::max(ltop, L - 7) : 1;
 	int lroot = L;
 	if (ltop >= 2)
@@ -378,13 +375,28 @@
 		while (lroot < L && (size_t)(1 << (L - lroot - 1)) * offL * sizeof(T) > 60 * 1024) ++lroot;
 		if (lroot < dom_d) lroot = L;
 	}
-	for (int lc = 2; lc <= lroot; ++lc)
+	return DownShape{ltop, wtop, lroot};
+}
+
+template <int P, typename T>
+static int run_downward_gen(nbco_ctx *c, const float *center, T *local, int L, int dom_d, int dom_g, int lc_first, int lc_last)
+{
+	constexpr int offL = (P + 1) * (P + 1);
+	const DownShape sh = down_shape<P, T>(L, dom_d);
+	const int ltop = sh.ltop, wtop = sh.wtop, lroot = sh.lroot;
+	if (lc_last >= 0 && lc_last > lroot) return c->fail(NBCO_ERR_ARG, "launch_downward_gen: the level range ends inside the subtree launch");
+	const bool to_end = lc_last < 0;
+	{
+	}
+	constexpr int offD = P * (P + 1) * (P + 2) / 6;
+	const int threads = 64 * ((std::max(offD, offL) + 63) / 64);
+	for (int lc = std::max(2, lc_first); lc <= (to_end ? lroot : lc_last); ++lc)
 	{
 		const int first = lc >= dom_d ? dom_g << (lc - dom_d) : 0, count = lc >= dom_d ? 1 << (lc - dom_d) : 1 << lc;
 		if (lc <= wtop) hipLaunchKernelGGL((l2l_wide_kernel<P, T>), dim3(count), dim3(threads), 0, c->stream, center, local, lc, first);
 		else hipLaunchKernelGGL((l2l_gen_kernel<P, T>), dim3(grid_for(count)), dim3(kBlock), 0, c->stream, center, local, lc, first, count);
 	}
-	if (lroot < L)
+	if (to_end && lroot < L)
 	{
 		const int first = dom_g << (lroot - dom_d), count = 1 << (lroot - dom_d);
 		hipLaunchKernelGGL((l2l_sub_kernel<P, T>), dim3(count), dim3(std::max(64, 1 << (L - lroot))), (size_t)(1 << (L - lroot - 1)) * offL * sizeof(T),
@@ -426,11 +438,11 @@
 	else return run_m2m_top_gen<P, T>(c, center, mpole, mult, ltop, write_geom);
 }
 template <int P, typename T>
-static int run_downward(nbco_ctx *c, const float *center, T *local, int L, int dom_d, int dom_g)
+static int run_downward(nbco_ctx *c, const float *center, T *local, int L, int dom_d, int dom_g, int lc_first, int lc_last)
 {
 	if constexpr (use_wide<P, T>())
 	{
-		for (int lc = 2; lc <= L; ++lc)
+		for (int lc = std::max(2, lc_first); lc <= (lc_last < 0 ? L : std::min(L, lc_last)); ++lc)
 		{
 			const int first = lc >= dom_d ? dom_g << (lc - dom_d) : 0, count = lc >= dom_d ? 1 << (lc - dom_d) : 1 << lc;
 			hipLaunchKernelGGL((l2l_wide_kernel<P, T>), dim3(count), dim3(kWide), 0, c->stream, center, local, lc, first);
@@ -438,7 +450,7 @@
 		NBCO_HIP(hipGetLastError());
 		return NBCO_OK;
 	}
-	else return run_downward_gen<P, T>(c, center, local, L, dom_d, dom_g);
+	else return run_downward_gen<P, T>(c, center, local, L, dom_d, dom_g, lc_first, lc_last);
 }
 
 template <int P, typename T>
@@ -516,15 +528,34 @@
 #undef CALL
 }
 
-int launch_downward_gen(nbco_ctx *c, int P, const float *center, void *local, int L, int dom_d, int dom_g, int f64)
+int launch_downward_gen(nbco_ctx *c, int P, const float *center, void *local, int L, int dom_d, int dom_g, int f64, int lc_first, int lc_last)
 {
 	if (f64)
 	{
-#define CALL(PP) run_downward<PP, double>(c, center, (double *)local, L, dom_d, dom_g)
+#define CALL(PP) run_downward<PP, double>(c, center, (double *)local, L, dom_d, dom_g, lc_first, lc_last)
 		NBCO_DISPATCH_P(P, CALL)
 #undef CALL
 	}
-#define CALL(PP) run_downward<PP, float>(c, center, (float *)local, L, dom_d, dom_g)
+#define CALL(PP) run_downward<PP, float>(c, center, (float *)local, L, dom_d, dom_g, lc_first, lc_last)
+	NBCO_DISPATCH_P(P, CALL)
+#undef CALL
+}
+
+template <int P, typename T>
+static int downward_wtop_of(int L, int dom_d)
+{
+	if constexpr (use_wide<P, T>()) return L;
+	else return down_shape<P, T>(L, dom_d).wtop;
+}
+int launch_downward_wtop(nbco_ctx *c, int P, int L, int dom_d, int f64, int *wtop)
+{
+	if (f64)
+	{
+#define CALL(PP) (*wtop = downward_wtop_of<PP, double>(L, dom_d), NBCO_OK)
+		NBCO_DISPATCH_P(P, CALL)
+#undef CALL
+	}
+#define CALL(PP) (*wtop = downward_wtop_of<PP, float>(L, dom_d), NBCO_OK)
 	NBCO_DISPATCH_P(P, CALL)
 #undef CALL
 }
diff --git a/coulomb_oscillators_amd/csrc/k_fmm_kd.hip b/coulomb_oscillators_amd/csrc/k_fmm_kd.hip
--- a/coulomb_oscillators_amd/csrc/k_fmm_kd.hip
+++ b/coulomb_oscillators_amd/csrc/k_fmm_kd.hip
@@ -314,7 +314,7 @@
 struct KdCounts
 {
 	long long np2p = 0, nm2l = 0;
-	int sel_overflow = 0, react_overflow = 0;
+	int sel_overflow = 0, react_overflow = 0, head_gave_up = 0;
 };
 
 static int kd_list_room(nbco_ctx *c, int ntot, long long &capR, long long &cap)
@@ -357,10 +357,23 @@
 	static_assert(kTcInts <= 1024, "traversal counter block");
 	int *tctr = c->trav_ctr.as<int>();
 	NBCO_TRY(c->flags_begin());
-	hipLaunchKernelGGL(traverse_init_kernel, dim3(grid1d((long long)(2 * (np_ + nm_)) / 8 + 1, 256)), dim3(kBlock), 0, st, fa, ctr, 104, tctr,
-	                   c->list_cnt.as<unsigned>(), (long long)(2 * (np_ + nm_)), (long long)self0, (long long)(c->o.coll ? nself : 0));
+	const long long words = (long long)(2 * (np_ + nm_));
+	int S = std::min(kHeadMaxSteps, L - 1) & ~1;
+	const int fcap = c->trav_head_cap > 0 ? std::min(c->trav_head_cap, kHeadCap) : kHeadCap;
+	if (!c->trav_head_enabled || dm.d != 0 || S < 4 || (long long)(fcap + kTravK - 1) / kTravK > capR) S = 0;
+	if (S > 0 && c->trav_head_cooldown > 0) { --c->trav_head_cooldown; S = 0; }
+	c->trav_head_used = S;
+	if (S > 0)
+		hipLaunchKernelGGL(traverse_head_kernel, dim3(1 + grid1d(words / 32 + 1, 255)), dim3(kHeadBlock), 0, st, tv, tab, (S / 2) & 1 ? fb : fa,
+		                   c->m2l_list.as<int2>(), c->m2l_list.as<int2>() + cap, ctr, 104, tctr, c->list_cnt.as<unsigned>(), words, (long long)self0,
+		                   (long long)(c->o.coll ? nself : 0), (long long)(cnt_m2l - c->list_cnt.as<unsigned>()), S, fcap, capR, c->o.tree_radius,
+		                   c->o.m2l_first, dm);
+	else
+		hipLaunchKernelGGL(traverse_init_kernel, dim3(grid1d(words / 8 + 1, 256)), dim3(kBlock), 0, st, fa, ctr, 104, tctr,
+		                   c->list_cnt.as<unsigned>(), words, (long long)self0, (long long)(c->o.coll ? nself : 0));
 	const int iters = L + NBCO_TRAV_EXTRA;
-	for (int it = 0; it < iters; ++it)
+	if ((S / 2) & 1) std::swap(fa, fb);
+	for (int it = S / 2; it < iters; ++it)
 	{
 		hipLaunchKernelGGL(traverse_kernel, dim3(1024), dim3(kBlock), 0, st, tv, tab, (const int2 *)fa, fb, c->p2p_list.as<int2>(),
 		                   c->m2l_list.as<int2>(), c->p2p_list.as<int2>() + cap, c->m2l_list.as<int2>() + cap, ctr, tctr, it, capR,
@@ -472,14 +485,44 @@
 			NBCO_TRY(build_directed_list(c, c->m2l_list.as<int2>(), c->m2l_list.as<int2>() + cap, m2l_pref, capR, nm2l_hint, 0, 0, 0, ntot, shift, cm,
 			                             c->m2l_start.as<int>(), c->m2l_keys.as<uint64_t>(), c->m2l_keys_alt.as<uint64_t>(), c->scan_tmp_aux));
 			if (let) NBCO_TRY(launch_let_guard(c, c->m2l_keys_alt.as<uint64_t>(), c->m2l_start.as<int>() + ntot, shift, let->node, 0, 2 * nm2l_hint));
+			auto m2l_range = [&](int t_first, int t_end) -> int {
+				PhaseScope ph(c, NBCO_PH_M2L);
+				if (f64) return launch_m2l_lanes_f64(c, P, tv.csz, (const double *)tv.mpole, (double *)tv.local, c->m2l_keys_alt.as<uint64_t>(), c->m2l_start.as<int>(), shift, ntot, 0, t_first, t_end);
+				return launch_m2l_lanes(c, P, tv.csz, tv.mpole, tv.local, c->m2l_keys_alt.as<uint64_t>(), c->m2l_start.as<int>(), shift, ntot, 0, t_first, t_end);
+			};
+			auto l2l_range = [&](int lc_first, int lc_last) -> int {
+				PhaseScope ph(c, NBCO_PH_L2L);
+				return launch_downward_gen(c, P, tv.center, tv.local, L, dm.d, dm.g, f64, lc_first, lc_last);
+			};
+			int wtop = 1;
+			NBCO_TRY(launch_downward_wtop(c, P, L, dm.d, f64, &wtop));
+			const int ls = std::min(wtop - 1, 7);
+			const bool split = c->far_split_enabled && !c->aux_is_main && dm.d == 0 && ls >= 2;
+			c->info.far_split = split ? 1 : 0;
+			if (split)
 			{
-				PhaseScope ph(c, NBCO_PH_M2L);
-				if (f64) NBCO_TRY(launch_m2l_lanes_f64(c, P, tv.csz, (const double *)tv.mpole, (double *)tv.local, c->m2l_keys_alt.as<uint64_t>(), c->m2l_start.as<int>(), shift, ntot));
-				else NBCO_TRY(launch_m2l_lanes(c, P, tv.csz, tv.mpole, tv.local, c->m2l_keys_alt.as<uint64_t>(), c->m2l_start.as<int>(), shift, ntot));
+				const int t_top = (1 << (ls + 1)) - 1;
+				NBCO_TRY(c->far2_ready());
+				NBCO_HIP(hipEventRecord(c->ev_far_fork, c->aux));
+				NBCO_HIP(hipStreamWaitEvent(c->far2, c->ev_far_fork, 0));
+				int rc;
+				{
+					StreamScope on_far2(c, c->far2);
+					rc = m2l_range(0, t_top);
+					if (rc == NBCO_OK) rc = l2l_range(2, ls);
+				}
+				const hipError_t e1 = hipEventRecord(c->ev_far_join, c->far2);
+				if (rc == NBCO_OK) rc = m2l_range(t_top, ntot);
+				const hipError_t e2 = hipStreamWaitEvent(c->aux, c->ev_far_join, 0);
+				NBCO_HIP(e1);
+				NBCO_HIP(e2);
+				NBCO_TRY(rc);
+				NBCO_TRY(l2l_range(ls + 1, -1));
 			}
+			else
 			{
-				PhaseScope ph(c, NBCO_PH_L2L);
-				NBCO_TRY(launch_downward_gen(c, P, tv.center, tv.local, L, dm.d, dm.g, f64));
+				NBCO_TRY(m2l_range(0, ntot));
+				NBCO_TRY(l2l_range(2, -1));
 			}
 		}
 		NBCO_HIP(hipGetLastError());
@@ -500,6 +543,11 @@
 	if (h[3] != 0)
 	{
 		out.sel_overflow = 1;
+		return NBCO_OK;
+	}
+	if (c->trav_head_used > 0 && h[5] != 0)
+	{
+		out.head_gave_up = 1;
 		return NBCO_OK;
 	}
 	if (h[2] == 2) return c->fail(NBCO_ERR_HIP, "internal error: the dual tree traversal did not finish in its launches");
@@ -590,6 +638,7 @@
 	if (rc != NBCO_OK) return rc;
 	if (cnt.sel_overflow)
 		return c->demote_build() ? NBCO_OK : c->fail(NBCO_ERR_UNSUPPORTED, "kd-tree build: tie flag raised by the sorting build");
+	if (cnt.head_gave_up) { c->note_head_gave_up(); return NBCO_OK; }
 	if (rebuild && c->sel_warm_used) c->note_warm_ok();
 	again = false;
 	return NBCO_OK;
@@ -604,6 +653,7 @@
 	nbco_kd_info &info = c->info;
 	info.L = k.L; info.ntot = k.ntot; info.order = k.order; info.mlt_max = k.mlt_max; info.n = k.n;
 	info.p2p_pairs = cnt.np2p; info.m2l_pairs = cnt.nm2l; info.rebuilt = rebuilt ? 1 : 0;
+	info.trav_head_steps = c->trav_head_used;
 	info.directed_p2p = -1;
 }
 
diff --git a/coulomb_oscillators_amd/csrc/k_m2l.hip b/coulomb_oscillators_amd/csrc/k_m2l.hip
--- a/coulomb_oscillators_amd/csrc/k_m2l.hip
+++ b/coulomb_oscillators_amd/csrc/k_m2l.hip
@@ -16,14 +16,14 @@
 template <int P, typename T>
 __global__ __launch_bounds__(64) void m2l_lane_kernel(const float4 *__restrict__ csz, const T *__restrict__ mpole,
                                                       T *__restrict__ local, const uint64_t *__restrict__ keys,
-                                                      const int *__restrict__ start, int shift, int ntot, float eps2, int mstride)
+                                                      const int *__restrict__ start, int shift, int t_first, int t_end, float eps2, int mstride)
 {
 	constexpr int offM = P * (P + 1) * (P + 2) / 6, offL = (P + 1) * (P + 1), NOUT = offL - 1;
 	constexpr int CPL = (NOUT + 63) / 64;
 	__shared__ T buf[64][NOUT + 1 + (NOUT % 2)];
 	__shared__ int tg[64];
 	const int lane = threadIdx.x;
-	const int t0 = blockIdx.x * kTargets, t1 = min(t0 + kTargets, ntot);
+	const int t0 = t_first + blockIdx.x * kTargets, t1 = min(t0 + kTargets, t_end);
 	const int i0 = start[t0], i1 = start[t1];
 	const uint64_t mask = (1ull << shift) - 1;
 	T acc[CPL];
@@ -111,28 +111,32 @@
 }
 
 template <int P, typename T>
-static void launch(nbco_ctx *c, const float4 *csz, const T *mpole, T *local, const uint64_t *keys, const int *start, int shift, int ntot, int mstride)
+static void launch(nbco_ctx *c, const float4 *csz, const T *mpole, T *local, const uint64_t *keys, const int *start, int shift, int t_first, int t_end, int mstride)
 {
-	const int grid = (ntot + kTargets - 1) / kTargets;
-	hipLaunchKernelGGL((m2l_lane_kernel<P, T>), dim3(grid), dim3(64), 0, c->stream, csz, mpole, local, keys, start, shift, ntot, c->o.eps2,
+	if (t_end <= t_first) return;
+	const int grid = (t_end - t_first + kTargets - 1) / kTargets;
+	hipLaunchKernelGGL((m2l_lane_kernel<P, T>), dim3(grid), dim3(64), 0, c->stream, csz, mpole, local, keys, start, shift, t_first, t_end, c->o.eps2,
 	                   mstride > 0 ? mstride : P * (P + 1) * (P + 2) / 6);
 }
 
 template <typename T>
-static int dispatch(nbco_ctx *c, int P, const float4 *csz, const T *mpole, T *local, const uint64_t *keys, const int *start, int shift, int ntot, int mstride)
+static int dispatch(nbco_ctx *c, int P, const float4 *csz, const T *mpole, T *local, const uint64_t *keys, const int *start, int shift, int ntot, int mstride,
+                    int t_first, int t_end)
 {
+	if (t_end < 0) t_end = ntot;
+	if (t_first < 0 || t_end > ntot) return c->fail(NBCO_ERR_ARG, "launch_m2l_lanes: target range outside the list");
 	switch (P)
 	{
-	case 1: launch<1, T>(c, csz, mpole, local, keys, start, shift, ntot, mstride); break;
-	case 2: launch<2, T>(c, csz, mpole, local, keys, start, shift, ntot, mstride); break;
-	case 3: launch<3, T>(c, csz, mpole, local, keys, start, shift, ntot, mstride); break;
-	case 4: launch<4, T>(c, csz, mpole, local, keys, start, shift, ntot, mstride); break;
-	case 5: launch<5, T>(c, csz, mpole, local, keys, start, shift, ntot, mstride); break;
-	case 6: launch<6, T>(c, csz, mpole, local, keys, start, shift, ntot, mstride); break;
-	case 7: launch<7, T>(c, csz, mpole, local, keys, start, shift, ntot, mstride); break;
-	case 8: launch<8, T>(c, csz, mpole, local, keys, start, shift, ntot, mstride); break;
-	case 9: launch<9, T>(c, csz, mpole, local, keys, start, shift, ntot, mstride); break;
-	case 10: launch<10, T>(c, csz, mpole, local, keys, start, shift, ntot, mstride); break;
+	case 1: launch<1, T>(c, csz, mpole, local, keys, start, shift, t_first, t_end, mstride); break;
+	case 2: launch<2, T>(c, csz, mpole, local, keys, start, shift, t_first, t_end, mstride); break;
+	case 3: launch<3, T>(c, csz, mpole, local, keys, start, shift, t_first, t_end, mstride); break;
+	case 4: launch<4, T>(c, csz, mpole, local, keys, start, shift, t_first, t_end, mstride); break;
+	case 5: launch<5, T>(c, csz, mpole, local, keys, start, shift, t_first, t_end, mstride); break;
+	case 6: launch<6, T>(c, csz, mpole, local, keys, start, shift, t_first, t_end, mstride); break;
+	case 7: launch<7, T>(c, csz, mpole, local, keys, start, shift, t_first, t_end, mstride); break;
+	case 8: launch<8, T>(c, csz, mpole, local, keys, start, shift, t_first, t_end, mstride); break;
+	case 9: launch<9, T>(c, csz, mpole, local, keys, start, shift, t_first, t_end, mstride); break;
+	case 10: launch<10, T>(c, csz, mpole, local, keys, start, shift, t_first, t_end, mstride); break;
 	default: return c->fail(NBCO_ERR_UNSUPPORTED, "launch_m2l_lanes: order not generated");
 	}
 	NBCO_HIP(hipGetLastError());
@@ -142,12 +146,12 @@
 }
 
 int launch_m2l_lanes(nbco_ctx *c, int P, const float4 *csz, const float *mpole, float *local, const uint64_t *keys, const int *start,
-                     int shift, int ntot, int mstride)
+                     int shift, int ntot, int mstride, int t_first, int t_end)
 {
-	return dispatch<float>(c, P, csz, mpole, local, keys, start, shift, ntot, mstride);
+	return dispatch<float>(c, P, csz, mpole, local, keys, start, shift, ntot, mstride, t_first, t_end);
 }
 int launch_m2l_lanes_f64(nbco_ctx *c, int P, const float4 *csz, const double *mpole, double *local, const uint64_t *keys, const int *start,
-                         int shift, int ntot, int mstride)
+                         int shift, int ntot, int mstride, int t_first, int t_end)
 {
-	return dispatch<double>(c, P, csz, mpole, local, keys, start, shift, ntot, mstride);
+	return dispatch<double>(c, P, csz, mpole, local, keys, start, shift, ntot, mstride, t_first, t_end);
 }
diff --git a/coulomb_oscillators_amd/csrc/kd_traverse_kernels.hpp b/coulomb_oscillators_amd/csrc/kd_traverse_kernels.hpp
--- a/coulomb_oscillators_amd/csrc/kd_traverse_kernels.hpp
+++ b/coulomb_oscillators_amd/csrc/kd_traverse_kernels.hpp
@@ -256,6 +256,92 @@
 	if (threadIdx.x == 0) { frontier[0] = make_int2(0, 0); tctr[kTcFrontier] = 1; }
 }
 
+constexpr int kHeadBlock = 1024;
+constexpr int kHeadMaxSteps = 10;
+constexpr int kHeadNodes = (1 << kHeadMaxSteps) - 1;
+constexpr int kHeadCap = 8192;
+__global__ __launch_bounds__(kHeadBlock) void traverse_head_kernel(TreeView t, AdmTab tab_arg, int2 *__restrict__ fout, int2 *__restrict__ m2l,
+                                                                   int2 *__restrict__ m2l_rank, int *__restrict__ counters, int nctr, int *__restrict__ tctr,
+                                                                   unsigned *__restrict__ list_cnt, long long words, long long self0, long long nself,
+                                                                   long long m2l_at, int S, int fcap, long long capR, float par, int m2l_first, const Dom dm)
+{
+	const int nrec = (1 << S) - 1;
+	if (blockIdx.x != 0)
+	{
+		for (long long i = (long long)(blockIdx.x - 1) * kHeadBlock + threadIdx.x; i < words; i += (long long)(gridDim.x - 1) * kHeadBlock)
+			if (i < m2l_at || i >= m2l_at + nrec) list_cnt[i] = (i >= self0 && i < self0 + nself) ? 1u : 0u;
+		return;
+	}
+	__shared__ float4 rc_c[kHeadNodes + 1];
+	__shared__ int rc_m[kHeadNodes + 1];
+	__shared__ unsigned hcnt[kHeadNodes + 1];
+	__shared__ int2 fr_a[kHeadCap], fr_b[kHeadCap];
+	__shared__ AdmTab tab;
+	__shared__ int sh_next[kHeadMaxSteps], sh_m2l, sh_flags;
+	const int tid = threadIdx.x;
+	for (int q = tid; q < (int)(sizeof(AdmTab) / sizeof(int)); q += kHeadBlock) reinterpret_cast<int *>(&tab)[q] = reinterpret_cast<const int *>(&tab_arg)[q];
+	for (int i = tid; i < nrec; i += kHeadBlock) { rc_c[i] = t.csz[i]; rc_m[i] = t.mult[i]; hcnt[i] = 0u; }
+	for (int i = tid; i < nctr; i += kHeadBlock) counters[i] = 0;
+	for (int i = tid; i < kTcInts; i += kHeadBlock) tctr[i] = 0;
+	if (tid < kHeadMaxSteps) sh_next[tid] = 0;
+	if (tid == 0) { fr_a[0] = make_int2(0, 0); sh_m2l = 0; sh_flags = 0; }
+	__syncthreads();
+	int ncur = 1;
+	bool full = false;
+	for (int s = 0; s < S; ++s)
+	{
+		const int2 *cur = (s & 1) ? fr_b : fr_a;
+		int2 *nxt = (s & 1) ? fr_a : fr_b;
+		for (int base = 0; base < ncur; base += kHeadBlock)
+		{
+			const int i = base + tid;
+			if (i < ncur)
+			{
+				const int2 p = cur[i];
+				const NodeRec X{rc_c[p.x], rc_m[p.x]}, Y{rc_c[p.y], rc_m[p.y]};
+				const int k = classify_rec(t.ntot, &tab, p, X, Y, par, m2l_first, dm);
+				if (k == 2)
+				{
+					const int e = atomicAdd(&sh_m2l, 1);
+					const long long off = e / kTravK, at = (long long)(e % kTravK) * capR + off;
+					const int sx = (dm.d == 0 || dom_touch(dm, p.x)) ? (int)atomicAdd(&hcnt[p.x], 1u) : -1;
+					const int sy = (dm.d == 0 || dom_touch(dm, p.y)) ? (int)atomicAdd(&hcnt[p.y], 1u) : -1;
+					if (off < capR) { m2l[at] = p; m2l_rank[at] = make_int2(sx, sy); }
+					else sh_flags = 1;
+				}
+				const PairKids g = pair_children(k, p);
+				if (g.n > 0)
+				{
+					const int at = atomicAdd(&sh_next[s], g.n);
+					if (at + g.n <= fcap)
+					{
+						nxt[at] = g.a;
+						nxt[at + 1] = g.b;
+						if (g.n > 2) nxt[at + 2] = g.c;
+					}
+				}
+			}
+		}
+		__syncthreads();
+		ncur = sh_next[s];
+		if (ncur > fcap) { full = true; ncur = 0; break; }
+	}
+	__syncthreads();
+	const int it0 = S / 2, nm = sh_m2l;
+	for (int j = tid; j < ncur; j += kHeadBlock) fout[(long long)(j % kTravK) * capR + j / kTravK] = fr_a[j];
+	if (tid < kTravK)
+	{
+		tctr[kTcFrontier + it0 * kTravK + tid] = (ncur + kTravK - 1 - tid) / kTravK;
+		tctr[kTcM2L + tid] = (nm + kTravK - 1 - tid) / kTravK;
+	}
+	for (int i = tid; i < nrec; i += kHeadBlock) list_cnt[m2l_at + i] = hcnt[i];
+	if (tid == 0)
+	{
+		if (sh_flags) counters[2] = 1;
+		if (full) counters[3] = 1;
+	}
+}
+
 __global__ __launch_bounds__(1024) void traverse_finish_kernel(int *counters, int *tctr, long long capR, unsigned *cnt_all, long long ncnt,
                                                                unsigned *cnt_self, int nself, int *__restrict__ host_flags, int iters, int seq)
 {
@@ -278,7 +364,7 @@
 	}
 	int left = lane < kTravK ? tctr[kTcFrontier + iters * kTravK + lane] : 0;
 	for (int o = 32; o > 0; o >>= 1) left += __shfl_xor(left, o);
-	if (lane == 0) { host_flags[2] = overflow ? 1 : (left != 0 ? 2 : 0); host_flags[3] = counters[110]; }
+	if (lane == 0) { host_flags[2] = overflow ? 1 : (left != 0 ? 2 : 0); host_flags[3] = counters[110]; host_flags[5] = counters[3]; }
 	__threadfence_system();
 	if (lane == 0) __hip_atomic_store(&host_flags[4], seq, __ATOMIC_RELEASE, __HIP_MEMORY_SCOPE_SYSTEM);
 }
diff --git a/coulomb_oscillators_amd/csrc/nbco_api.hip b/coulomb_oscillators_amd/csrc/nbco_api.hip
--- a/coulomb_oscillators_amd/csrc/nbco_api.hip
+++ b/coulomb_oscillators_amd/csrc/nbco_api.hip
@@ -51,6 +51,18 @@
 		NBCO_HIP_M(this, hipEventCreateWithFlags(&ev_join, hipEventDisableTiming));
 	}
 	NBCO_HIP_M(this, hipEventRecord(ev_fork, stream));
+	return NBCO_OK;
+}
+
+int nbco_ctx::far2_ready()
+{
+	if (far2) return NBCO_OK;
+	int prio_lo = 0, prio_hi = 0;
+	NBCO_HIP_M(this, hipDeviceGetStreamPriorityRange(&prio_lo, &prio_hi));
+	if (getenv("NBCO_AUX_PRIO") && atoi(getenv("NBCO_AUX_PRIO")) == 0) prio_hi = prio_lo;
+	NBCO_HIP_M(this, hipStreamCreateWithPriority(&far2, hipStreamNonBlocking, prio_hi));
+	NBCO_HIP_M(this, hipEventCreateWithFlags(&ev_far_fork, hipEventDisableTiming));
+	NBCO_HIP_M(this, hipEventCreateWithFlags(&ev_far_join, hipEventDisableTiming));
 	return NBCO_OK;
 }
 
@@ -184,6 +196,9 @@
 	c->stream = (hipStream_t)c->o.stream;
 	c->poison = getenv("NBCO_POISON") && atoi(getenv("NBCO_POISON")) != 0;
 	if (getenv("NBCO_SEL_WARM")) c->sel_warm_enabled = atoi(getenv("NBCO_SEL_WARM")) != 0;
+	if (getenv("NBCO_TRAV_HEAD")) c->trav_head_enabled = atoi(getenv("NBCO_TRAV_HEAD")) != 0;
+	if (getenv("NBCO_TRAV_HEAD_CAP")) c->trav_head_cap = atoi(getenv("NBCO_TRAV_HEAD_CAP"));
+	if (getenv("NBCO_FAR_SPLIT")) c->far_split_enabled = atoi(getenv("NBCO_FAR_SPLIT")) != 0;
 	if (hipMalloc(&c->small.ptr, 4096) != hipSuccess) { delete c; return NBCO_ERR_HIP; }
 	c->small.bytes = 4096;
 	*out = c;
@@ -198,6 +213,9 @@
 	if (!c) return NBCO_OK;
 	hipStreamSynchronize(c->stream);
 	if (c->aux && !c->aux_is_main) { hipStreamSynchronize(c->aux); hipStreamDestroy(c->aux); }
+	if (c->far2) { hipStreamSynchronize(c->far2); hipStreamDestroy(c->far2); }
+	if (c->ev_far_fork) hipEventDestroy(c->ev_far_fork);
+	if (c->ev_far_join) hipEventDestroy(c->ev_far_join);
 	if (c->ev_fork) hipEventDestroy(c->ev_fork);
 	if (c->ev_join) hipEventDestroy(c->ev_join);
 	if (c->ev_flags) hipEventDestroy(c->ev_flags);
diff --git a/coulomb_oscillators_amd/csrc/nbco_internal.hpp b/coulomb_oscillators_amd/csrc/nbco_internal.hpp
--- a/coulomb_oscillators_amd/csrc/nbco_internal.hpp
+++ b/coulomb_oscillators_amd/csrc/nbco_internal.hpp
@@ -116,6 +116,10 @@
 	hipStream_t aux = nullptr;
 	hipEvent_t ev_fork = nullptr, ev_join = nullptr;
 	bool aux_pending = false;
+	hipStream_t far2 = nullptr;
+	hipEvent_t ev_far_fork = nullptr, ev_far_join = nullptr;
+	bool far_split_enabled = true;
+	int far2_ready();
 	int list_growth = 1;
 	bool grow_lists(int ntot)
 	{
@@ -211,6 +215,13 @@
 		if (!sel_three_pass) { sel_three_pass = true; return true; }
 		if (!force_sort_build) { force_sort_build = true; return true; }
 		return false;
+	}
+	bool trav_head_enabled = true;
+	int trav_head_cap = 0, trav_head_used = 0, trav_head_cooldown = 0, trav_head_cool_len = 128;
+	void note_head_gave_up()
+	{
+		trav_head_cooldown = trav_head_cool_len;
+		trav_head_cool_len = trav_head_cool_len < 2048 ? 2 * trav_head_cool_len : 4096;
 	}
 	bool demote_build()
 	{
@@ -325,7 +336,8 @@
                     float *lbound, float *rbound, int *splitdim, int *index, int *flag, bool warm = false, const KdRoot &root = KdRoot{});
 int launch_upward_gen(nbco_ctx *c, int P, const float4 *pos, float *center, void *mpole, int *mult, const int *index, int L, int write_geom, int f64 = 0);
 int launch_kd_centres(nbco_ctx *c, float *center, int *mult, int L, const float *lbound, const float *rbound, float4 *csz);
-int launch_downward_gen(nbco_ctx *c, int P, const float *center, void *local, int L, int dom_d, int dom_g, int f64 = 0);
+int launch_downward_gen(nbco_ctx *c, int P, const float *center, void *local, int L, int dom_d, int dom_g, int f64 = 0, int lc_first = 2, int lc_last = -1);
+int launch_downward_wtop(nbco_ctx *c, int P, int L, int dom_d, int f64, int *wtop);
 int launch_m2m_top_gen(nbco_ctx *c, int P, float *center, void *mpole, int *mult, int ltop, int L, int write_geom, int f64 = 0);
 int launch_kd_centres_top(nbco_ctx *c, float *center, int *mult, int ltop, const float *lbound, const float *rbound, float4 *csz);
 int launch_l2p_gen(nbco_ctx *c, int P, const float4 *pos, const float *center, const void *local, const float4 *near, const int *chunk_off,
@@ -333,6 +345,6 @@
                    long long own0, long long own_n, const int2 *sec_range = nullptr, const float4 *react = nullptr, long long react_cap = 0,
                    int react_stride = 32, int f64 = 0);
 int launch_m2l_lanes(nbco_ctx *c, int P, const float4 *csz, const float *mpole, float *local, const uint64_t *keys, const int *start,
-                     int shift, int ntot, int mstride = 0);
+                     int shift, int ntot, int mstride = 0, int t_first = 0, int t_end = -1);
 int launch_m2l_lanes_f64(nbco_ctx *c, int P, const float4 *csz, const double *mpole, double *local, const uint64_t *keys, const int *start,
-                         int shift, int ntot, int mstride = 0);
+                         int shift, int ntot, int mstride = 0, int t_first = 0, int t_end = -1);
diff --git a/coulomb_oscillators_amd/engine.py b/coulomb_oscillators_amd/engine.py
--- a/coulomb_oscillators_amd/engine.py
+++ b/coulomb_oscillators_amd/engine.py
@@ -36,7 +36,8 @@
     _fields_ = [("L", C.c_int), ("ntot", C.c_int), ("order", C.c_int), ("mlt_max", C.c_int), ("n", C.c_longlong),
                 ("p2p_pairs", C.c_longlong), ("m2l_pairs", C.c_longlong), ("directed_p2p", C.c_longlong),
                 ("rebuilt", C.c_int), ("build_mode", C.c_int), ("p2p_halves", C.c_int), ("warm_builds", C.c_longlong), ("warm_misses", C.c_longlong),
-                ("real_bytes", C.c_int), ("long_lists", C.c_int)]
+                ("real_bytes", C.c_int), ("long_lists", C.c_int), ("trav_head_steps", C.c_int),
+                ("far_split", C.c_int)]
 
 
 class OctInfo(C.Structure):
diff --git a/include/nbco.h b/include/nbco.h
--- a/include/nbco.h
+++ b/include/nbco.h
@@ -99,6 +99,8 @@
 	long long warm_misses;
 	int real_bytes;
 	int long_lists;
+	int trav_head_steps;
+	int far_split;
 } nbco_kd_info;
 int nbco_kd_get_info(nbco_ctx *c, nbco_kd_info *info);
 
```

Result: slower. 667.3 million particle-steps/s (-2.2%).
